# jlogan03/interpn

Hardware: AMD Instinct MI355X
Metric: Mpoints/sec (f64) per GPU + achieved HBM GB/s vs roofline, 3D linear-regular (higher is better)
Workload: dtype f64

## Files before the change

### interpn_amd/csrc/abi_binned.hip

```cpp
#include "abi_internal.h"

using namespace interpn;
using namespace interpn_abi;

namespace interpn_abi {


size_t bin_slice_points(const GridDesc& g) {
  const int lg = g.cfg.bin_slice_log2 >= 16 && g.cfg.bin_slice_log2 <= 27 ? g.cfg.bin_slice_log2 : 25;
  const size_t s = (size_t)1 << lg;
  return s < kBinSlicePoints ? s : kBinSlicePoints;
}

int binned_applies(const GridDesc& g, size_t npoints) {
  if (g.method != kCubic || !g.bricks || g.ndims < 2 || g.ndims > 4) return 0;
  if (g.cfg.binned == 0 || g.cfg.force_generic) return 1;
  const bool main11 = g.brick_step[0] == 1 && g.brick_step[1] == 1;
  const bool second = !main11 && g.bricks11 != nullptr;
  if (g.cfg.binned < 0) {
    if (g.ndims != 4 && g.ndims != 3) return 0;
    if (!main11 && !second) return 0;
    if (g.ndims == 3) return 0;
    if (main11) {
      unsigned nb[2];
// ... 117 lines not shown
    } else if (column) {
      if (g.dtype == kF64)
        err = launch_cubic_column<double>(*use, plan, extras, index, reinterpret_cast<double*>(dst), count, max_parts, h->first_bad, begin, stream);
      else
        err = launch_cubic_column<float>(*use, plan, extras, index, reinterpret_cast<float*>(dst), count, max_parts, h->first_bad, begin, stream);
    } else if (g.dtype == kF64) {
      err = launch_cubic_brick<double>(*use, reinterpret_cast<const double* const*>(sorted), reinterpret_cast<double*>(dst), count,
                                       h->first_bad, stream, index, begin);
    } else {
      err = launch_cubic_brick<float>(*use, reinterpret_cast<const float* const*>(sorted), reinterpret_cast<float*>(dst), count,
                                      h->first_bad, stream, index, begin);
    }
  }
  release_bin_slot(h, slot, stream, stage && err == hipSuccess && hipEventRecord(stage[4], stream) == hipSuccess);
  if (err == hipSuccess) {
    std::lock_guard<std::mutex> lk(h->bin_mu);
    h->desc.tag = use->tag;
    h->desc.last_binned = 1;
  }
  if (err != hipSuccess) {
    (void)hipGetLastError();
    return hip_fail(err);
  }
  return INTERPN_HIP_OK;
}

}

extern "C" {

int interpn_hip_eval_device_ex(interpn_hip_interp* h, const void* const* obs, size_t nobs, void* out, size_t npoints,
                               void* stream, unsigned flags, int* path_taken, int* why_out) {
  if (path_taken) *path_taken = INTERPN_HIP_PATH_IN_PLACE;
  if (why_out) *why_out = INTERPN_HIP_WHY_NONE;
  if (!h || (!obs && nobs)) return INTERPN_HIP_ERR_INVALID_ARGUMENT;
  if (flags & ~(unsigned)INTERPN_HIP_EVAL_NO_ALLOC) return INTERPN_HIP_ERR_INVALID_ARGUMENT;
  int st = validate_obs(h->desc, nullptr, nobs, npoints);
  if (st) return st;
  if (npoints == 0) return INTERPN_HIP_OK;
  if (!out) return INTERPN_HIP_ERR_INVALID_ARGUMENT;
  for (size_t i = 0; i < nobs; ++i)
    if (!obs[i]) return INTERPN_HIP_ERR_INVALID_ARGUMENT;
  DeviceGuard guard(h->device);
  if (!guard.ok()) return INTERPN_HIP_ERR_NO_DEVICE;
  int why = INTERPN_HIP_WHY_NONE;
  st = eval_device_binned(h, obs, out, npoints, static_cast<hipStream_t>(stream), flags, &why);
  if (why_out) *why_out = why;
  if (st > 0) {
    std::lock_guard<std::mutex> lk(h->marks_mu);
    h->sync_device_at_destroy = true;
    return st;
  }
  bool swept = false;
  if (st < 0 && sweep_applies(h->desc, npoints)) {
    int why_sweep = INTERPN_HIP_WHY_NONE;
    const int ss = eval_device_sweep(h, obs, out, npoints, static_cast<hipStream_t>(stream), flags, &why_sweep);
    if (why_out && (why == INTERPN_HIP_WHY_NONE || why_sweep > INTERPN_HIP_WHY_SMALL_OR_OFF)) *why_out = why_sweep;
    if (ss > 0) {
      std::lock_guard<std::mutex> lk(h->marks_mu);
      h->sync_device_at_destroy = true;
      return ss;
    }
    swept = ss == 0;
  }
  if (swept) {
    if (path_taken) *path_taken = INTERPN_HIP_PATH_SWEEP;
    h->desc.last_binned = 0;
    h->evals_sweep.fetch_add(1);
  } else if (st < 0) {
    HIP_TRY(launch_any(h->desc, obs, out, npoints, h->first_bad, static_cast<hipStream_t>(stream)));
    if (binned_applies(h->desc, npoints)) {
      std::lock_guard<std::mutex> lk(h->bin_mu);
      h->desc.last_binned = 0;
    } else {
      h->desc.last_binned = 0;
    }
    h->evals_in_place.fetch_add(1);
  } else {
    if (path_taken) *path_taken = INTERPN_HIP_PATH_BINNED;
    h->evals_binned.fetch_add(1);
  }
  mark_stream(h, static_cast<hipStream_t>(stream));
  return INTERPN_HIP_OK;
}

int interpn_hip_eval_device(interpn_hip_interp* h, const void* const* obs, size_t nobs, void* out, size_t npoints,
                            void* stream) {
  return interpn_hip_eval_device_ex(h, obs, nobs, out, npoints, stream, 0u, nullptr, nullptr);
}

int interpn_hip_stage_ms(interpn_hip_interp* h, double* ms, size_t n) {
  if (!h || !ms || n < 4) return INTERPN_HIP_ERR_INVALID_ARGUMENT;
  DeviceGuard guard(h->device);
  if (!guard.ok()) return INTERPN_HIP_ERR_NO_DEVICE;
  std::lock_guard<std::mutex> lk(h->bin_mu);
  const interpn_hip_interp::BinSlot* best = nullptr;
  for (const auto& sl : h->bin_slots)
    if (sl.staged && !sl.busy && (!best || sl.stamp > best->stamp)) best = &sl;
  if (!best) return INTERPN_HIP_ERR_INVALID_ARGUMENT;
  HIP_TRY(hipEventSynchronize(best->stage[4]));
  for (int k = 0; k < 4; ++k) {
    float f = 0.f;
    HIP_TRY(hipEventElapsedTime(&f, best->stage[k], best->stage[k + 1]));
    ms[k] = (double)f;
  }
  return INTERPN_HIP_OK;
}

int interpn_hip_reserve(interpn_hip_interp* h, size_t npoints, int nstreams) {
  if (!h || nstreams < 0) return INTERPN_HIP_ERR_INVALID_ARGUMENT;
  if ((size_t)nstreams > interpn_hip_interp::kMaxBinSlots) nstreams = (int)interpn_hip_interp::kMaxBinSlots;
  const GridDesc& g = h->desc;
  const bool sorts = binned_applies(g, npoints) >= 2, sweeps = sweep_applies(g, npoints) >= 2;
  if (npoints == 0 || nstreams == 0 || (!sorts && !sweeps)) return INTERPN_HIP_OK;
  DeviceGuard guard(h->device);
  if (!guard.ok()) return INTERPN_HIP_ERR_NO_DEVICE;
  const size_t slice_max = bin_slice_points(g);
  const size_t need = sorts ? bin_scratch_bytes(g, npoints < slice_max ? npoints : slice_max) : sweep_work_bytes();
  return reserve_slots(h, need, nstreams);
}

}
```

### interpn_amd/csrc/abi_create.hip

```cpp
#include "abi_internal.h"
#include "cubic_cell_record.h"

using namespace interpn;
using namespace interpn_abi;

namespace interpn_abi {

thread_local bool t_defer_tables = false;

int finish_create(interpn_hip_interp* h, const void* vals, size_t nvals, size_t elem, int vals_mem) {
  GridDesc& g = h->desc;
  {
    const DeviceProps dp = device_props(h->device);
    g.cfg.num_cus = dp.num_cus;
    g.cfg.num_xcds = dp.num_xcds;
    g.cfg.l2_bytes = dp.l2_bytes;
    g.cfg.lds_per_cu = dp.lds_per_cu;
    g.cfg.lds_per_wg = dp.lds_per_wg;
  }
  latch_env(g.cfg);
  g.nvals = nvals;
  if (vals_mem == INTERPN_HIP_MEM_DEVICE) {
    g.vals = vals;
  } else {
// ... 474 lines not shown
  g.axis_image = nullptr;
  g.tag = KernelTag();
  for (int d = 0; d < 8; ++d) g.grid[d] = nullptr;
  const size_t elem = g.dtype == kF64 ? 8 : 4;
  hipError_t e = pool_alloc(dev, &h->vals_owned, g.nvals * elem);
  if (e == hipSuccess) e = hipMemcpyPeer(h->vals_owned, dev, src->desc.vals, src->device, g.nvals * elem);
  if (e == hipSuccess && src->desc.axis_image && g.axis_alloc_bytes) {
    e = pool_alloc(dev, &h->grids_owned, g.axis_alloc_bytes);
    if (e == hipSuccess) e = hipMemcpyPeer(h->grids_owned, dev, src->desc.axis_image, src->device, g.axis_alloc_bytes);
    if (e == hipSuccess) {
      g.axis_image = h->grids_owned;
      for (int d = 0; d < g.ndims; ++d) g.grid[d] = (const char*)h->grids_owned + g.axis_g_off[d];
    }
  }
  if (e != hipSuccess) {
    interpn_hip_destroy(h);
    return hip_fail(e);
  }
  st = finish_create(h, h->vals_owned, g.nvals, elem, INTERPN_HIP_MEM_DEVICE);
  if (st) {
    interpn_hip_destroy(h);
    return st;
  }
  *out = h;
  return INTERPN_HIP_OK;
}

int interpn_hip_elem_size(const interpn_hip_interp* h) { return h ? (h->desc.dtype == kF64 ? 8 : 4) : 0; }
int interpn_hip_ndims(const interpn_hip_interp* h) { return h ? h->desc.ndims : 0; }
int interpn_hip_device(const interpn_hip_interp* h) { return h ? h->device : -1; }

void interpn_hip_destroy(interpn_hip_interp* h) {
  if (!h) return;
  DeviceGuard guard(h->device);
  scratch_slots::destroy_wait(*h, [h] {
    bool ok = true;
    for (auto& l : h->lane)
      if (l.stream && hipStreamSynchronize(l.stream) != hipSuccess) { (void)hipGetLastError(); ok = false; }
    return ok;
  });
  for (auto& l : h->lane) {
    if (l.stream) pool_return_kit(h->device, l.stream, l.flag_host);
    pool_free(h->device, l.flag_dev);
    pool_free(h->device, l.obs);
    pool_free(h->device, l.out);
  }
  pool_return_small(h->device, h->small_host);
  scratch_slots::free_blocks(*h, [](interpn_hip_interp::BinSlot& sl) {
    for (hipEvent_t e : sl.stage)
      if (e) (void)hipEventDestroy(e);
  });
  pool_free(h->device, h->first_bad);
  pool_return_pinned_word(h->device, h->finish_word);
  pool_return_pinned_word(h->device, h->sampling.host);
  pool_free(h->device, h->grids_owned);
  pool_free(h->device, h->bricks_owned);
  pool_free(h->device, h->bricks11_owned);
  pool_free(h->device, h->sweep_owned);
  pool_free(h->device, h->vals_owned);
  delete h;
}

}
```

### interpn_amd/csrc/abi_fields.hip

```cpp
#include <climits>

#include "abi_internal.h"

using namespace interpn;
using namespace interpn_abi;

namespace {

struct DeferTables {
  explicit DeferTables(bool on) { t_defer_tables = on; }
  ~DeferTables() { t_defer_tables = false; }
};

long long env_number(const char* name, long long fallback) {
  const char* env = getenv(name);
  if (!env || !*env) return fallback;
  char* end = nullptr;
  const long long v = strtoll(env, &end, 0);
  return (end == env || *end != 0) ? fallback : v;
}

}

namespace interpn_abi {
// ... 299 lines not shown
  for (size_t i = 0; i < nobs; ++i)
    if (!obs[i]) return INTERPN_HIP_ERR_INVALID_ARGUMENT;
  DeviceGuard guard(s->device);
  if (!guard.ok()) return INTERPN_HIP_ERR_NO_DEVICE;
  hipStream_t hs = static_cast<hipStream_t>(stream);
  const bool fused = columns_take_fused(s, npoints, hs, flags);
  st = eval_columns(s, fused, obs, out, out_stride, npoints, hs, flags);
  if (st == INTERPN_HIP_OK && fused && path_taken) *path_taken = INTERPN_HIP_FIELDS_PATH_FUSED;
  return st;
}

int interpn_hip_fields_finish(interpn_hip_fields* s, void* stream, uint64_t* first_bad_index) {
  if (!s || s->sub.empty()) return INTERPN_HIP_ERR_INVALID_ARGUMENT;
  const size_t count = s->per_field_pending ? s->nfields : 1;
  s->per_field_pending = false;
  if (count > 1 && count <= (size_t)kMaxStatusWords) {
    unsigned long long* words[kMaxStatusWords];
    for (size_t f = 0; f < count; ++f) words[f] = s->sub[f]->first_bad;
    const int st = finish_words(s->sub[0], static_cast<hipStream_t>(stream), words, (int)count, first_bad_index);
    if (st >= 0) return st;
  }
  int error = INTERPN_HIP_OK;
  uint64_t best = ~(uint64_t)0;
  for (size_t f = 0; f < count; ++f) {
    uint64_t bad = 0;
    const int st = interpn_hip_finish(s->sub[f], stream, &bad);
    if (st == s->sub[f]->desc.unrep_status) best = bad < best ? bad : best;
    else if (st != INTERPN_HIP_OK && error == INTERPN_HIP_OK) error = st;
  }
  if (error) return error;
  if (best != ~(uint64_t)0) {
    if (first_bad_index) *first_bad_index = best;
    return s->sub[0]->desc.unrep_status;
  }
  return INTERPN_HIP_OK;
}

int interpn_hip_fields_eval_host(interpn_hip_fields* s, const void* const* obs, const size_t* obs_lens, size_t nobs, void* out,
                                 size_t out_stride, size_t nout) {
  if (!s || s->sub.empty() || (!obs && nobs) || (!obs_lens && nobs)) return INTERPN_HIP_ERR_INVALID_ARGUMENT;
  int st = validate_obs(s->sub[0]->desc, obs_lens, nobs, nout);
  if (st) return st;
  if (nout == 0) return INTERPN_HIP_OK;
  if (!out || out_stride < nout) return INTERPN_HIP_ERR_INVALID_ARGUMENT;
  for (size_t i = 0; i < nobs; ++i)
    if (!obs[i]) return INTERPN_HIP_ERR_INVALID_ARGUMENT;
  DeviceGuard guard(s->device);
  if (!guard.ok()) return INTERPN_HIP_ERR_NO_DEVICE;
  const size_t elem = s->dtype == kF64 ? 8 : 4;
  const long long opt_chunk = s->sub[0]->desc.cfg.host_chunk;
  size_t chunk = opt_chunk >= 1 ? (size_t)opt_chunk : ((size_t)2 << 20);
  if (chunk > nout) chunk = nout;
  std::lock_guard<std::mutex> host_lock(s->host_mu);
  if (!s->stream) HIP_TRY(pool_take_kit(s->device, &s->stream, &s->kit_word));
  if (s->host_points < chunk) {
    HIP_TRY(hipStreamSynchronize(s->stream));
    pool_free(s->device, s->host_obs);
    pool_free(s->device, s->host_out);
    s->host_obs = s->host_out = nullptr;
    s->host_points = 0;
    HIP_TRY(pool_alloc(s->device, &s->host_obs, (size_t)s->ndims * chunk * elem));
    HIP_TRY(pool_alloc(s->device, &s->host_out, s->nfields * chunk * elem));
    s->host_points = chunk;
  }
  const size_t cap = s->host_points;
  char* dev_obs_base = static_cast<char*>(s->host_obs);
  char* dev_out = static_cast<char*>(s->host_out);
  const void* dev_obs[8];
  for (size_t begin = 0; begin < nout; begin += chunk) {
    const size_t count = nout - begin < chunk ? nout - begin : chunk;
    for (int d = 0; d < s->ndims; ++d) {
      char* dst = dev_obs_base + (size_t)d * cap * elem;
      HIP_TRY(hipMemcpyAsync(dst, static_cast<const char*>(obs[d]) + begin * elem, count * elem, hipMemcpyHostToDevice, s->stream));
      dev_obs[d] = dst;
    }
    st = interpn_hip_fields_eval_device(s, dev_obs, nobs, dev_out, cap, count, s->stream, 0u, nullptr);
    if (st) return st;
    uint64_t bad = 0;
    st = interpn_hip_fields_finish(s, s->stream, &bad);
    const bool failed = st == s->sub[0]->desc.unrep_status;
    if (st && !failed) return st;
    const size_t good = failed ? (size_t)bad : count;
    if (good)
      for (size_t f = 0; f < s->nfields; ++f)
        HIP_TRY(hipMemcpyAsync(static_cast<char*>(out) + (f * out_stride + begin) * elem, dev_out + f * cap * elem, good * elem,
                               hipMemcpyDeviceToHost, s->stream));
    HIP_TRY(hipStreamSynchronize(s->stream));
    if (failed) return st;
  }
  return INTERPN_HIP_OK;
}

int interpn_hip_fields_eval_points_device(interpn_hip_fields* s, const void* pts, size_t point_stride, size_t npoints, void* out,
                                          size_t out_stride, void* stream, unsigned flags, int* path_taken) {
  if (path_taken) *path_taken = INTERPN_HIP_FIELDS_POINTS_PATH_SPLIT;
  if (flags & ~(unsigned)INTERPN_HIP_EVAL_NO_ALLOC) return INTERPN_HIP_ERR_INVALID_ARGUMENT;
  bool nothing = false;
  int path = INTERPN_HIP_FIELDS_POINTS_PATH_SPLIT;
  const int st0 = points_checks(s, pts, point_stride, npoints, out, out_stride, &nothing, &path);
  if (st0 || nothing) return st0;
  DeviceGuard guard(s->device);
  if (!guard.ok()) return INTERPN_HIP_ERR_NO_DEVICE;
  const int st = points_device(s, path, pts, point_stride, npoints, out, out_stride, static_cast<hipStream_t>(stream), flags);
  if (st == INTERPN_HIP_OK && path_taken) *path_taken = path;
  return st;
}

int interpn_hip_fields_reserve_points(interpn_hip_fields* s, size_t npoints, int nstreams) {
  if (!s || s->sub.empty() || nstreams < 0) return INTERPN_HIP_ERR_INVALID_ARGUMENT;
  if ((size_t)nstreams > interpn_hip_interp::kMaxBinSlots) nstreams = (int)interpn_hip_interp::kMaxBinSlots;
  if (npoints == 0 || nstreams == 0) return INTERPN_HIP_OK;
  DeviceGuard guard(s->device);
  if (!guard.ok()) return INTERPN_HIP_ERR_NO_DEVICE;
  return reserve_slots(s->sub[0], points_need(s, npoints), nstreams);
}

int interpn_hip_fields_eval_points_host(interpn_hip_fields* s, const void* pts, size_t point_stride, size_t npoints, void* out,
                                        size_t out_stride) {
  bool nothing = false;
  int path = INTERPN_HIP_FIELDS_POINTS_PATH_SPLIT;
  const int st0 = points_checks(s, pts, point_stride, npoints, out, out_stride, &nothing, &path);
  if (st0 || nothing) return st0;
  DeviceGuard guard(s->device);
  if (!guard.ok()) return INTERPN_HIP_ERR_NO_DEVICE;
  const size_t elem = s->dtype == kF64 ? 8 : 4;
  const size_t nd = (size_t)s->ndims, k = s->nfields;
  const long long opt_chunk = s->sub[0]->desc.cfg.host_chunk;
  size_t chunk = opt_chunk >= 1 ? (size_t)opt_chunk : ((size_t)2 << 20);
  if (chunk > npoints) chunk = npoints;
  const size_t widest = point_stride > k ? point_stride : k;
  const size_t cap = ((size_t)256 << 20) / (widest * elem);
  if (chunk > cap) chunk = cap ? cap : 1;
  std::lock_guard<std::mutex> host_lock(s->host_mu);
  if (!s->stream) HIP_TRY(pool_take_kit(s->device, &s->stream, &s->kit_word));
  const size_t rows_bytes = align_up(chunk * point_stride * elem, 256);
  void* block = nullptr;
  if (pool_alloc(s->device, &block, rows_bytes + chunk * k * elem) != hipSuccess) { (void)hipGetLastError(); return INTERPN_HIP_ERR_OUT_OF_MEMORY; }
  char* results = static_cast<char*>(block) + rows_bytes;
  hipError_t err = hipSuccess;
  int st = INTERPN_HIP_OK;
  for (size_t begin = 0; begin < npoints && err == hipSuccess && st == INTERPN_HIP_OK; begin += chunk) {
    const size_t count = npoints - begin < chunk ? npoints - begin : chunk;
    err = hipMemcpyAsync(block, static_cast<const char*>(pts) + begin * point_stride * elem, ((count - 1) * point_stride + nd) * elem,
                         hipMemcpyHostToDevice, s->stream);
    if (err != hipSuccess) break;
    st = points_device(s, path, block, point_stride, count, results, k, s->stream, 0u);
    if (st) break;
    uint64_t bad = 0;
    st = interpn_hip_fields_finish(s, s->stream, &bad);
    const bool failed = st == s->sub[0]->desc.unrep_status;
    if (st && !failed) break;
    const size_t good = failed ? (size_t)bad : count;
    char* dst = static_cast<char*>(out) + begin * out_stride * elem;
    if (good && out_stride == k) err = hipMemcpyAsync(dst, results, good * k * elem, hipMemcpyDeviceToHost, s->stream);
    else if (good) err = hipMemcpy2DAsync(dst, out_stride * elem, results, k * elem, k * elem, good, hipMemcpyDeviceToHost, s->stream);
    if (err == hipSuccess) err = hipStreamSynchronize(s->stream);
  }
  (void)hipStreamSynchronize(s->stream);
  pool_free(s->device, block);
  if (err != hipSuccess) return hip_fail(err);
  return st;
}

void interpn_hip_fields_destroy(interpn_hip_fields* s) {
  if (!s) return;
  DeviceGuard guard(s->device);
  if (s->stream && hipStreamSynchronize(s->stream) != hipSuccess) (void)hipGetLastError();
  for (interpn_hip_interp* h : s->sub) interpn_hip_destroy(h);
  if (s->stream) pool_return_kit(s->device, s->stream, s->kit_word);
  pool_free(s->device, s->host_obs);
  pool_free(s->device, s->host_out);
  pool_free(s->device, s->host_grad);
  pool_free(s->device, s->table);
  pool_free(s->device, s->vals_owned);
  delete s;
}

size_t interpn_hip_fields_count(const interpn_hip_fields* s) { return s ? s->nfields : 0; }
int interpn_hip_fields_ndims(const interpn_hip_fields* s) { return s ? s->ndims : 0; }
int interpn_hip_fields_elem_size(const interpn_hip_fields* s) { return s ? (s->dtype == kF64 ? 8 : 4) : 0; }
int interpn_hip_fields_device(const interpn_hip_fields* s) { return s ? s->device : -1; }

int interpn_hip_fields_kernel_name(const interpn_hip_fields* s, char* buf, size_t buflen) {
  if (!s || s->sub.empty()) return INTERPN_HIP_ERR_INVALID_ARGUMENT;
  return interpn_hip_kernel_name(s->sub[0], buf, buflen);
}
// ... 56 lines not shown
```

### interpn_amd/csrc/abi_fields_grad.hip

```cpp
#include "abi_internal.h"

using namespace interpn;
using namespace interpn_abi;

namespace {

bool grad_auto_takes_fused(const interpn_hip_fields* s) { return s->table != nullptr; }

bool grad_takes_fused(const interpn_hip_fields* s) {
  return s->table && (s->fused == 1 || (s->fused < 0 && grad_auto_takes_fused(s)));
}

int fields_grad_checks(const interpn_hip_fields* s, const void* const* obs, const size_t* obs_lens, bool need_lens, size_t nobs,
                       const void* out, size_t out_stride, const void* grad, size_t grad_stride, size_t npoints, bool* nothing) {
  *nothing = false;
  if (!s || s->sub.empty() || (!obs && nobs) || (need_lens && !obs_lens && nobs)) return INTERPN_HIP_ERR_INVALID_ARGUMENT;
  const int method = s->sub[0]->desc.method;
  if (method != kLinear && method != kCubic) return INTERPN_HIP_ERR_UNSUPPORTED;
  const int st = validate_obs(s->sub[0]->desc, obs_lens, nobs, npoints);
  if (st) return st;
  if (npoints == 0) { *nothing = true; return INTERPN_HIP_OK; }
  if (!out || out_stride < npoints || !grad || grad_stride < npoints) return INTERPN_HIP_ERR_INVALID_ARGUMENT;
  for (size_t i = 0; i < nobs; ++i)
    if (!obs[i]) return INTERPN_HIP_ERR_INVALID_ARGUMENT;
// ... 12 lines not shown
    return INTERPN_HIP_OK;
  }
  if (!s->sub_tables && !(flags & INTERPN_HIP_EVAL_NO_ALLOC) && !stream_capturing(hs)) {
    const int st = ensure_sub_tables(s);
    if (st) return st;
  }
  const size_t elem = s->dtype == kF64 ? 8 : 4;
  const size_t nd = (size_t)s->ndims;
  const bool cubic = s->sub[0]->desc.method == kCubic;
  s->per_field_pending = true;
  s->last_path = INTERPN_HIP_FIELDS_PATH_PER_FIELD;
  for (size_t f = 0; f < s->nfields; ++f) {
    void* rows[8];
    for (size_t d = 0; d < nd; ++d) rows[d] = static_cast<char*>(grad) + (f * nd + d) * grad_stride * elem;
    void* out_f = static_cast<char*>(out) + f * out_stride * elem;
    const int st = cubic ? interpn_hip_eval_cubic_grad_device(s->sub[f], obs, nobs, out_f, rows, npoints, hs)
                         : interpn_hip_eval_grad_device(s->sub[f], obs, nobs, out_f, rows, npoints, hs);
    if (st) return st;
  }
  return INTERPN_HIP_OK;
}

}

extern "C" {

int interpn_hip_fields_eval_grad_device(interpn_hip_fields* s, const void* const* obs, size_t nobs, void* out, size_t out_stride,
                                        void* grad, size_t grad_stride, size_t npoints, void* stream, unsigned flags,
                                        int* path_taken) {
  if (path_taken) *path_taken = INTERPN_HIP_FIELDS_PATH_PER_FIELD;
  if (flags & ~(unsigned)INTERPN_HIP_EVAL_NO_ALLOC) return INTERPN_HIP_ERR_INVALID_ARGUMENT;
  bool nothing = false;
  const int st = fields_grad_checks(s, obs, nullptr, false, nobs, out, out_stride, grad, grad_stride, npoints, &nothing);
  if (st || nothing) return st;
  DeviceGuard guard(s->device);
  if (!guard.ok()) return INTERPN_HIP_ERR_NO_DEVICE;
  return fields_grad_device(s, obs, nobs, out, out_stride, grad, grad_stride, npoints, static_cast<hipStream_t>(stream), flags,
                            path_taken);
}

int interpn_hip_fields_eval_grad_host(interpn_hip_fields* s, const void* const* obs, const size_t* obs_lens, size_t nobs, void* out,
                                      size_t out_stride, void* grad, size_t grad_stride, size_t nout) {
  bool nothing = false;
  int st = fields_grad_checks(s, obs, obs_lens, true, nobs, out, out_stride, grad, grad_stride, nout, &nothing);
  if (st || nothing) return st;
  DeviceGuard guard(s->device);
  if (!guard.ok()) return INTERPN_HIP_ERR_NO_DEVICE;
  const size_t elem = s->dtype == kF64 ? 8 : 4;
  const size_t nd = (size_t)s->ndims;
  const long long opt_chunk = s->sub[0]->desc.cfg.host_chunk;
  size_t chunk = opt_chunk >= 1 ? (size_t)opt_chunk : ((size_t)2 << 20);
  if (chunk > nout) chunk = nout;
  std::lock_guard<std::mutex> host_lock(s->host_mu);
  if (!s->stream) HIP_TRY(pool_take_kit(s->device, &s->stream, &s->kit_word));
  if (s->host_points < chunk) {
    HIP_TRY(hipStreamSynchronize(s->stream));
    pool_free(s->device, s->host_obs);
    pool_free(s->device, s->host_out);
    s->host_obs = s->host_out = nullptr;
    s->host_points = 0;
    HIP_TRY(pool_alloc(s->device, &s->host_obs, nd * chunk * elem));
    HIP_TRY(pool_alloc(s->device, &s->host_out, s->nfields * chunk * elem));
    s->host_points = chunk;
  }
  if (s->host_grad_points < chunk) {
    HIP_TRY(hipStreamSynchronize(s->stream));
    pool_free(s->device, s->host_grad);
    s->host_grad = nullptr;
    s->host_grad_points = 0;
    HIP_TRY(pool_alloc(s->device, &s->host_grad, s->nfields * nd * chunk * elem));
    s->host_grad_points = chunk;
  }
  const size_t cap = s->host_points, gcap = s->host_grad_points;
  char* dev_obs_base = static_cast<char*>(s->host_obs);
  char* dev_out = static_cast<char*>(s->host_out);
  char* dev_grad = static_cast<char*>(s->host_grad);
  const void* dev_obs[8];
  for (size_t begin = 0; begin < nout; begin += chunk) {
    const size_t count = nout - begin < chunk ? nout - begin : chunk;
    for (size_t d = 0; d < nd; ++d) {
      char* dst = dev_obs_base + d * cap * elem;
      HIP_TRY(hipMemcpyAsync(dst, static_cast<const char*>(obs[d]) + begin * elem, count * elem, hipMemcpyHostToDevice, s->stream));
      dev_obs[d] = dst;
    }
    st = fields_grad_device(s, dev_obs, nobs, dev_out, cap, dev_grad, gcap, count, s->stream, 0u, nullptr);
    if (st) return st;
    uint64_t bad = 0;
    st = interpn_hip_fields_finish(s, s->stream, &bad);
    const bool failed = st == s->sub[0]->desc.unrep_status;
    if (st && !failed) return st;
    const size_t good = failed ? (size_t)bad : count;
    if (good)
      for (size_t f = 0; f < s->nfields; ++f) {
        HIP_TRY(hipMemcpyAsync(static_cast<char*>(out) + (f * out_stride + begin) * elem, dev_out + f * cap * elem, good * elem,
                               hipMemcpyDeviceToHost, s->stream));
        for (size_t d = 0; d < nd; ++d)
          HIP_TRY(hipMemcpyAsync(static_cast<char*>(grad) + ((f * nd + d) * grad_stride + begin) * elem,
                                 dev_grad + (f * nd + d) * gcap * elem, good * elem, hipMemcpyDeviceToHost, s->stream));
      }
    HIP_TRY(hipStreamSynchronize(s->stream));
    if (failed) return st;
  }
  return INTERPN_HIP_OK;
}

}
// ... 1 lines not shown
```

### interpn_amd/csrc/abi_fields_lattice.hip

```cpp
#include "abi_internal.h"
#include "lattice.h"

using namespace interpn;
using namespace interpn_abi;

namespace {

using Slot = interpn_hip_interp::BinSlot;

constexpr size_t kHostChunkPointsFields = (size_t)1 << 25;

bool layout_ok(int layout) { return layout == INTERPN_HIP_FIELDS_LATTICE_FIELD_MAJOR || layout == INTERPN_HIP_FIELDS_LATTICE_FIELDS_LAST; }

FieldsLatticePlan plan_for(const interpn_hip_fields* s, const LatticeShape& sh, int layout) {
  const GridDesc& g = s->sub[0]->desc;
  if (!fast_path(g) || g.cfg.force_generic) return FieldsLatticePlan();
  return fields_lattice_plan(g.method, g.ndims, g.dtype == kF64 ? 8 : 4, g.n, sh.m, s->nfields, layout, lattice_lds_budget(g.cfg),
                             g.cfg.num_cus, g.cfg.lattice);
}

size_t slice_leading(const interpn_hip_fields* s, const LatticeShape& sh) {
  const size_t elem = s->dtype == kF64 ? 8 : 4;
  size_t points = kExpandSliceBytes / (s->nfields * elem);
  const long long opt = s->sub[0]->desc.cfg.points_slice;
// ... 126 lines not shown
}

}

extern "C" {

int interpn_hip_fields_eval_lattice_device(interpn_hip_fields* s, const void* const* axes, const size_t* axis_lens, size_t naxes,
                                           void* out, size_t out_stride, int layout, void* stream, unsigned flags, int* path_taken) {
  if (path_taken) *path_taken = INTERPN_HIP_FIELDS_LATTICE_PATH_PER_FIELD;
  if (flags & ~(unsigned)INTERPN_HIP_EVAL_NO_ALLOC) return INTERPN_HIP_ERR_INVALID_ARGUMENT;
  LatticeShape sh;
  bool empty = false;
  const int st = checks(s, axes, axis_lens, naxes, out, out_stride, layout, &sh, &empty);
  if (st || empty) return st;
  DeviceGuard guard(s->device);
  if (!guard.ok()) return INTERPN_HIP_ERR_NO_DEVICE;
  return fields_lattice_device(s, sh, out, out_stride, layout, static_cast<hipStream_t>(stream), flags, path_taken);
}

int interpn_hip_fields_reserve_lattice(interpn_hip_fields* s, const size_t* axis_lens, size_t naxes, int nstreams) {
  if (!s || s->sub.empty() || nstreams < 0 || (!axis_lens && naxes)) return INTERPN_HIP_ERR_INVALID_ARGUMENT;
  interpn_hip_interp* h0 = s->sub[0];
  if (is_one_dim(h0->desc.method)) return INTERPN_HIP_ERR_UNSUPPORTED;
  int st = validate_obs(h0->desc, nullptr, naxes, 0);
  if (st) return st;
  LatticeShape sh;
  st = lattice_make_shape(nullptr, axis_lens, naxes, &sh);
  if (st) return st;
  if ((size_t)nstreams > interpn_hip_interp::kMaxBinSlots) nstreams = (int)interpn_hip_interp::kMaxBinSlots;
  if (sh.npoints == 0 || nstreams == 0) return INTERPN_HIP_OK;
  DeviceGuard guard(s->device);
  if (!guard.ok()) return INTERPN_HIP_ERR_NO_DEVICE;
  for (size_t f = 1; f < s->nfields; ++f) {
    st = reserve_slots(s->sub[f], lattice_reserve_need(s->sub[f]->desc, sh), nstreams);
    if (st) return st;
  }
  size_t need = lattice_reserve_need(h0->desc, sh);
  const size_t rows = join_need(s, sh);
  if (rows > need) need = rows;
  int blocks = 2 * nstreams;
  if ((size_t)blocks > interpn_hip_interp::kMaxBinSlots) blocks = (int)interpn_hip_interp::kMaxBinSlots;
  return reserve_slots(h0, need, blocks);
}

int interpn_hip_fields_eval_lattice_host(interpn_hip_fields* s, const void* const* axes, const size_t* axis_lens, size_t naxes,
                                         void* out, size_t out_stride, int layout, uint64_t* first_bad_index) {
  LatticeShape sh;
  bool empty = false;
  int st = checks(s, axes, axis_lens, naxes, out, out_stride, layout, &sh, &empty);
  if (st || empty) return st;
  DeviceGuard guard(s->device);
  if (!guard.ok()) return INTERPN_HIP_ERR_NO_DEVICE;
  std::lock_guard<std::mutex> host_lock(s->host_mu);
  if (!s->stream) HIP_TRY(pool_take_kit(s->device, &s->stream, &s->kit_word));
  const size_t elem = s->dtype == kF64 ? 8 : 4;
  const size_t k = s->nfields;
  const bool last = layout == INTERPN_HIP_FIELDS_LATTICE_FIELDS_LAST;
  const size_t per0 = (size_t)sh.weight[0];
  const long long opt_chunk = s->sub[0]->desc.cfg.host_chunk;
  const size_t chunk_points = opt_chunk >= 1 ? (size_t)opt_chunk : kHostChunkPointsFields / k;
  size_t rows0 = chunk_points / per0;
  if (rows0 < 1) rows0 = 1;
  if (rows0 > sh.m[0]) rows0 = sh.m[0];
  size_t axes_bytes = 0, off[8] = {0};
  for (int d = 0; d < sh.ndims; ++d) { off[d] = axes_bytes; axes_bytes += align_up(sh.m[d] * elem, 256); }
  void* block = nullptr;
  if (pool_alloc(s->device, &block, axes_bytes + rows0 * per0 * k * elem) != hipSuccess) { (void)hipGetLastError(); return INTERPN_HIP_ERR_OUT_OF_MEMORY; }
  char* dev_out = static_cast<char*>(block) + axes_bytes;
  hipError_t err = hipSuccess;
  for (int d = 0; d < sh.ndims && err == hipSuccess; ++d)
    err = hipMemcpyAsync(static_cast<char*>(block) + off[d], axes[d], sh.m[d] * elem, hipMemcpyHostToDevice, s->stream);
  st = INTERPN_HIP_OK;
  for (size_t i0 = 0; i0 < sh.m[0] && err == hipSuccess && st == INTERPN_HIP_OK; i0 += rows0) {
    const size_t cnt0 = sh.m[0] - i0 < rows0 ? sh.m[0] - i0 : rows0;
    const void* sub_axes[8];
    size_t sub_lens[8];
    for (int d = 0; d < sh.ndims; ++d) {
      sub_axes[d] = static_cast<char*>(block) + off[d] + (d == 0 ? i0 * elem : 0);
      sub_lens[d] = d == 0 ? cnt0 : sh.m[d];
    }
    LatticeShape sub;
    st = lattice_make_shape(sub_axes, sub_lens, (size_t)sh.ndims, &sub);
    if (st) break;
    const size_t count = sub.npoints;
    st = fields_lattice_device(s, sub, dev_out, last ? k : count, layout, s->stream, 0u, nullptr);
    if (st) break;
    uint64_t bad = 0;
    st = interpn_hip_fields_finish(s, s->stream, &bad);
    const bool failed = st == s->sub[0]->desc.unrep_status;
    if (st && !failed) break;
    const size_t good = failed ? (size_t)bad : count;
    if (failed && first_bad_index) *first_bad_index = (uint64_t)(i0 * per0 + good);
    if (good && !last) {
      for (size_t f = 0; f < k && err == hipSuccess; ++f)
        err = hipMemcpyAsync(static_cast<char*>(out) + (f * out_stride + i0 * per0) * elem, dev_out + f * count * elem, good * elem,
                             hipMemcpyDeviceToHost, s->stream);
    } else if (good) {
      char* dst = static_cast<char*>(out) + i0 * per0 * out_stride * elem;
      if (out_stride == k) err = hipMemcpyAsync(dst, dev_out, good * k * elem, hipMemcpyDeviceToHost, s->stream);
      else err = hipMemcpy2DAsync(dst, out_stride * elem, dev_out, k * elem, k * elem, good, hipMemcpyDeviceToHost, s->stream);
    }
    if (err == hipSuccess) err = hipStreamSynchronize(s->stream);
  }
  (void)hipStreamSynchronize(s->stream);
  pool_free(s->device, block);
  if (err != hipSuccess) return hip_fail(err);
// ... 26 lines not shown
```

### interpn_amd/csrc/abi_grad.hip

```cpp
#include "abi_internal.h"

using namespace interpn;
using namespace interpn_abi;

namespace {

constexpr size_t kGradChunkPoints = (size_t)2 << 20;

struct PoolBlock {
  int device;
  void* p = nullptr;
  explicit PoolBlock(int dev) : device(dev) {}
  ~PoolBlock() { if (p) pool_free(device, p); }
};

int grad_checks(interpn_hip_interp* h, int method, const void* const* obs, const size_t* obs_lens, bool need_lens, size_t nobs,
                void* out, void* const* grad, size_t npoints, bool* nothing) {
  *nothing = false;
  if (!h || (!obs && nobs) || (need_lens && !obs_lens && nobs)) return INTERPN_HIP_ERR_INVALID_ARGUMENT;
  if (h->desc.method != method) return INTERPN_HIP_ERR_UNSUPPORTED;
  const int st = validate_obs(h->desc, obs_lens, nobs, npoints);
  if (st) return st;
  if (npoints == 0) { *nothing = true; return INTERPN_HIP_OK; }
  if (!out || !grad) return INTERPN_HIP_ERR_INVALID_ARGUMENT;
  for (size_t i = 0; i < nobs; ++i)
    if (!obs[i] || !grad[i]) return INTERPN_HIP_ERR_INVALID_ARGUMENT;
  return INTERPN_HIP_OK;
}

}

namespace interpn_abi {

hipError_t launch_grad(const GridDesc& g, const void* const* obs, void* out, void* const* grad, size_t npts,
                       unsigned long long* first_bad, hipStream_t stream) {
  return g.method == kCubic ? launch_cubic_grad(g, obs, out, grad, npts, first_bad, stream)
                            : launch_linear_grad(g, obs, out, grad, npts, first_bad, stream);
}

}

namespace {

int grad_device(interpn_hip_interp* h, int method, const void* const* obs, size_t nobs, void* out, void* const* grad,
                size_t npoints, void* stream) {
  bool nothing = false;
  const int st = grad_checks(h, method, obs, nullptr, false, nobs, out, grad, npoints, &nothing);
  if (st || nothing) return st;
  DeviceGuard guard(h->device);
  if (!guard.ok()) return INTERPN_HIP_ERR_NO_DEVICE;
  HIP_TRY(launch_grad(h->desc, obs, out, grad, npoints, h->first_bad, static_cast<hipStream_t>(stream)));
  h->desc.last_binned = 0;
  h->evals_in_place.fetch_add(1);
  mark_stream(h, static_cast<hipStream_t>(stream));
  return INTERPN_HIP_OK;
}

int grad_host(interpn_hip_interp* h, int method, const void* const* obs, const size_t* obs_lens, size_t nobs, void* out, size_t nout,
              void* const* grad) {
  bool nothing = false;
  const int st0 = grad_checks(h, method, obs, obs_lens, true, nobs, out, grad, nout, &nothing);
  if (st0 || nothing) return st0;
  std::lock_guard<std::mutex> host_lock(h->host_mu);
  DeviceGuard guard(h->device);
  if (!guard.ok()) return INTERPN_HIP_ERR_NO_DEVICE;
  const size_t elem = h->desc.dtype == kF64 ? 8 : 4;
  const int nd = h->desc.ndims;
  size_t chunk = nout < kGradChunkPoints ? nout : kGradChunkPoints;
  if (h->desc.cfg.host_chunk >= 1)
    chunk = (size_t)h->desc.cfg.host_chunk < nout ? (size_t)h->desc.cfg.host_chunk : nout;
  const int st = ensure_lane(h, 0, chunk);
  if (st) return st;
  const interpn_hip_interp::HostLane& l = h->lane[0];
  PoolBlock gbuf(h->device);
  if (pool_alloc(h->device, &gbuf.p, (size_t)nd * chunk * elem) != hipSuccess) {
    (void)hipGetLastError();
    gbuf.p = nullptr;
    return INTERPN_HIP_ERR_OUT_OF_MEMORY;
  }
  const void* dev_obs[8];
  void* dev_grad[8];
  for (int d = 0; d < nd; ++d) {
    dev_obs[d] = (char*)l.obs + (size_t)d * l.points * elem;
    dev_grad[d] = (char*)gbuf.p + (size_t)d * chunk * elem;
  }
  for (size_t begin = 0; begin < nout; begin += chunk) {
    const size_t count = (nout - begin) < chunk ? (nout - begin) : chunk;
    for (int d = 0; d < nd; ++d)
      HIP_TRY(hipMemcpyAsync(const_cast<void*>(dev_obs[d]), (const char*)obs[d] + begin * elem, count * elem, hipMemcpyHostToDevice, l.stream));
    HIP_TRY(launch_grad(h->desc, dev_obs, l.out, dev_grad, count, l.flag_dev, l.stream));
    HIP_TRY(hipMemcpyAsync(l.flag_host, l.flag_dev, sizeof(unsigned long long), hipMemcpyDeviceToHost, l.stream));
    HIP_TRY(hipStreamSynchronize(l.stream));
    const unsigned long long bad = *l.flag_host;
    size_t good = count;
    if (bad != kNoBadIndexHost) {
      HIP_TRY(hipMemsetAsync(l.flag_dev, 0xFF, sizeof(unsigned long long), l.stream));
      good = (size_t)bad;
    }
    if (good) {
      HIP_TRY(hipMemcpyAsync((char*)out + begin * elem, l.out, good * elem, hipMemcpyDeviceToHost, l.stream));
      for (int d = 0; d < nd; ++d)
        HIP_TRY(hipMemcpyAsync((char*)grad[d] + begin * elem, dev_grad[d], good * elem, hipMemcpyDeviceToHost, l.stream));
    }
    HIP_TRY(hipStreamSynchronize(l.stream));
    if (bad != kNoBadIndexHost) return h->desc.unrep_status;
  }
  return INTERPN_HIP_OK;
}

}

extern "C" {

int interpn_hip_eval_grad_device(interpn_hip_interp* h, const void* const* obs, size_t nobs, void* out, void* const* grad,
                                 size_t npoints, void* stream) {
  return grad_device(h, kLinear, obs, nobs, out, grad, npoints, stream);
// ... 19 lines not shown
```

### interpn_amd/csrc/abi_host.hip

```cpp
#include "abi_internal.h"

using namespace interpn;
using namespace interpn_abi;

namespace interpn_abi {

int ensure_lane(interpn_hip_interp* h, int which, size_t points) {
  interpn_hip_interp::HostLane& l = h->lane[which];
  if (l.points >= points && l.obs) return INTERPN_HIP_OK;
  const size_t elem = h->desc.dtype == kF64 ? 8 : 4;
  if (l.obs) { HIP_TRY(hipStreamSynchronize(l.stream)); pool_free(h->device, l.obs); l.obs = nullptr; }
  if (l.out) { pool_free(h->device, l.out); l.out = nullptr; }
  l.points = 0;
  if (!l.stream) HIP_TRY(pool_take_kit(h->device, &l.stream, &l.flag_host));
  HIP_TRY(pool_alloc(h->device, &l.obs, (size_t)h->desc.ndims * points * elem));
  HIP_TRY(pool_alloc(h->device, &l.out, points * elem));
  if (!l.flag_dev) {
    HIP_TRY(pool_alloc(h->device, (void**)&l.flag_dev, sizeof(unsigned long long)));
    HIP_TRY(hipMemsetAsync(l.flag_dev, 0xFF, sizeof(unsigned long long), l.stream));
  }
  l.points = points;
  return INTERPN_HIP_OK;
}

// ... 80 lines not shown
    void* buf = nullptr;
    if (pool_take_small(h->device, &buf) != hipSuccess) { (void)hipGetLastError(); return kSmallPathUnavailable; }
    void* dbuf = nullptr;
    if (hipHostGetDevicePointer(&dbuf, buf, 0) != hipSuccess || !dbuf) {
      (void)hipGetLastError();
      pool_return_small(h->device, buf);
      return kSmallPathUnavailable;
    }
    h->small_host = buf;
    h->small_dev = dbuf;
  }
  if (!l.stream) HIP_TRY(pool_take_kit(h->device, &l.stream, &l.flag_host));
  if (!l.flag_dev) {
    HIP_TRY(pool_alloc(h->device, (void**)&l.flag_dev, sizeof(unsigned long long)));
    HIP_TRY(hipMemsetAsync(l.flag_dev, 0xFF, sizeof(unsigned long long), l.stream));
  }
  const size_t elem = h->desc.dtype == kF64 ? 8 : 4;
  const int nd = h->desc.ndims;
  const size_t stride = kSmallPoints * 8;
  const void* dev_obs[8];
  for (int d = 0; d < nd; ++d) {
    memcpy((char*)h->small_host + (size_t)d * stride, obs[d], nout * elem);
    dev_obs[d] = (const char*)h->small_dev + (size_t)d * stride;
  }
  char* host_out = (char*)h->small_host + (size_t)8 * stride;
  void* dev_out = (char*)h->small_dev + (size_t)8 * stride;
  HIP_TRY(launch_any(h->desc, dev_obs, dev_out, nout, l.flag_dev, l.stream));
  HIP_TRY(hipMemcpyAsync(l.flag_host, l.flag_dev, sizeof(unsigned long long), hipMemcpyDeviceToHost, l.stream));
  HIP_TRY(hipStreamSynchronize(l.stream));
  const unsigned long long bad = *l.flag_host;
  size_t good = nout;
  if (bad != kNoBadIndexHost) {
    HIP_TRY(hipMemsetAsync(l.flag_dev, 0xFF, sizeof(unsigned long long), l.stream));
    good = (size_t)bad;
  }
  if (good) memcpy(out, host_out, good * elem);
  if (bad != kNoBadIndexHost) {
    if (bad_index) *bad_index = (size_t)bad;
    return h->desc.unrep_status;
  }
  return INTERPN_HIP_OK;
}

constexpr size_t kPipelineChunkPoints = (size_t)2 << 20;

}

namespace interpn_abi {

int eval_host_impl(interpn_hip_interp* h, const void* const* obs, size_t nobs, void* out, size_t nout,
                          size_t* bad_index) {
  (void)nobs;
  std::lock_guard<std::mutex> host_lock(h->host_mu);
  DeviceGuard guard(h->device);
  if (!guard.ok()) return INTERPN_HIP_ERR_NO_DEVICE;
  if (nout <= kSmallPoints && h->desc.cfg.host_chunk < 1) {
    const int sst = eval_host_small(h, obs, out, nout, bad_index);
    if (sst != kSmallPathUnavailable) return sst;
  }
  HostPipeline p;
  p.h = h;
  p.obs = obs;
  p.out = out;
  p.nout = nout;
  p.chunk = nout <= kPipelineChunkPoints ? nout : kPipelineChunkPoints;
  if (h->desc.cfg.host_chunk >= 1)
    p.chunk = (size_t)h->desc.cfg.host_chunk < nout ? (size_t)h->desc.cfg.host_chunk : nout;
  p.nchunks = (nout + p.chunk - 1) / p.chunk;
  int st = ensure_lane(h, 0, p.chunk);
  if (st) return st;
  if (p.nchunks > 1) {
    st = ensure_lane(h, 1, p.chunk);
    if (st) return st;
    std::thread helper([&p] { p.lane_main(1); });
    p.lane_main(0);
    helper.join();
  } else {
    p.checked[1] = ~(size_t)0;
    p.lane_main(0);
  }
  if (p.error) return p.error;
  if (p.fail_chunk != ~(size_t)0) {
    if (bad_index) *bad_index = p.fail_index;
    return h->desc.unrep_status;
  }
  return INTERPN_HIP_OK;
}

}

namespace {
struct StatusWords {
  const unsigned long long* word[interpn_abi::kMaxStatusWords];
  int count;
};
__global__ void k_status_to_host(StatusWords w, unsigned long long* host_word) {
  unsigned long long v = ~0ull;
  for (int k = 0; k < w.count; ++k) {
    const unsigned long long x = __hip_atomic_load(w.word[k], __ATOMIC_RELAXED, __HIP_MEMORY_SCOPE_AGENT);
    v = x < v ? x : v;
  }
  __hip_atomic_store(host_word, v, __ATOMIC_RELEASE, __HIP_MEMORY_SCOPE_SYSTEM);
}
}

namespace interpn_abi {

int finish_words(interpn_hip_interp* h, hipStream_t s, unsigned long long* const* words, int count, uint64_t* first_bad_index) {
  DeviceGuard guard(h->device);
  if (!guard.ok()) return INTERPN_HIP_ERR_NO_DEVICE;
  std::lock_guard<std::mutex> lk(h->finish_mu);
  if (!h->finish_word) {
    HIP_TRY(pool_take_pinned_word(h->device, &h->finish_word));
    void* dp = nullptr;
    if (hipHostGetDevicePointer(&dp, h->finish_word, 0) == hipSuccess) h->finish_word_dev = static_cast<unsigned long long*>(dp);
    else (void)hipGetLastError();
  }
  hipStreamCaptureStatus cs = hipStreamCaptureStatusNone;
  const hipError_t asked = hipStreamIsCapturing(s, &cs);
  if (asked != hipSuccess) (void)hipGetLastError();
  const bool by_kernel = h->finish_word_dev && h->desc.cfg.finish_kernel != 0 && count <= kMaxStatusWords && asked == hipSuccess &&
                         cs == hipStreamCaptureStatusNone;
  if (!by_kernel && count > 1) return -1;
  if (by_kernel) {
    StatusWords w;
    for (int k = 0; k < kMaxStatusWords; ++k) w.word[k] = words[k < count ? k : 0];
    w.count = count;
    hipLaunchKernelGGL(k_status_to_host, dim3(1), dim3(1), 0, s, w, h->finish_word_dev);
    HIP_TRY(hipGetLastError());
  } else {
    HIP_TRY(hipMemcpyAsync(h->finish_word, words[0], sizeof(unsigned long long), hipMemcpyDeviceToHost, s));
  }
  HIP_TRY(hipStreamSynchronize(s));
  const unsigned long long word = *(volatile unsigned long long*)h->finish_word;
  if (word == kNoBadIndexHost) return INTERPN_HIP_OK;
  for (int k = 0; k < count; ++k) HIP_TRY(hipMemsetAsync(words[k], 0xFF, sizeof(word), s));
  HIP_TRY(hipStreamSynchronize(s));
  if (first_bad_index) *first_bad_index = (uint64_t)word;
  return h->desc.unrep_status;
}

}

extern "C" {

int interpn_hip_finish(interpn_hip_interp* h, void* stream, uint64_t* first_bad_index) {
  if (!h) return INTERPN_HIP_ERR_INVALID_ARGUMENT;
  return finish_words(h, static_cast<hipStream_t>(stream), &h->first_bad, 1, first_bad_index);
}

int interpn_hip_eval_host(interpn_hip_interp* h, const void* const* obs, const size_t* obs_lens, size_t nobs,
                          void* out, size_t nout) {
  if (!h || (!obs && nobs) || (!obs_lens && nobs)) return INTERPN_HIP_ERR_INVALID_ARGUMENT;
  int st = validate_obs(h->desc, obs_lens, nobs, nout);
  if (st) return st;
  if (nout == 0) return INTERPN_HIP_OK;
  if (!out) return INTERPN_HIP_ERR_INVALID_ARGUMENT;
  for (size_t i = 0; i < nobs; ++i)
    if (!obs[i]) return INTERPN_HIP_ERR_INVALID_ARGUMENT;
  return eval_host_impl(h, obs, nobs, out, nout, nullptr);
}

#define ONESHOT_TAIL(T)                                                                         \
  st = interpn_hip_eval_host(h, reinterpret_cast<const void* const*>(obs), obs_lens, nobs, out, nout); \
  interpn_hip_destroy(h);                                                                       \
  return st;

#define ONESHOT_PRECHECK(METHOD, NDIMS, VALIDATE)                  \
  {                                                                \
    int pst = (VALIDATE);                                          \
    if (pst) return pst;                                           \
    GridDesc tmp;                                                  \
    tmp.method = (METHOD);                                         \
    tmp.ndims = (int)(NDIMS);                                      \
    if (!obs_lens && nobs) return INTERPN_HIP_ERR_INVALID_ARGUMENT; \
    pst = validate_obs(tmp, obs_lens, nobs, nout);                 \
    if (pst) return pst;                                           \
  }

#define DEFINE_ONESHOT(T, SUFFIX)                                                                             \
  int interpn_hip_linear_regular_##SUFFIX(const size_t* dims, size_t ndims, const T* starts, size_t nstarts, \
                                          const T* steps, size_t nsteps, const T* vals, size_t nvals,        \
                                          const T* const* obs, const size_t* obs_lens, size_t nobs, T* out,  \
                                          size_t nout) {                                                     \
                                                                               \
    if (nstarts != ndims || nsteps != ndims || nobs != ndims) return INTERPN_HIP_ERR_DIM_MISMATCH;           \
    ONESHOT_PRECHECK(kLinear, ndims, validate_regular<T>(kLinear, dims, ndims, starts, nstarts, steps, nsteps, nvals)) \
    interpn_hip_interp* h = nullptr;                                                                         \
// ... 73 lines not shown
```

### interpn_amd/csrc/abi_internal.h

```cpp
#pragma once
#include <hip/hip_runtime.h>

#include <atomic>
#include <condition_variable>
#include <cctype>
#include <cmath>
#include <cstdint>
#include <cstdio>
#include <cstdlib>
#include <cstring>
#include <chrono>
#include <mutex>
#include <new>
#include <string>
#include <thread>
#include <unordered_map>
#include <vector>

#include "../../include/interpn_hip.h"
#include "interpn_host.h"
#include "scratch_slots.h"

namespace interpn {
hipError_t launch_linear_grad(const GridDesc& g, const void* const* obs, void* out, void* const* grad, size_t npts,
// ... 71 lines not shown
  using Stream = hipStream_t;
  using Event = hipEvent_t;
  static constexpr int kNotReady = (int)hipErrorNotReady;
  const int* device = nullptr;
  int is_capturing(Stream s, bool* capturing) const {
    hipStreamCaptureStatus cs = hipStreamCaptureStatusNone;
    const hipError_t e = hipStreamIsCapturing(s, &cs);
    *capturing = cs != hipStreamCaptureStatusNone;
    return (int)e;
  }
  int event_create(Event* ev) const { return (int)hipEventCreateWithFlags(ev, hipEventDisableTiming); }
  int event_destroy(Event ev) const { return (int)hipEventDestroy(ev); }
  int event_record(Event ev, Stream s) const { return (int)hipEventRecord(ev, s); }
  int event_query(Event ev) const { return (int)hipEventQuery(ev); }
  int event_synchronize(Event ev) const { return (int)hipEventSynchronize(ev); }
  int stream_wait_event(Stream s, Event ev) const { return (int)hipStreamWaitEvent(s, ev, 0); }
  int stream_synchronize(Stream s) const { return (int)hipStreamSynchronize(s); }
  int device_synchronize() const { return (int)hipDeviceSynchronize(); }
  void clear_last_error() const { (void)hipGetLastError(); }
  int alloc_block(void** out, size_t bytes) const { return (int)pool_alloc(*device, out, bytes); }
  void free_block(void* p) const { pool_free(*device, p); }
};

}

struct interpn_hip_interp : scratch_slots::Table<interpn_abi::HipRuntime> {
  interpn::GridDesc desc;
  int device = 0;
  void* vals_owned = nullptr;
  void* grids_owned = nullptr;
  void* bricks_owned = nullptr;
  void* bricks11_owned = nullptr;
  void* sweep_owned = nullptr;
  unsigned long long* first_bad = nullptr;
  unsigned long long* finish_word = nullptr;
  unsigned long long* finish_word_dev = nullptr;
  std::mutex finish_mu;
  std::mutex host_mu;
  struct HostLane {
    size_t points = 0;
    void* obs = nullptr;
    void* out = nullptr;
    unsigned long long* flag_dev = nullptr;
    unsigned long long* flag_host = nullptr;
    hipStream_t stream = nullptr;
  } lane[2];
  void* small_host = nullptr;
  void* small_dev = nullptr;
  interpn_hip_interp() {
    rt.device = &device;
    word_in_block = &sampling.last_word;
  }
  std::atomic<long long> evals_binned{0}, evals_in_place{0}, evals_sweep{0};
  struct SweepSampling {
    unsigned long long* host = nullptr;
    unsigned* host_dev = nullptr;
    unsigned seq = 0, seen = 0;
    int streak = 0;
    int streak_coherent = 0;
    int skipped = 0;
    const void* last_word = nullptr;
  } sampling;
};

struct interpn_hip_fields {
  int device = 0;
  int dtype = interpn::kF64;
  int ndims = 0;
  size_t nfields = 0;
  size_t field_stride = 0;
  size_t field_elems = 0;
  int per_line = 0;
  size_t lines = 0;
  void* vals_owned = nullptr;
  const void* vals = nullptr;
  std::vector<interpn_hip_interp*> sub;
  void* table = nullptr;
  size_t table_bytes = 0;
  int fused = -1;
  int last_path = INTERPN_HIP_FIELDS_PATH_PER_FIELD;
  int points_path = -1;
  int last_points_path = -1;
  int last_lattice_path = -1;
  int last_lattice_group = 0;
  bool sub_tables = true;
  bool per_field_pending = false;
  std::mutex mu;
  std::mutex host_mu;
  hipStream_t stream = nullptr;
  unsigned long long* kit_word = nullptr;
  void* host_obs = nullptr;
  void* host_out = nullptr;
  size_t host_points = 0;
  void* host_grad = nullptr;
  size_t host_grad_points = 0;
};

namespace interpn {
struct LatticeShape;
struct LatticePlan;
}

namespace interpn_abi {

template <typename T>
int validate_regular(int method, const size_t* dims, size_t ndims, const T* starts, size_t nstarts,
// ... 82 lines not shown
int create_one_dim(int method, int kind, T start, T step, const T* grid, size_t ngrid, const T* vals, size_t nvals,
                   int vals_mem, int device, interpn_hip_interp** handle);

inline size_t align_up(size_t v, size_t a) { return (v + a - 1) / a * a; }

inline bool stream_capturing(hipStream_t stream) {
  hipStreamCaptureStatus cs = hipStreamCaptureStatusNone;
  if (hipStreamIsCapturing(stream, &cs) != hipSuccess) { (void)hipGetLastError(); return true; }
  return cs != hipStreamCaptureStatusNone;
}

inline int fail_sequence(interpn_hip_interp* h, hipError_t err, int st) {
  (void)hipGetLastError();
  std::lock_guard<std::mutex> lk(h->marks_mu);
  h->sync_device_at_destroy = true;
  return err != hipSuccess ? hip_fail(err) : st;
}

hipError_t launch_any(const GridDesc& g, const void* const* obs, void* out, size_t npts,
                      unsigned long long* first_bad, hipStream_t stream);
void mark_stream(interpn_hip_interp* h, hipStream_t stream);
constexpr size_t kHostChunkPoints = (size_t)4 << 20;

constexpr int kMaxStatusWords = 32;
int finish_words(interpn_hip_interp* h, hipStream_t s, unsigned long long* const* words, int count, uint64_t* first_bad_index);

int binned_applies(const GridDesc& g, size_t npoints);
interpn_hip_interp::BinSlot* take_bin_slot(interpn_hip_interp* h, size_t need, hipStream_t stream, bool may_alloc, int* why);
void release_bin_slot(interpn_hip_interp* h, interpn_hip_interp::BinSlot* slot, hipStream_t stream, bool staged);
bool settle_slot(interpn_hip_interp* h, interpn_hip_interp::BinSlot& slot);

interpn_hip_interp::BinSlot* take_slot_captured(interpn_hip_interp* h, size_t need, hipStream_t stream);
void release_slot_captured(interpn_hip_interp* h, interpn_hip_interp::BinSlot* slot);
void claim_slot(interpn_hip_interp* h, interpn_hip_interp::BinSlot* slot);
int reserve_slots(interpn_hip_interp* h, size_t need, int nstreams);
int lattice_plan_args(size_t elem_size, int method, size_t ndims, const size_t* dims, const size_t* axis_lens, int* n,
                      interpn::LatticeShape* s, bool* indexable);
int lattice_make_shape(const void* const* axes, const size_t* axis_lens, size_t naxes, interpn::LatticeShape* s);
int validate_lattice(const interpn_hip_interp* h, const void* const* axes, const size_t* axis_lens, size_t naxes, const void* out,
                     interpn::LatticeShape* s, bool* empty);
interpn::LatticePlan lattice_plan_for(const GridDesc& g, const interpn::LatticeShape& s);
size_t lattice_scratch_need(const GridDesc& g, const interpn::LatticeShape& s, const interpn::LatticePlan& p);
size_t lattice_reserve_need(const GridDesc& g, const interpn::LatticeShape& s);
size_t lattice_expand_slice(const GridDesc& g, size_t npoints);
int lattice_device(interpn_hip_interp* h, const interpn::LatticeShape& s, void* out, hipStream_t stream, unsigned flags, int* path_taken);
constexpr size_t kExpandSliceBytes = (size_t)64 << 20;
constexpr size_t kExpandSliceMin = (size_t)1 << 16;

int ensure_sub_tables(interpn_hip_fields* s);

hipError_t launch_grad(const GridDesc& g, const void* const* obs, void* out, void* const* grad, size_t npts,
                       unsigned long long* first_bad, hipStream_t stream);

int eval_device_sweep(interpn_hip_interp* h, const void* const* obs, void* out, size_t npoints, hipStream_t stream,
                      unsigned flags, int* why);

int ensure_lane(interpn_hip_interp* h, int which, size_t points);
int eval_host_impl(interpn_hip_interp* h, const void* const* obs, size_t nobs, void* out, size_t nout, size_t* bad_index);

}
```

### interpn_amd/csrc/abi_lattice.hip

```cpp
#include "abi_internal.h"
#include "lattice.h"

using namespace interpn;
using namespace interpn_abi;

namespace interpn_abi {

using Slot = interpn_hip_interp::BinSlot;

Slot* take_slot_captured(interpn_hip_interp* h, size_t need, hipStream_t stream) { return scratch_slots::take_slot_captured(*h, need, stream); }

void release_slot_captured(interpn_hip_interp* h, Slot* slot) { scratch_slots::release_slot_captured(*h, slot); }

void claim_slot(interpn_hip_interp* h, Slot* slot) {
  std::lock_guard<std::mutex> lk(h->bin_mu);
  slot->totals_clean = false;
  slot->sweep_clean = false;
  slot->staged = false;
  const unsigned char* word = static_cast<const unsigned char*>(h->sampling.last_word);
  const unsigned char* base = static_cast<const unsigned char*>(slot->scratch);
  if (word && word >= base && word < base + slot->bytes) h->sampling.last_word = nullptr;
}

int reserve_slots(interpn_hip_interp* h, size_t need, int nstreams) {
// ... 159 lines not shown
  LatticeShape s;
  bool indexable = false;
  const int st = lattice_plan_args(elem_size, method, ndims, dims, axis_lens, n, &s, &indexable);
  if (st) return st;
  method &= 0xFF;
  LaunchConfig c;
  latch_env(c);
  LatticePlan p;
  if (indexable && s.npoints && !c.force_generic)
    p = lattice_plan(method, (int)ndims, elem_size, n, s.m, lattice_lds_budget(c), c.num_cus, c.lattice);
  if (path) *path = p.fused ? INTERPN_HIP_LATTICE_PATH_FUSED : INTERPN_HIP_LATTICE_PATH_EXPANDED;
  if (lds_bytes) *lds_bytes = p.lds_bytes;
  if (npoints) *npoints = s.npoints;
  return INTERPN_HIP_OK;
}

int interpn_hip_eval_lattice_device(interpn_hip_interp* h, const void* const* axes, const size_t* axis_lens, size_t naxes,
                                    void* out, void* stream, unsigned flags, int* path_taken) {
  if (path_taken) *path_taken = INTERPN_HIP_LATTICE_PATH_EXPANDED;
  if (flags & ~(unsigned)INTERPN_HIP_EVAL_NO_ALLOC) return INTERPN_HIP_ERR_INVALID_ARGUMENT;
  LatticeShape s;
  bool empty = false;
  const int st = validate_lattice(h, axes, axis_lens, naxes, out, &s, &empty);
  if (st || empty) return st;
  DeviceGuard guard(h->device);
  if (!guard.ok()) return INTERPN_HIP_ERR_NO_DEVICE;
  return lattice_device(h, s, out, static_cast<hipStream_t>(stream), flags, path_taken);
}

int interpn_hip_reserve_lattice(interpn_hip_interp* h, const size_t* axis_lens, size_t naxes, int nstreams) {
  if (!h || nstreams < 0 || (!axis_lens && naxes)) return INTERPN_HIP_ERR_INVALID_ARGUMENT;
  if (is_one_dim(h->desc.method)) return INTERPN_HIP_ERR_UNSUPPORTED;
  int st = validate_obs(h->desc, nullptr, naxes, 0);
  if (st) return st;
  LatticeShape s;
  st = lattice_make_shape(nullptr, axis_lens, naxes, &s);
  if (st) return st;
  if ((size_t)nstreams > interpn_hip_interp::kMaxBinSlots) nstreams = (int)interpn_hip_interp::kMaxBinSlots;
  if (s.npoints == 0 || nstreams == 0) return INTERPN_HIP_OK;
  const GridDesc& g = h->desc;
  const size_t need = lattice_reserve_need(g, s);
  DeviceGuard guard(h->device);
  if (!guard.ok()) return INTERPN_HIP_ERR_NO_DEVICE;
  return reserve_slots(h, need, nstreams);
}

int interpn_hip_eval_lattice_host(interpn_hip_interp* h, const void* const* axes, const size_t* axis_lens, size_t naxes,
                                  void* out, uint64_t* first_bad_index) {
  LatticeShape s;
  bool empty = false;
  int st = validate_lattice(h, axes, axis_lens, naxes, out, &s, &empty);
  if (st || empty) return st;
  std::lock_guard<std::mutex> host_lock(h->host_mu);
  DeviceGuard guard(h->device);
  if (!guard.ok()) return INTERPN_HIP_ERR_NO_DEVICE;
  interpn_hip_interp::HostLane& l = h->lane[0];
  if (!l.stream) HIP_TRY(pool_take_kit(h->device, &l.stream, &l.flag_host));
  const size_t elem = h->desc.dtype == kF64 ? 8 : 4;
  const size_t per0 = (size_t)s.weight[0];
  size_t rows0 = kHostChunkPointsLattice / per0;
  if (rows0 < 1) rows0 = 1;
  if (rows0 > s.m[0]) rows0 = s.m[0];
  size_t axes_bytes = 0, off[8] = {0};
  for (int d = 0; d < s.ndims; ++d) { off[d] = axes_bytes; axes_bytes += align_up(s.m[d] * elem, 256); }
  void* block = nullptr;
  HIP_TRY(pool_alloc(h->device, &block, axes_bytes + rows0 * per0 * elem));
  char* dev_out = static_cast<char*>(block) + axes_bytes;
  hipError_t err = hipSuccess;
  for (int d = 0; d < s.ndims && err == hipSuccess; ++d)
    err = hipMemcpyAsync(static_cast<char*>(block) + off[d], axes[d], s.m[d] * elem, hipMemcpyHostToDevice, l.stream);
  st = INTERPN_HIP_OK;
  for (size_t i0 = 0; i0 < s.m[0] && err == hipSuccess && st == INTERPN_HIP_OK; i0 += rows0) {
    const size_t cnt0 = s.m[0] - i0 < rows0 ? s.m[0] - i0 : rows0;
    const void* sub_axes[8];
    size_t sub_lens[8];
    for (int d = 0; d < s.ndims; ++d) {
      sub_axes[d] = static_cast<char*>(block) + off[d] + (d == 0 ? i0 * elem : 0);
      sub_lens[d] = d == 0 ? cnt0 : s.m[d];
    }
    LatticeShape sub;
    st = lattice_make_shape(sub_axes, sub_lens, (size_t)s.ndims, &sub);
    if (st) break;
    st = lattice_device(h, sub, dev_out, l.stream, 0u, nullptr);
    if (st) break;
    err = hipMemcpyAsync(l.flag_host, h->first_bad, sizeof(unsigned long long), hipMemcpyDeviceToHost, l.stream);
    if (err == hipSuccess) err = hipStreamSynchronize(l.stream);
    if (err != hipSuccess) break;
    const unsigned long long bad = *l.flag_host;
    size_t good = sub.npoints;
    if (bad != kNoBadIndexHost) {
      err = hipMemsetAsync(h->first_bad, 0xFF, sizeof(unsigned long long), l.stream);
      good = (size_t)bad;
      if (first_bad_index) *first_bad_index = (uint64_t)(i0 * per0 + good);
      st = h->desc.unrep_status;
    }
    if (good && err == hipSuccess)
      err = hipMemcpyAsync(static_cast<char*>(out) + i0 * per0 * elem, dev_out, good * elem, hipMemcpyDeviceToHost, l.stream);
    if (err == hipSuccess) err = hipStreamSynchronize(l.stream);
  }
  (void)hipStreamSynchronize(l.stream);
  pool_free(h->device, block);
  if (err != hipSuccess) return hip_fail(err);
  return st;
}

}
// ... 1 lines not shown
```

### interpn_amd/csrc/abi_lattice_grad.hip

```cpp
#include "abi_internal.h"
#include "lattice.h"

using namespace interpn;
using namespace interpn_abi;

namespace {

using Slot = interpn_hip_interp::BinSlot;

constexpr size_t kHostChunkResultsLatticeGrad = (size_t)1 << 25;

LatticePlan grad_plan_for(const GridDesc& g, const LatticeShape& s) {
  if (!fast_path(g) || g.cfg.force_generic) return LatticePlan();
  return lattice_grad_plan(g.method, g.ndims, g.dtype == kF64 ? 8 : 4, g.n, s.m, lattice_lds_budget(g.cfg), g.cfg.num_cus, g.cfg.lattice);
}

int lattice_grad_device(interpn_hip_interp* h, const LatticeShape& s, void* out, void* const* grad, hipStream_t stream, unsigned flags,
                        int* path_taken) {
  const GridDesc& g = h->desc;
  const LatticePlan plan = grad_plan_for(g, s);
  const size_t elem = g.dtype == kF64 ? 8 : 4;
  const bool capturing = stream_capturing(stream);
  const size_t need = lattice_scratch_need(g, s, plan);
  Slot* slot = nullptr;
// ... 48 lines not shown
  if (st) return st;
  if (h->desc.method != kLinear && h->desc.method != kCubic) return INTERPN_HIP_ERR_UNSUPPORTED;
  if (*empty) return INTERPN_HIP_OK;
  if (!grad) return INTERPN_HIP_ERR_INVALID_ARGUMENT;
  for (size_t d = 0; d < naxes; ++d)
    if (!grad[d]) return INTERPN_HIP_ERR_INVALID_ARGUMENT;
  return INTERPN_HIP_OK;
}

}

extern "C" {

int interpn_hip_lattice_grad_plan(size_t elem_size, int method, size_t ndims, const size_t* dims, const size_t* axis_lens,
                                  int* path, size_t* lds_bytes, size_t* npoints) {
  int n[8] = {0};
  LatticeShape s;
  bool indexable = false;
  const int st = lattice_plan_args(elem_size, method, ndims, dims, axis_lens, n, &s, &indexable);
  if (st) return st;
  method &= 0xFF;
  if (method == kNearest) return INTERPN_HIP_ERR_UNSUPPORTED;
  LaunchConfig c;
  latch_env(c);
  LatticePlan p;
  if (indexable && s.npoints && !c.force_generic)
    p = lattice_grad_plan(method, (int)ndims, elem_size, n, s.m, lattice_lds_budget(c), c.num_cus, c.lattice);
  if (path) *path = p.fused ? INTERPN_HIP_LATTICE_PATH_FUSED : INTERPN_HIP_LATTICE_PATH_EXPANDED;
  if (lds_bytes) *lds_bytes = p.lds_bytes;
  if (npoints) *npoints = s.npoints;
  return INTERPN_HIP_OK;
}

int interpn_hip_eval_lattice_grad_device(interpn_hip_interp* h, const void* const* axes, const size_t* axis_lens, size_t naxes,
                                         void* out, void* const* grad, void* stream, unsigned flags, int* path_taken) {
  if (path_taken) *path_taken = INTERPN_HIP_LATTICE_PATH_EXPANDED;
  if (flags & ~(unsigned)INTERPN_HIP_EVAL_NO_ALLOC) return INTERPN_HIP_ERR_INVALID_ARGUMENT;
  LatticeShape s;
  bool empty = false;
  const int st = checks(h, axes, axis_lens, naxes, out, grad, &s, &empty);
  if (st || empty) return st;
  DeviceGuard guard(h->device);
  if (!guard.ok()) return INTERPN_HIP_ERR_NO_DEVICE;
  return lattice_grad_device(h, s, out, grad, static_cast<hipStream_t>(stream), flags, path_taken);
}

int interpn_hip_eval_lattice_grad_host(interpn_hip_interp* h, const void* const* axes, const size_t* axis_lens, size_t naxes,
                                       void* out, void* const* grad, uint64_t* first_bad_index) {
  LatticeShape s;
  bool empty = false;
  int st = checks(h, axes, axis_lens, naxes, out, grad, &s, &empty);
  if (st || empty) return st;
  std::lock_guard<std::mutex> host_lock(h->host_mu);
  DeviceGuard guard(h->device);
  if (!guard.ok()) return INTERPN_HIP_ERR_NO_DEVICE;
  interpn_hip_interp::HostLane& l = h->lane[0];
  if (!l.stream) HIP_TRY(pool_take_kit(h->device, &l.stream, &l.flag_host));
  const size_t elem = h->desc.dtype == kF64 ? 8 : 4;
  const int nd = s.ndims;
  const size_t per0 = (size_t)s.weight[0];
  const long long opt_chunk = h->desc.cfg.host_chunk;
  const size_t chunk_points = opt_chunk >= 1 ? (size_t)opt_chunk : kHostChunkResultsLatticeGrad / (size_t)(nd + 1);
  size_t rows0 = chunk_points / per0;
  if (rows0 < 1) rows0 = 1;
  if (rows0 > s.m[0]) rows0 = s.m[0];
  size_t axes_bytes = 0, off[8] = {0};
  for (int d = 0; d < nd; ++d) { off[d] = axes_bytes; axes_bytes += align_up(s.m[d] * elem, 256); }
  const size_t pitch = align_up(rows0 * per0 * elem, 256);
  void* block = nullptr;
  if (pool_alloc(h->device, &block, axes_bytes + (size_t)(nd + 1) * pitch) != hipSuccess) { (void)hipGetLastError(); return INTERPN_HIP_ERR_OUT_OF_MEMORY; }
  char* dev_out = static_cast<char*>(block) + axes_bytes;
  void* dev_grad[8] = {nullptr};
  for (int d = 0; d < nd; ++d) dev_grad[d] = dev_out + (size_t)(d + 1) * pitch;
  hipError_t err = hipSuccess;
  for (int d = 0; d < nd && err == hipSuccess; ++d)
    err = hipMemcpyAsync(static_cast<char*>(block) + off[d], axes[d], s.m[d] * elem, hipMemcpyHostToDevice, l.stream);
  st = INTERPN_HIP_OK;
  for (size_t i0 = 0; i0 < s.m[0] && err == hipSuccess && st == INTERPN_HIP_OK; i0 += rows0) {
    const size_t cnt0 = s.m[0] - i0 < rows0 ? s.m[0] - i0 : rows0;
    const void* sub_axes[8];
    size_t sub_lens[8];
    for (int d = 0; d < nd; ++d) {
      sub_axes[d] = static_cast<char*>(block) + off[d] + (d == 0 ? i0 * elem : 0);
      sub_lens[d] = d == 0 ? cnt0 : s.m[d];
    }
    LatticeShape sub;
    st = lattice_make_shape(sub_axes, sub_lens, (size_t)nd, &sub);
    if (st) break;
    st = lattice_grad_device(h, sub, dev_out, dev_grad, l.stream, 0u, nullptr);
    if (st) break;
    err = hipMemcpyAsync(l.flag_host, h->first_bad, sizeof(unsigned long long), hipMemcpyDeviceToHost, l.stream);
    if (err == hipSuccess) err = hipStreamSynchronize(l.stream);
    if (err != hipSuccess) break;
    const unsigned long long bad = *l.flag_host;
    size_t good = sub.npoints;
    if (bad != kNoBadIndexHost) {
      err = hipMemsetAsync(h->first_bad, 0xFF, sizeof(unsigned long long), l.stream);
      good = (size_t)bad;
      if (first_bad_index) *first_bad_index = (uint64_t)(i0 * per0 + good);
      st = h->desc.unrep_status;
    }
    if (good && err == hipSuccess)
      err = hipMemcpyAsync(static_cast<char*>(out) + i0 * per0 * elem, dev_out, good * elem, hipMemcpyDeviceToHost, l.stream);
    for (int d = 0; d < nd && good && err == hipSuccess; ++d)
      err = hipMemcpyAsync(static_cast<char*>(grad[d]) + i0 * per0 * elem, dev_grad[d], good * elem, hipMemcpyDeviceToHost, l.stream);
    if (err == hipSuccess) err = hipStreamSynchronize(l.stream);
// ... 9 lines not shown
```

### interpn_amd/csrc/abi_launch.hip

```cpp
#include "abi_internal.h"

using namespace interpn;
using namespace interpn_abi;

namespace interpn_abi {

template <typename T>
hipError_t launch(const GridDesc& g, const T* const* obs, T* out, size_t npts, unsigned long long* first_bad,
                  hipStream_t stream) {
  if (npts == 0) return hipSuccess;
  if (g.method == kNearest) return launch_nearest<T>(g, obs, out, npts, first_bad, stream);
  if (g.cfg.force_generic || !fast_path(g)) return launch_generic<T>(g, obs, out, npts, first_bad, stream);
  if (g.method == kLinear)
    return g.kind == kRegular ? launch_linear_regular<T>(g, obs, out, npts, first_bad, stream)
                              : launch_linear_rectilinear<T>(g, obs, out, npts, first_bad, stream);
  return g.kind == kRegular ? launch_cubic_regular<T>(g, obs, out, npts, first_bad, stream)
                            : launch_cubic_rectilinear<T>(g, obs, out, npts, first_bad, stream);
}

hipError_t launch_any(const GridDesc& g, const void* const* obs, void* out, size_t npts,
                      unsigned long long* first_bad, hipStream_t stream) {
  if (is_one_dim(g.method)) return launch_one_dim(g, obs[0], out, npts, first_bad, stream);
  if (g.bricks && npts && g.method == kCubic && !g.cfg.force_generic) {
    if (g.dtype == kF64)
      return launch_cubic_brick<double>(g, reinterpret_cast<const double* const*>(obs), static_cast<double*>(out),
                                        npts, first_bad, stream);
    return launch_cubic_brick<float>(g, reinterpret_cast<const float* const*>(obs), static_cast<float*>(out), npts,
                                     first_bad, stream);
  }
  if (g.bricks && npts && g.ndims == 1 && g.method == kLinear && g.rec1_buckets && !g.cfg.force_generic) {
    if (g.dtype == kF64)
      return launch_linear1_records<double>(g, reinterpret_cast<const double* const*>(obs), static_cast<double*>(out), npts, stream);
    return launch_linear1_records<float>(g, reinterpret_cast<const float* const*>(obs), static_cast<float*>(out), npts, stream);
  }
  if (g.bricks && npts && g.ndims == 2 && !g.cfg.force_generic) {
    if (g.dtype == kF64)
      return launch_linear2_brick<double>(g, reinterpret_cast<const double* const*>(obs), static_cast<double*>(out),
                                          npts, first_bad, stream);
    return launch_linear2_brick<float>(g, reinterpret_cast<const float* const*>(obs), static_cast<float*>(out), npts,
                                       first_bad, stream);
  }
  if (g.bricks && npts && !g.cfg.force_generic) {
    if (g.dtype == kF64)
      return launch_linear_brick<double>(g, reinterpret_cast<const double* const*>(obs), static_cast<double*>(out),
                                         npts, first_bad, stream);
    return launch_linear_brick<float>(g, reinterpret_cast<const float* const*>(obs), static_cast<float*>(out), npts,
                                      first_bad, stream);
  }
  if (g.dtype == kF64)
    return launch<double>(g, reinterpret_cast<const double* const*>(obs), static_cast<double*>(out), npts, first_bad, stream);
  return launch<float>(g, reinterpret_cast<const float* const*>(obs), static_cast<float*>(out), npts, first_bad, stream);
}

void mark_stream(interpn_hip_interp* h, hipStream_t stream) { scratch_slots::mark_stream(*h, stream); }

}
```

### interpn_amd/csrc/abi_options.hip

```cpp
#include "abi_internal.h"

using namespace interpn;
using namespace interpn_abi;

namespace interpn_abi {

bool option_access(LaunchConfig& c, const char* name, long long* value, bool set) {
  struct Opt { const char* name; int* field; long long lo, hi; };
  const Opt opts[] = {
      {"blocks_per_cu", &c.blocks_per_cu, 1, 65536},
      {"iters_per_block", &c.iters_per_block, 0, 65536},
      {"ppl", &c.ppl, 0, 2},
      {"axis_regs", &c.axis_regs, -1, 2},
      {"force_generic", &c.force_generic, 0, 1},
      {"generic_runtime", &c.generic_runtime, 0, 1},
      {"generic_vec", &c.generic_vec, -1, 1},
      {"persistent", &c.persistent, 0, 1},
      {"axis_lds_kb", &c.axis_lds_kb, -1, 60},
      {"binned", &c.binned, -1, 1},
      {"deal", &c.deal, 0, 1},
      {"bin_slice_log2", &c.bin_slice_log2, 16, 27},
      {"column", &c.column, -1, 1},
      {"column_part", &c.column_part, 0, 1 << 20},
      {"column_threads", &c.column_threads, 256, 1024},
// ... 111 lines not shown
  if (!strcmp(name, "fma")) { *value = h->desc.fma; return INTERPN_HIP_OK; }
  if (!strcmp(name, "last_lattice_path")) { *value = h->desc.last_lattice_path; return INTERPN_HIP_OK; }
  if (!strcmp(name, "last_points_path")) { *value = h->desc.last_points_path; return INTERPN_HIP_OK; }
  if (!strcmp(name, "axis_rec_mode")) { *value = h->desc.axis_rec_bytes ? (h->desc.axis_rec_compact ? 2 : 1) : 0; return INTERPN_HIP_OK; }
  if (!strcmp(name, "axis_rec_bytes")) { *value = h->desc.axis_rec_bytes; return INTERPN_HIP_OK; }
  if (!strcmp(name, "axis_image_bytes")) { *value = h->desc.axis_image_bytes; return INTERPN_HIP_OK; }
  {
    const LaunchConfig& c = h->desc.cfg;
    const Thresholds t = thresholds(c);
    const struct { const char* nm; long long v; } ro[] = {
        {"dev_num_cus", c.num_cus}, {"dev_num_xcds", c.num_xcds}, {"dev_l2_bytes", c.l2_bytes}, {"dev_lds_per_cu", c.lds_per_cu},
        {"dev_lds_per_wg", c.lds_per_wg}, {"thr_table_l2_sized", (long long)t.table_l2_sized}, {"thr_table_l2_share", (long long)t.table_l2_share},
        {"thr_binned_table_min", (long long)t.binned_table_min}, {"thr_binned_points_min", (long long)t.binned_points_min},
        {"thr_bin_table_share", (long long)t.bin_table_share}, {"thr_axis_lds", (long long)t.axis_lds},
        {"thr_axis_lds_wide", (long long)t.axis_lds_wide}, {"thr_column_lds", (long long)t.column_lds}};
    for (const auto& r : ro)
      if (!strcmp(name, r.nm)) { *value = r.v; return INTERPN_HIP_OK; }
  }
  if (!strncmp(name, "col_", 4)) {
    ColumnPlan cp;
    const bool ok = h->desc.method == kCubic && h->desc.ndims == 4 && cubic_column_plan(h->desc, &cp);
    const struct { const char* nm; long long v; } ro[] = {
        {"col_applies", ok ? 1 : 0}, {"col_nphase", ok ? cp.nphase : 0}, {"col_cpp", ok ? cp.cpp : 0}, {"col_pitch", ok ? (long long)cp.pitch : 0},
        {"col_lds_bytes", ok ? (long long)cp.lds_bytes : 0}, {"col_part_points", ok ? (long long)cp.part_points : 0},
        {"col_perm_pad", ok ? (long long)cp.perm_pad : 0}, {"col_q3", ok ? cp.q3 : 0}, {"col_sh3", ok ? cp.sh3 : 0},
        {"col_threads", ok ? cp.threads : 0}, {"col_groups", ok ? cp.groups : 0}};
    for (const auto& r : ro)
      if (!strcmp(name, r.nm)) { *value = r.v; return INTERPN_HIP_OK; }
    return INTERPN_HIP_ERR_INVALID_ARGUMENT;
  }
  if (!strcmp(name, "evals_binned")) { *value = h->evals_binned.load(); return INTERPN_HIP_OK; }
  if (!strcmp(name, "evals_in_place")) { *value = h->evals_in_place.load(); return INTERPN_HIP_OK; }
  if (!strcmp(name, "evals_sweep")) { *value = h->evals_sweep.load(); return INTERPN_HIP_OK; }
  if (!strcmp(name, "sweep_table_bytes")) { *value = h->desc.sweep_bricks ? (long long)h->desc.sweep_table_bytes : 0; return INTERPN_HIP_OK; }
  if (!strcmp(name, "sweep_probe_took_brick")) {
    interpn_hip_interp* hm = const_cast<interpn_hip_interp*>(h);
    std::lock_guard<std::mutex> lk(hm->bin_mu);
    const unsigned char* word = static_cast<const unsigned char*>(hm->sampling.last_word);
    bool idle = false;
    for (const auto& sl : hm->bin_slots) {
      const unsigned char* base = static_cast<const unsigned char*>(sl.scratch);
      if (!sl.busy && word && base && word >= base && word + sizeof(unsigned) <= base + sl.bytes) idle = true;
    }
    *value = -1;
    if (idle) {
      DeviceGuard guard(h->device);
      if (!guard.ok()) return INTERPN_HIP_ERR_NO_DEVICE;
      unsigned w = 0;
      if (hipDeviceSynchronize() != hipSuccess || hipMemcpy(&w, word, sizeof(w), hipMemcpyDeviceToHost) != hipSuccess) { (void)hipGetLastError(); return INTERPN_HIP_ERR_INVALID_ARGUMENT; }
      *value = w ? 1 : 0;
    }
    return INTERPN_HIP_OK;
  }
  if (!strcmp(name, "sweep_probe_streak")) {
    interpn_hip_interp* hm = const_cast<interpn_hip_interp*>(h);
    std::lock_guard<std::mutex> lk(hm->bin_mu);
    *value = hm->sampling.streak;
    return INTERPN_HIP_OK;
  }
  if (!strcmp(name, "sweep_cell")) { *value = h->desc.sweep_bricks ? h->desc.sweep_cell : 0; return INTERPN_HIP_OK; }
  if (!strcmp(name, "dev_pci")) {
    int dom = 0, bus = 0, dv = 0;
    if (hipDeviceGetAttribute(&dom, hipDeviceAttributePciDomainID, h->device) != hipSuccess ||
        hipDeviceGetAttribute(&bus, hipDeviceAttributePciBusId, h->device) != hipSuccess ||
        hipDeviceGetAttribute(&dv, hipDeviceAttributePciDeviceId, h->device) != hipSuccess) {
      (void)hipGetLastError();
      *value = -1;
    } else {
      *value = ((long long)dom << 16) | ((long long)(bus & 0xFF) << 8) | (long long)(dv & 0xFF);
    }
    return INTERPN_HIP_OK;
  }
  if (!strcmp(name, "sweep_layout")) { *value = h->desc.sweep_bricks ? h->desc.sweep_step[0] * 10 + h->desc.sweep_step[1] : 0; return INTERPN_HIP_OK; }
  if (!strcmp(name, "scratch_allocs")) { *value = h->scratch_allocs.load(); return INTERPN_HIP_OK; }
  if (!strcmp(name, "scratch_bytes")) {
    interpn_hip_interp* hm = const_cast<interpn_hip_interp*>(h);
    std::lock_guard<std::mutex> lk(hm->bin_mu);
    long long tot = 0;
    for (const auto& sl : hm->bin_slots) tot += (long long)sl.bytes;
    *value = tot;
    return INTERPN_HIP_OK;
  }
  LaunchConfig c = h->desc.cfg;
  return option_access(c, name, value, false) ? INTERPN_HIP_OK : INTERPN_HIP_ERR_INVALID_ARGUMENT;
}

int interpn_hip_kernel_name(const interpn_hip_interp* h, char* buf, size_t buflen) {
  if (!h || !buf || buflen == 0) return INTERPN_HIP_ERR_INVALID_ARGUMENT;
  const KernelTag t = h->desc.tag;
  if (!t.name) {
    buf[0] = 0;
    return INTERPN_HIP_OK;
  }
  std::string out = std::string("interpn::") + t.name + "<" + (h->desc.dtype == kF64 ? "double" : "float");
  for (int k = 0; k < t.nargs; ++k) {
    out += ", ";
    if (t.bool_mask & (1u << k)) out += t.args[k] ? "true" : "false";
    else out += std::to_string(t.args[k]);
  }
  out += ">";
  snprintf(buf, buflen, "%s", out.c_str());
  return INTERPN_HIP_OK;
}

size_t interpn_hip_table_bytes(const interpn_hip_interp* h, int* step_i, int* step_j) {
  if (!h || !h->desc.bricks) return 0;
// ... 22 lines not shown
```

### interpn_amd/csrc/abi_points.hip

```cpp
#include "abi_internal.h"

using namespace interpn;
using namespace interpn_abi;

namespace {

constexpr size_t kPointsChunk = (size_t)2 << 20;

using Slot = interpn_hip_interp::BinSlot;

size_t split_slice(const GridDesc& g, size_t npoints) {
  const size_t elem = g.dtype == kF64 ? 8 : 4;
  size_t slice = kExpandSliceBytes / ((size_t)g.ndims * elem);
  if (slice < kExpandSliceMin) slice = kExpandSliceMin;
  if (g.cfg.points_slice > 0) slice = (size_t)g.cfg.points_slice < 256 ? 256 : (size_t)g.cfg.points_slice;
  slice &= ~(size_t)255;
  return npoints < slice ? npoints : slice;
}

size_t split_need(const GridDesc& g, size_t npoints) {
  const size_t elem = g.dtype == kF64 ? 8 : 4;
  return 256 + (size_t)g.ndims * align_up(split_slice(g, npoints) * elem, 256);
}

// ... 110 lines not shown

int points_grad_checks(const interpn_hip_interp* h, const void* pts, size_t stride, size_t npoints, const void* out, const void* grad,
                       size_t gstride, bool* nothing, int* path) {
  *nothing = false;
  if (!h) return INTERPN_HIP_ERR_INVALID_ARGUMENT;
  if (h->desc.method != kLinear && h->desc.method != kCubic) return INTERPN_HIP_ERR_UNSUPPORTED;
  if (stride < (size_t)h->desc.ndims || gstride < (size_t)h->desc.ndims) return INTERPN_HIP_ERR_INVALID_ARGUMENT;
  if (npoints == 0) { *nothing = true; return INTERPN_HIP_OK; }
  if (!pts || !out || !grad) return INTERPN_HIP_ERR_INVALID_ARGUMENT;
  if (npoints > (~(size_t)0) / 8 / stride || npoints > (~(size_t)0) / 8 / gstride) return INTERPN_HIP_ERR_INVALID_ARGUMENT;
  *path = choose_grad_path(h->desc, stride, gstride);
  return *path < 0 ? INTERPN_HIP_ERR_UNSUPPORTED : INTERPN_HIP_OK;
}

int split_grad_device(interpn_hip_interp* h, const void* pts, size_t stride, size_t npoints, void* out, void* grad, size_t gstride,
                      hipStream_t stream, unsigned flags) {
  const GridDesc& g = h->desc;
  const size_t elem = g.dtype == kF64 ? 8 : 4;
  void* comp[8] = {nullptr};
  return split_slices(
      h, split_grad_need(g, npoints), pts, stride, npoints, stream, flags,
      [&](void* const* col, unsigned char* rest, size_t pitch, size_t begin, size_t count, hipError_t* err) {
        for (int d = 0; d < g.ndims; ++d) comp[d] = rest + (size_t)d * pitch;
        *err = launch_grad(g, col, static_cast<char*>(out) + begin * elem, comp, count, h->first_bad, stream);
        return (int)INTERPN_HIP_OK;
      },
      [&](unsigned char*, size_t, size_t begin, size_t count) {
        return launch_join_grad(g, comp, static_cast<char*>(grad) + begin * gstride * elem, gstride, count, stream);
      });
}

int points_grad_device(interpn_hip_interp* h, int path, const void* pts, size_t stride, size_t npoints, void* out, void* grad,
                       size_t gstride, hipStream_t stream, unsigned flags) {
  if (path == INTERPN_HIP_POINTS_PATH_SPLIT) {
    const int st = split_grad_device(h, pts, stride, npoints, out, grad, gstride, stream, flags);
    if (st) return st;
  } else {
    if (path == INTERPN_HIP_POINTS_PATH_FUSED)
      HIP_TRY(launch_points_grad(h->desc, pts, stride, out, grad, gstride, npoints, h->first_bad, stream));
    else
      HIP_TRY(launch_grad(h->desc, &pts, out, &grad, npoints, h->first_bad, stream));
    mark_stream(h, stream);
  }
  h->desc.last_binned = 0;
  h->evals_in_place.fetch_add(1);
  h->desc.last_points_path = path;
  return INTERPN_HIP_OK;
}

template <typename Bytes, typename Eval, typename Download>
int host_chunks(interpn_hip_interp* h, const void* pts, size_t point_stride, size_t npoints, Bytes result_bytes, Eval eval,
                Download download) {
  std::lock_guard<std::mutex> host_lock(h->host_mu);
  DeviceGuard guard(h->device);
  if (!guard.ok()) return INTERPN_HIP_ERR_NO_DEVICE;
  interpn_hip_interp::HostLane& l = h->lane[0];
  if (!l.stream) HIP_TRY(pool_take_kit(h->device, &l.stream, &l.flag_host));
  const size_t elem = h->desc.dtype == kF64 ? 8 : 4;
  const size_t nd = (size_t)h->desc.ndims;
  size_t chunk = npoints < kPointsChunk ? npoints : kPointsChunk;
  if (h->desc.cfg.host_chunk >= 1)
    chunk = (size_t)h->desc.cfg.host_chunk < npoints ? (size_t)h->desc.cfg.host_chunk : npoints;
  const size_t cap = ((size_t)256 << 20) / (point_stride * elem);
  if (chunk > cap) chunk = cap ? cap : 1;
  const size_t rows_bytes = align_up(chunk * point_stride * elem, 256);
  void* block = nullptr;
  if (pool_alloc(h->device, &block, rows_bytes + result_bytes(chunk)) != hipSuccess) { (void)hipGetLastError(); return INTERPN_HIP_ERR_OUT_OF_MEMORY; }
  char* results = static_cast<char*>(block) + rows_bytes;
  hipError_t err = hipSuccess;
  int st = INTERPN_HIP_OK;
  for (size_t begin = 0; begin < npoints && err == hipSuccess && st == INTERPN_HIP_OK; begin += chunk) {
    const size_t count = npoints - begin < chunk ? npoints - begin : chunk;
    err = hipMemcpyAsync(block, static_cast<const char*>(pts) + begin * point_stride * elem, ((count - 1) * point_stride + nd) * elem,
                         hipMemcpyHostToDevice, l.stream);
    if (err != hipSuccess) break;
    st = eval(block, results, chunk, count, l.stream);
    if (st) break;
    err = hipMemcpyAsync(l.flag_host, h->first_bad, sizeof(unsigned long long), hipMemcpyDeviceToHost, l.stream);
    if (err == hipSuccess) err = hipStreamSynchronize(l.stream);
    if (err != hipSuccess) break;
    const unsigned long long bad = *l.flag_host;
    size_t good = count;
    if (bad != kNoBadIndexHost) {
      err = hipMemsetAsync(h->first_bad, 0xFF, sizeof(unsigned long long), l.stream);
      good = (size_t)bad;
      st = h->desc.unrep_status;
    }
    if (good && err == hipSuccess) err = download(results, chunk, begin, good, l.stream);
    if (err == hipSuccess) err = hipStreamSynchronize(l.stream);
  }
  (void)hipStreamSynchronize(l.stream);
  pool_free(h->device, block);
  if (err != hipSuccess) return hip_fail(err);
  return st;
}

}

extern "C" {

int interpn_hip_eval_points_device(interpn_hip_interp* h, const void* pts, size_t point_stride, size_t npoints, void* out,
                                   void* stream, unsigned flags, int* path_taken) {
  if (path_taken) *path_taken = INTERPN_HIP_POINTS_PATH_SPLIT;
  if (flags & ~(unsigned)INTERPN_HIP_EVAL_NO_ALLOC) return INTERPN_HIP_ERR_INVALID_ARGUMENT;
  bool nothing = false;
  int path = INTERPN_HIP_POINTS_PATH_SPLIT;
// ... 86 lines not shown
```

### interpn_amd/csrc/abi_sweep.hip

```cpp
#include "abi_internal.h"

using namespace interpn;
using namespace interpn_abi;

namespace interpn {

int sweep_applies(const GridDesc& g, size_t npts) {
  if (g.method == kNearest) return nearest_sweep_applies(g, npts);
  if (g.method == kCubic) return cubic_sweep_applies(g, npts);
  if (g.ndims == 2) return linear2_sweep_applies(g, npts);
  return linear3_sweep_applies(g, npts);
}

hipError_t launch_sweep(const GridDesc& g, const void* const* obs, void* out, size_t npts, unsigned long long* first_bad,
                        void* work, hipStream_t stream) {
  if (!work || npts == 0) return hipErrorInvalidValue;
  if (g.method == kNearest) return launch_nearest_sweep(g, obs, out, npts, first_bad, work, stream);
  if (g.method == kCubic) return launch_cubic_sweep(g, obs, out, npts, first_bad, work, stream);
  if (g.ndims == 2) return launch_linear2_sweep(g, obs, out, npts, first_bad, work, stream);
  return launch_linear3_sweep(g, obs, out, npts, first_bad, work, stream);
}

}

// ... 1 lines not shown

namespace {

struct SampleChoice {
  bool sample = false;
  bool one_pass_only = false;
  unsigned* host_word = nullptr;
  unsigned seq = 0;
};

SampleChoice choose_sample(interpn_hip_interp* h, size_t npoints) {
  const GridDesc& g = h->desc;
  SampleChoice c;
  c.sample = sweep_probe_applies(g) && npoints >= 256u * 64u;
  std::lock_guard<std::mutex> lk(h->bin_mu);
  interpn_hip_interp::SweepSampling& s = h->sampling;
  if (c.sample && g.cfg.sweep_probe == 2) {
    if (!s.host) {
      void* dp = nullptr;
      if (pool_take_pinned_word(h->device, &s.host) == hipSuccess && s.host &&
          hipHostGetDevicePointer(&dp, s.host, 0) == hipSuccess && dp) {
        *(volatile unsigned long long*)s.host = 0;
        s.host_dev = static_cast<unsigned*>(dp);
      } else {
        (void)hipGetLastError();
        s.host_dev = nullptr;
      }
    }
    if (s.host_dev) {
      const unsigned w = (unsigned)*(volatile unsigned long long*)s.host;
      if ((w >> 1) != s.seen && (w >> 1) != 0) {
        s.seen = w >> 1;
        s.streak = (w & 1u) ? 0 : s.streak + 1;
        s.streak_coherent = (w & 1u) ? s.streak_coherent + 1 : 0;
      }
      if ((s.streak >= 3 || s.streak_coherent >= 3) && s.skipped < 15) {
        ++s.skipped;
        c.sample = false;
        c.one_pass_only = s.streak < 3;
      } else {
        s.skipped = 0;
        s.seq = s.seq >= 0x7FFFFFFEu ? 1u : s.seq + 1u;
        c.host_word = s.host_dev;
        c.seq = s.seq;
      }
    }
  }
  s.last_word = nullptr;
  return c;
}

}

int eval_device_sweep(interpn_hip_interp* h, const void* const* obs, void* out, size_t npoints, hipStream_t stream,
                      unsigned flags, int* why) {
  const GridDesc& g = h->desc;
  *why = INTERPN_HIP_WHY_NONE;
  const int applies = sweep_applies(g, npoints);
  if (applies < 2) { *why = applies ? INTERPN_HIP_WHY_SMALL_OR_OFF : INTERPN_HIP_WHY_NONE; return -1; }
  if (reinterpret_cast<uintptr_t>(out) % 16) { *why = INTERPN_HIP_WHY_MISALIGNED; return -1; }
  for (int d = 0; d < g.ndims; ++d)
    if (reinterpret_cast<uintptr_t>(obs[d]) % 16) { *why = INTERPN_HIP_WHY_MISALIGNED; return -1; }
  hipStreamCaptureStatus cs = hipStreamCaptureStatusNone;
  if (hipStreamIsCapturing(stream, &cs) != hipSuccess) { (void)hipGetLastError(); *why = INTERPN_HIP_WHY_CAPTURE; return -1; }
  if (cs != hipStreamCaptureStatusNone) { *why = INTERPN_HIP_WHY_CAPTURE; return -1; }
  const SampleChoice c = choose_sample(h, npoints);
  if (c.one_pass_only) {
    GridDesc gb = g;
    gb.launch_fat = true;
    const hipError_t e1 = launch_any(gb, obs, out, npoints, h->first_bad, stream);
    g.tag = gb.tag;
    if (e1 != hipSuccess) {
      (void)hipGetLastError();
      return hip_fail(e1);
    }
    return INTERPN_HIP_OK;
  }
  interpn_hip_interp::BinSlot* slot = take_bin_slot(h, sweep_work_bytes(), stream, !(flags & INTERPN_HIP_EVAL_NO_ALLOC), why);
  if (!slot) return -1;
  if (c.sample) {
    std::lock_guard<std::mutex> lk(h->bin_mu);
    h->sampling.last_word = static_cast<const unsigned char*>(slot->scratch) + sweep_probe_word_offset();
  }
  hipError_t err = hipSuccess;
  if (!slot->sweep_clean) err = hipMemsetAsync(slot->scratch, 0, sweep_work_bytes(), stream);
  if (c.sample && err == hipSuccess) err = launch_sweep_probe(g, obs, npoints, slot->scratch, stream, c.host_word, c.seq);
  if (err == hipSuccess) {
    if (c.sample) {
      GridDesc gs = g;
      gs.sweep_gated = true;
      err = launch_sweep(gs, obs, out, npoints, h->first_bad, slot->scratch, stream);
      g.tag = gs.tag;
    } else {
      err = launch_sweep(g, obs, out, npoints, h->first_bad, slot->scratch, stream);
    }
  }
  if (c.sample && err == hipSuccess) {
    GridDesc gb = g;
    gb.launch_gate = reinterpret_cast<const unsigned*>(static_cast<const unsigned char*>(slot->scratch) + sweep_probe_word_offset());
    err = launch_any(gb, obs, out, npoints, h->first_bad, stream);
  }
  slot->sweep_clean = err == hipSuccess;
  slot->totals_clean = false;
  release_bin_slot(h, slot, stream, false);
  if (err != hipSuccess) {
    (void)hipGetLastError();
    return hip_fail(err);
  }
  return INTERPN_HIP_OK;
}

}
```

### interpn_amd/csrc/interpn_host.h

```cpp
#pragma once

#include <hip/hip_runtime.h>
#include <stddef.h>

#include <initializer_list>

namespace interpn {

enum Method : int { kLinear = 0, kCubic = 1, kNearest = 2 };
enum OneDimMethod : int { kLinear1D = 16, kLinearHoldLast1D = 17, kLeft1D = 18, kRight1D = 19, kNearest1D = 20 };
inline bool is_one_dim(int method) { return method >= kLinear1D && method <= kNearest1D; }
enum Kind : int { kRegular = 0, kRectilinear = 1 };
enum DType : int { kF64 = 0, kF32 = 1 };

struct LaunchConfig {
  int num_cus = 256;
  int num_xcds = 8;
  long long l2_bytes = 4ll << 20;
  long long lds_per_cu = 160ll << 10;
  long long lds_per_wg = 64ll << 10;
  int blocks_per_cu = 8;
  int iters_per_block = 0;
  int ppl = 0;
  int axis_regs = -1;
// ... 2 lines not shown
  int generic_vec = -1;
  int persistent = 0;
  int axis_lds_kb = -1;
  long long host_chunk = 0;
  int deal = 1;
  int binned = -1;
  int column = -1;
  int column_part = 0;
  int axis_records = 1;
  int stage_timing = 0;
  int bin_scramble = 0;
  int column_threads = 768;
  int column_groups = 1;
  int scatter_staged = 1;
  int column_coef = 1;
  int column_tail = 0x84;
  int column_keys = 1;
  int hist_wgs_per_cu = 4;
  int column_pad = -1;
  int column_cpp = 0;
  long long debug_stamps = 0;
  long long debug_stamps_bytes = 0;
  int bin_slice_log2 = 25;
  int sweep = -1;
  int finish_kernel = 1;
  int gated_iters = 4;
  int sweep_probe = 2;
  int lattice = -1;
  int points_path = 0;
  int points_load = 0;
  int points_store = 0;
  long long points_slice = 0;
  int sweep_period = 0;
};

struct KernelTag {
  const char* name = nullptr;
  int nargs = 0;
  int args[12] = {0};
  unsigned bool_mask = 0;
  void set(const char* nm, std::initializer_list<int> a, unsigned bools) {
    name = nm;
    nargs = 0;
    for (int v : a)
      if (nargs < 12) args[nargs++] = v;
    bool_mask = bools;
  }
};

struct GridDesc {
  const unsigned* launch_gate = nullptr;
  bool sweep_gated = false;
  bool launch_fat = false;
  int method = kLinear;
  int kind = kRegular;
  int dtype = kF64;
  int ndims = 0;
  int linearize = 0;
  int fma = 1;
  int n[8] = {0};
  double start[8] = {0};
  double step[8] = {0};
  const void* vals = nullptr;
  size_t nvals = 0;
  const void* grid[8] = {nullptr};
  size_t grid_total = 0;
  const void* axis_image = nullptr;
  unsigned axis_image_bytes = 0;
  unsigned axis_alloc_bytes = 0;
  unsigned axis_g_off[8] = {0};
  unsigned axis_tab_off[8] = {0};
  int axis_buckets[8] = {0};
  double axis_g0[8] = {0};
  double axis_scale[8] = {0};
  unsigned axis_ltab_off[8] = {0};
  double axis_lscale[8] = {0};
  int axis_lscan[8] = {0};
  unsigned axis_rec_off[8] = {0};
  unsigned axis_rec_base = 0;
  unsigned axis_rec_bytes = 0;
  int axis_rec_compact = 0;
  unsigned axis_recg_off[8] = {0};
  unsigned axis_crec_off[8] = {0};
  unsigned axis_crec_bytes = 0;
  const void* bricks = nullptr;
  int rec1_buckets = 0;
  double rec1_scale = 0.0;
  int brick_step[2] = {2, 2};
  unsigned brick_nb[4] = {0, 0, 0, 0};
  const void* bricks11 = nullptr;
  unsigned bricks11_nb[2] = {0, 0};
  int brick_cell = 0;
  const void* sweep_bricks = nullptr;
  int sweep_step[2] = {0, 0};
  int sweep_cell = 0;
  unsigned sweep_nb[3] = {0, 0, 0};
  size_t sweep_table_bytes = 0;
  double bound_lo[8] = {0};
  double bound_hi[8] = {0};
  int unrep_status = 7;
  double od_start = 0, od_step = 0, od_stop = 0, od_rstep = 0;
  int od_fast = 0;
  int od_M = 0;
  double od_g0 = 0, od_scale = 0;
  size_t od_g_off = 0, od_tab_off = 0, od_table_bytes = 0;
  LaunchConfig cfg;
// ... 12 lines not shown

constexpr unsigned long long kNoBadIndexHost = ~0ull;

constexpr size_t kMaxGridLdsBytes = 20 * 1024;
constexpr size_t kMaxGridLdsBytesWide = 60 * 1024;

struct Thresholds {
  size_t table_l2_sized;
  size_t table_l2_share;
  double table_l2_model;
  size_t binned_table_min;
  size_t binned_points_min;
  size_t bin_table_share;
  size_t axis_lds;
  size_t axis_lds_wide;
  size_t column_lds;
};
inline Thresholds thresholds(const LaunchConfig& c) {
  Thresholds t;
  const size_t l2 = (size_t)c.l2_bytes;
  t.table_l2_sized = l2 + l2 / 2;
  t.table_l2_share = l2 - l2 / 4;
  t.table_l2_model = 0.875 * (double)l2;
  t.binned_table_min = 2 * l2;
  t.binned_points_min = (size_t)2048 * (size_t)c.num_cus;
  t.bin_table_share = l2 / 8;
  t.axis_lds = (size_t)c.lds_per_cu / 8;
  t.axis_lds_wide = (size_t)c.lds_per_wg - 4096;
  t.column_lds = (size_t)c.lds_per_cu;
  return t;
}

int sweep_applies(const GridDesc& g, size_t npts);
hipError_t launch_sweep(const GridDesc& g, const void* const* obs, void* out, size_t npts, unsigned long long* first_bad,
                        void* work, hipStream_t stream);
size_t sweep_work_bytes();
bool sweep_layout(const GridDesc& g, int* si, int* sj, int* cell);
int linear3_sweep_applies(const GridDesc& g, size_t npts);
hipError_t launch_linear3_sweep(const GridDesc& g, const void* const* obs, void* out, size_t npts, unsigned long long* first_bad,
                                void* work, hipStream_t stream);
int linear2_sweep_applies(const GridDesc& g, size_t npts);
hipError_t launch_linear2_sweep(const GridDesc& g, const void* const* obs, void* out, size_t npts, unsigned long long* first_bad,
                                void* work, hipStream_t stream);
int nearest_sweep_applies(const GridDesc& g, size_t npts);
hipError_t launch_nearest_sweep(const GridDesc& g, const void* const* obs, void* out, size_t npts, unsigned long long* first_bad,
                                void* work, hipStream_t stream);
int cubic_sweep_applies(const GridDesc& g, size_t npts);
hipError_t launch_cubic_sweep(const GridDesc& g, const void* const* obs, void* out, size_t npts, unsigned long long* first_bad,
                              void* work, hipStream_t stream);
bool sweep_probe_applies(const GridDesc& g);
hipError_t launch_sweep_probe(const GridDesc& g, const void* const* obs, size_t npts, void* work, hipStream_t stream,
                              unsigned* host_word = nullptr, unsigned seq = 0);
size_t sweep_probe_word_offset();

hipError_t allow_dynamic_lds(const void* kernel, size_t bytes);

template <typename T>
hipError_t launch_linear_regular(const GridDesc& g, const T* const* obs, T* out, size_t npts,
                                 unsigned long long* first_bad, hipStream_t stream);
template <typename T>
hipError_t launch_linear_rectilinear(const GridDesc& g, const T* const* obs, T* out, size_t npts,
                                     unsigned long long* first_bad, hipStream_t stream);
template <typename T>
hipError_t launch_cubic_regular(const GridDesc& g, const T* const* obs, T* out, size_t npts,
                                unsigned long long* first_bad, hipStream_t stream);
template <typename T>
hipError_t launch_cubic_rectilinear(const GridDesc& g, const T* const* obs, T* out, size_t npts,
                                    unsigned long long* first_bad, hipStream_t stream);
template <typename T>
hipError_t launch_nearest(const GridDesc& g, const T* const* obs, T* out, size_t npts,
                          unsigned long long* first_bad, hipStream_t stream);
template <typename T>
hipError_t launch_generic(const GridDesc& g, const T* const* obs, T* out, size_t npts,
                          unsigned long long* first_bad, hipStream_t stream);

void brick_geometry(const GridDesc& g, int si, int sj, unsigned nb[3], size_t* bytes);
void brick_cell_geometry(const GridDesc& g, unsigned nb[4], size_t* bytes);
void brick_j4_geometry(const GridDesc& g, unsigned nb[3], size_t* bytes);
hipError_t build_bricks(const GridDesc& g, void* bricks, hipStream_t stream);
template <typename T>
hipError_t launch_linear_brick(const GridDesc& g, const T* const* obs, T* out, size_t npts,
                               unsigned long long* first_bad, hipStream_t stream);

struct FieldsGeometry {
  int fields_per_line = 0;
  size_t lines_per_point = 0;
  size_t cells = 0;
  size_t table_bytes = 0;
};
bool fields_geometry(size_t elem_size, int ndims, const size_t* dims, size_t nfields, FieldsGeometry* out);
hipError_t build_fields_table(const GridDesc& g, const void* vals, size_t field_stride, int nfields, void* table, hipStream_t stream);
hipError_t launch_linear_fields(const GridDesc& g, const void* table, int nfields, const void* const* obs, void* out,
                                size_t out_stride, size_t npts, unsigned long long* first_bad, hipStream_t stream);
hipError_t launch_linear_fields_grad(const GridDesc& g, const void* table, int nfields, const void* const* obs, void* out,
                                     size_t out_stride, void* grad, size_t grad_stride, size_t npts, unsigned long long* first_bad,
                                     hipStream_t stream);
hipError_t launch_linear_fields_points(const GridDesc& g, const void* table, int nfields, const void* pts, size_t stride, void* out,
                                       size_t out_stride, size_t npts, unsigned long long* first_bad, hipStream_t stream);
hipError_t launch_join_fields(const GridDesc& g, const void* src, size_t pitch, size_t nfields, void* out, size_t out_stride,
                              size_t count, hipStream_t stream);

size_t records1_bytes(const GridDesc& g, int M);
hipError_t build_records1(const GridDesc& g, int M, double scale, void* recs, unsigned* maxpop_dev, hipStream_t stream);
template <typename T>
hipError_t launch_linear1_records(const GridDesc& g, const T* const* obs, T* out, size_t npts, hipStream_t stream);

// ... 97 lines not shown
```

### interpn_amd/csrc/k_cubic_sweep.hip

```cpp
#include "cubic_sweep.h"

namespace interpn {

namespace {

constexpr int kCubicSweepThreads = 768;
template <typename T, bool RECT, int N = 3> constexpr int cubic_sweep_rows() { return N == 2 ? (sizeof(T) == 8 ? 10 : 24) : (sizeof(T) == 8 ? 6 : 16); }
template <typename T, bool RECT, int N = 3> constexpr int cubic_sweep_parked() { return N == 2 ? 4 : (sizeof(T) == 8 ? 2 : 4); }
template <typename T, bool RECT, int N = 3> constexpr int cubic_sweep_threads() { return RECT && sizeof(T) == 8 ? 512 : kCubicSweepThreads; }
constexpr size_t kCubicSweepAxisLds = 16 * 1024;

const void* tiles11(const GridDesc& g, unsigned nb[2]) {
  if (g.bricks && g.brick_step[0] == 1 && g.brick_step[1] == 1) { nb[0] = g.brick_nb[0]; nb[1] = g.brick_nb[1]; return g.bricks; }
  if (g.bricks11) { nb[0] = g.bricks11_nb[0]; nb[1] = g.bricks11_nb[1]; return g.bricks11; }
  return nullptr;
}

size_t cubic_sweep_wave_lds(const GridDesc& g) {
  const unsigned waves = kCubicSweepThreads / 64;
  if (g.ndims == 2)
    return g.dtype == kF64 ? (size_t)CubicSweepLds<double, cubic_sweep_rows<double, false, 2>(), cubic_sweep_parked<double, false, 2>(), 2>::kWave * waves + 16
                           : (size_t)CubicSweepLds<float, cubic_sweep_rows<float, false, 2>(), cubic_sweep_parked<float, false, 2>(), 2>::kWave * waves + 16;
  return g.dtype == kF64 ? (size_t)CubicSweepLds<double, cubic_sweep_rows<double, false, 3>(), cubic_sweep_parked<double, false, 3>(), 3>::kWave * waves + 16
                         : (size_t)CubicSweepLds<float, cubic_sweep_rows<float, false, 3>(), cubic_sweep_parked<float, false, 3>(), 3>::kWave * waves + 16;
}

}

int cubic_sweep_applies(const GridDesc& g, size_t npts) {
  if (g.method != kCubic || (g.ndims != 3 && g.ndims != 2) || g.cfg.sweep == 0 || g.cfg.force_generic) return 0;
  unsigned nb[2];
  if (!tiles11(g, nb)) return 0;
  if ((long long)cubic_sweep_wave_lds(g) > g.cfg.lds_per_cu) return 0;
  if (g.cfg.sweep > 0) return 2;
  if (g.kind == kRectilinear) return 1;
  if (g.ndims == 2) {
    if (g.dtype != kF64) return 1;
    const size_t cus2 = (size_t)(g.cfg.num_cus > 0 ? g.cfg.num_cus : 256);
    return npts >= (size_t)8 * 14 * kCubicSweepThreads * cus2 ? 2 : 1;
  }
  unsigned nbb[2];
  size_t bytes = 0;
  cubic_tile_geometry(g, 1, 1, nbb, &bytes);
  if (bytes <= thresholds(g.cfg).table_l2_sized) return 0;
  if (bytes > (g.dtype == kF64 ? (size_t)128 << 20 : (size_t)32 << 20)) return 0;
  const size_t cus = (size_t)(g.cfg.num_cus > 0 ? g.cfg.num_cus : 256);
  const size_t per_round = (size_t)(g.ndims == 2 ? (g.dtype == kF64 ? 14 : 28) : (g.dtype == kF64 ? 8 : 20)) * kCubicSweepThreads * cus;
  if (npts < (g.dtype == kF64 ? 2 * per_round : per_round + per_round / 2)) return 1;
  return 2;
}

template <typename T, int N, bool RECT, bool FMA, int K = cubic_sweep_rows<T, RECT, N>(), int KL = cubic_sweep_parked<T, RECT, N>(), int TH = cubic_sweep_threads<T, RECT, N>()>
static hipError_t go(const GridDesc& g, CubicSweepArgs<T, N> s, void* work, hipStream_t stream) {
  if (!sweep_schedule(s.r, g, s.r.npts, (size_t)64 * (K + KL), 4000, work)) return hipErrorInvalidValue;
  const unsigned blocks = sweep_blocks(g, s.r.rounds, TH);
  auto kern = k_cubic_sweep<T, RECT, FMA, K, KL, TH, N>;
  const size_t lds = (size_t)CubicSweepLds<T, K, KL, N>::kWave * (TH / 64) + CubicSweepLds<T, K, KL, N>::kWorkgroup + ((RECT && s.c.ax.use_lds) ? (size_t)s.c.ax.image_bytes : 0);
  size_t most = (size_t)CubicSweepLds<T, K, KL, N>::kWave * (TH / 64) + CubicSweepLds<T, K, KL, N>::kWorkgroup + (RECT ? kCubicSweepAxisLds : 0);
  if (g.cfg.lds_per_cu > 0 && most > (size_t)g.cfg.lds_per_cu) most = (size_t)g.cfg.lds_per_cu;
  hipError_t e = allow_dynamic_lds(reinterpret_cast<const void*>(kern), most);
  if (e != hipSuccess) return e;
  if (N == 3) g.tag.set("k_cubic_sweep", {RECT, FMA, K, KL, TH}, 0b00011u);
  else g.tag.set("k_cubic_sweep", {RECT, FMA, K, KL, TH, N}, 0b000011u);
  hipLaunchKernelGGL(kern, dim3(blocks), dim3(TH), lds, stream, s);
  return hipGetLastError();
}

template <typename T, int N>
static hipError_t launch_t(const GridDesc& g, const void* const* obs, void* out, size_t npts, unsigned long long* first_bad,
                           void* work, hipStream_t stream) {
  constexpr int KD = N == 3 ? 2 : 0;
  CubicSweepArgs<T, N> s;
  CubicBrickArgs<T, N>& a = s.c;
  unsigned nb[2];
  a.bricks = static_cast<const T*>(tiles11(g, nb));
  if (!a.bricks) return hipErrorInvalidValue;
  {
    unsigned nbb[2];
    size_t bytes = 0;
    cubic_tile_geometry(g, 1, 1, nbb, &bytes);
    if (bytes >= 0xFFFFF000ull) return hipErrorInvalidValue;
    a.table_bytes = (unsigned)bytes;
  }
  SweepRounds<T, N>& r = s.r;
  a.out = static_cast<T*>(out);
  a.first_bad = first_bad;
  a.npts = npts;
  r.out = a.out;
  r.npts = npts;
  a.scatter = nullptr;
  a.gate = nullptr;
  a.index_base = 0;
  a.eighth = 0;
  a.linearize = g.linearize;
  for (int d = 0; d < N; ++d) {
    a.obs[d] = static_cast<const T*>(obs[d]);
    r.obs[d] = a.obs[d];
    r.absent[d] = g.kind == kRectilinear ? (T)0 : (T)g.start[d];
    a.start[d] = (T)g.start[d];
    a.step[d] = (T)g.step[d];
    a.n[d] = g.n[d];
    a.plane_stride[d] = 0;
  }
  a.nbj = nb[1];
  if constexpr (N == 3) a.plane_stride[2] = nb[0] * nb[1] * 16u;
  step_reciprocals(g, s.rstep, &s.fastdiv);
  a.ax.use_lds = 0;
// ... 25 lines not shown
```

### interpn_amd/csrc/k_linear2_brick.hip

```cpp
#include <type_traits>

#include "lane_axes.h"
#include "linear_cell.h"
#include "sweep_rounds.h"
#include "rect_args.h"

namespace interpn {

template <typename T> struct Brick2Geom {
  static constexpr int KW = 64 / (int)sizeof(T);
  static constexpr int SJ = KW - 1;
  static constexpr int ELEMS = 2 * KW;
};

template <typename T>
struct Brick2Args {
  const T* bricks;
  const T* obs[2];
  T* out;
  unsigned long long* first_bad;
  size_t npts;
  T start[2];
  T step[2];
  int n[2];
// ... 247 lines not shown
  else if (axr == 1) { if (g.fma) GO(true, true, 1); else GO(true, false, 1); }
  else { if (g.fma) GO(true, true, 0); else GO(true, false, 0); }
#undef GO
#undef GO2
  return hipGetLastError();
}

template hipError_t launch_linear2_brick<double>(const GridDesc&, const double* const*, double*, size_t, unsigned long long*, hipStream_t);
template hipError_t launch_linear2_brick<float>(const GridDesc&, const float* const*, float*, size_t, unsigned long long*, hipStream_t);

namespace {
constexpr int kSweep2Threads = 768;
template <typename T> constexpr int sweep2_rows() { return sizeof(T) == 8 ? 16 : 28; }
template <typename T> constexpr int sweep2_parked() { return 4; }
}

int linear2_sweep_applies(const GridDesc& g, size_t npts) {
  if (g.method != kLinear || g.ndims != 2 || g.kind != kRegular || !g.bricks || g.cfg.sweep == 0 || g.cfg.force_generic) return 0;
  unsigned nb[2];
  size_t bytes = 0;
  brick2_geometry(g, nb, &bytes);
  if (bytes >= (1ull << 32) / 2) return 0;
  const size_t lds = (size_t)SweepRoundsLds<double, 2, 16, 4>::kWave * (kSweep2Threads / 64) + SweepRoundsLds<double, 2, 16, 4>::kWorkgroup;
  if ((long long)lds > g.cfg.lds_per_cu) return 0;
  if (g.cfg.sweep > 0) return 2;
  const bool beyond_l2 = bytes > thresholds(g.cfg).table_l2_sized;
  const size_t cus = (size_t)(g.cfg.num_cus > 0 ? g.cfg.num_cus : 256);
  const size_t per_round = (size_t)(g.dtype == kF64 ? 20 : 32) * kSweep2Threads * cus;
  if (npts < (beyond_l2 ? per_round * 5 / 2 : per_round * 6)) return 1;
  return 2;
}

template <typename T>
static hipError_t launch2_t(const GridDesc& g, const void* const* obs, void* out, size_t npts, unsigned long long* first_bad, void* work, hipStream_t stream) {
  constexpr int K = sweep2_rows<T>(), KL = sweep2_parked<T>(), TH = kSweep2Threads;
  Linear2SweepArgs<T> s;
  SweepRounds<T, 2>& r = s.r;
  s.bricks = static_cast<const T*>(g.bricks);
  r.out = static_cast<T*>(out);
  s.first_bad = first_bad;
  r.npts = npts;
  for (int d = 0; d < 2; ++d) {
    r.obs[d] = static_cast<const T*>(obs[d]);
    s.start[d] = (T)g.start[d];
    r.absent[d] = s.start[d];
    s.step[d] = (T)g.step[d];
    s.n[d] = g.n[d];
  }
  step_reciprocals(g, s.rstep, &s.fastdiv);
  s.nbj = g.brick_nb[1];
  sweep_key(g, 0, &r.key_start, &r.key_scale);
  r.key_cells = g.n[0] - 2;
  r.key_shift = sweep_key_shift(r.key_cells);
  if (!sweep_schedule(r, g, npts, (size_t)64 * (K + KL), 2500, work)) return hipErrorInvalidValue;
  const unsigned blocks = sweep_blocks(g, r.rounds, TH);
  const size_t lds = (size_t)SweepRoundsLds<T, 2, K, KL>::kWave * (TH / 64) + SweepRoundsLds<T, 2, K, KL>::kWorkgroup;
  auto launch = [&](auto kern, bool fma) -> hipError_t {
    hipError_t e = allow_dynamic_lds(reinterpret_cast<const void*>(kern), lds);
    if (e != hipSuccess) return e;
    g.tag.set("k_linear2_sweep", {fma, K, KL, TH}, 0b0001u);
    hipLaunchKernelGGL(kern, dim3(blocks), dim3(TH), lds, stream, s);
    return hipGetLastError();
  };
  return g.fma ? launch(k_linear2_sweep<T, true, K, KL, TH>, true) : launch(k_linear2_sweep<T, false, K, KL, TH>, false);
}

hipError_t launch_linear2_sweep(const GridDesc& g, const void* const* obs, void* out, size_t npts, unsigned long long* first_bad, void* work, hipStream_t stream) {
  if (g.ndims != 2 || !g.bricks) return hipErrorInvalidValue;
  if (g.dtype == kF64) return launch2_t<double>(g, obs, out, npts, first_bad, work, stream);
  return launch2_t<float>(g, obs, out, npts, first_bad, work, stream);
}

}
```

### interpn_amd/csrc/k_linear_sweep.hip

```cpp
#include <cstdlib>
#include <cstring>

#include "linear_sweep.h"

namespace interpn {

namespace {

constexpr int kSweepRows = 12;
constexpr int kSweepParked = 4;
#ifndef INTERPN_SWEEP_RECT_PARKED
#define INTERPN_SWEEP_RECT_PARKED 2
#endif
#ifndef INTERPN_SWEEP_RECT_ROWS
#define INTERPN_SWEEP_RECT_ROWS 12
#endif
constexpr int kSweepParkedRect = INTERPN_SWEEP_RECT_PARKED;
#ifndef INTERPN_SWEEP_F32_ROWS
#define INTERPN_SWEEP_F32_ROWS 24
#endif
#ifndef INTERPN_SWEEP_F32_PARKED
#define INTERPN_SWEEP_F32_PARKED 0
#endif
constexpr int kSweepRowsF32 = INTERPN_SWEEP_F32_ROWS;
// ... 115 lines not shown
    id = id * 0x9E3779B1u + (unsigned)(d == N - 1 ? c / p.sk : c);
  }
  const unsigned prev = (unsigned)__shfl_up((int)id, 1);
  const unsigned changes = (unsigned)__builtin_popcountll(__builtin_amdgcn_ballot_w64(lane > 0 && id != prev));
  if (lane == 0) {
    const unsigned r1 = atomicAdd(&p.work->probe_changes, changes);
    asm volatile("" ::"v"(r1));
    if (atomicAdd(&p.work->probe_done, 1u) == rows - 1u) {
      const unsigned total = atomicAdd(&p.work->probe_changes, 0u);
      const unsigned coherent = total * 4u < rows * 63u ? 1u : 0u;
      atomicExch(&p.work->take_brick, coherent);
      if (p.host_word) __hip_atomic_store(p.host_word, (p.seq << 1) | coherent, __ATOMIC_RELAXED, __HIP_MEMORY_SCOPE_SYSTEM);
      atomicExch(&p.work->probe_changes, 0u);
      atomicExch(&p.work->probe_done, 0u);
    }
  }
}

template <typename T, int N>
static hipError_t probe_t(const GridDesc& g, const void* const* obs, size_t npts, void* work, hipStream_t stream, unsigned* host_word, unsigned seq) {
  ProbeArgs<T, N> p;
  p.host_word = host_word;
  p.seq = seq;
  for (int d = 0; d < N; ++d) {
    p.obs[d] = static_cast<const T*>(obs[d]);
    sweep_key(g, d, &p.start[d], &p.scale[d]);
    p.top[d] = g.n[d] - 2;
  }
  const int per_line = (int)(128 / sizeof(T));
  if (g.method == kLinear && N == 3) p.sk = g.dtype == kF64 ? BrickGeom<double, 0>::SK : (g.brick_cell == 2 ? BrickGeom<float, 2>::SK : BrickGeom<float, 0>::SK);
  else if (g.method == kLinear) p.sk = per_line / 2 - 1;
  else if (g.method == kNearest) p.sk = per_line;
  else p.sk = 1;
  p.npts = npts;
  p.work = static_cast<SweepWork*>(work);
  hipLaunchKernelGGL((k_sweep_probe<T, N>), dim3(kProbeRows / 4), dim3(256), 0, stream, p);
  return hipGetLastError();
}

bool sweep_probe_applies(const GridDesc& g) {
  if (g.cfg.sweep == 0 || g.cfg.sweep == 1 || g.cfg.sweep_probe == 0) return false;
  if (g.ndims != 2 && g.ndims != 3) return false;
  if (g.method == kCubic) return g.ndims == 2;
  return g.method == kLinear ? g.bricks != nullptr : g.method == kNearest;
}

hipError_t launch_sweep_probe(const GridDesc& g, const void* const* obs, size_t npts, void* work, hipStream_t stream, unsigned* host_word, unsigned seq) {
  if ((g.ndims != 2 && g.ndims != 3) || !work || npts < (size_t)kProbeRows * 64) return hipErrorInvalidValue;
  if (g.ndims == 3) return g.dtype == kF64 ? probe_t<double, 3>(g, obs, npts, work, stream, host_word, seq) : probe_t<float, 3>(g, obs, npts, work, stream, host_word, seq);
  return g.dtype == kF64 ? probe_t<double, 2>(g, obs, npts, work, stream, host_word, seq) : probe_t<float, 2>(g, obs, npts, work, stream, host_word, seq);
}

size_t sweep_probe_word_offset() { return offsetof(SweepWork, take_brick); }

template <typename T>
static hipError_t launch_t(const GridDesc& g, const void* const* obs, void* out, size_t npts, unsigned long long* first_bad,
                           void* work, hipStream_t stream) {
  SweepArgs<T> s;
  BrickArgs<T, 3>& a = s.b;
  a.gate = nullptr;
  a.bricks = static_cast<const T*>(g.sweep_bricks);
  a.out = static_cast<T*>(out);
  a.first_bad = first_bad;
  a.npts = npts;
  for (int d = 0; d < 3; ++d) {
    a.obs[d] = static_cast<const T*>(obs[d]);
    a.start[d] = (T)g.start[d];
    a.step[d] = (T)g.step[d];
    a.n[d] = g.n[d];
  }
  a.nbj = g.sweep_nb[1];
  a.nbk = g.sweep_nb[2];
  a.lead_stride[0] = 0;
  a.iters = 1;
  a.ax.use_lds = 0;
  a.ax.image = nullptr;
  a.ax.image_bytes = 0;
  int axr = 0;
  if (g.kind == kRectilinear) {
    axr = lane_axes_mode(g);
    if (axr == 0) axr = 4;
    (void)fill_axis_args<T, 3>(g, a.ax, false, axr == 4);
    if (a.ax.use_lds && a.ax.image_bytes > kSweepAxisLds) a.ax.use_lds = 0;
  }
  sweep_key(g, 0, &s.key_start, &s.key_scale);
  s.key_shift = sweep_key_shift(g.n[0] - 2);
  step_reciprocals(g, s.rstep, &s.fastdiv);
  const size_t chunk = (size_t)64 * (g.kind == kRectilinear ? sweep_rows<T, true>() + sweep_parked<T, true>() : sweep_rows<T, false>() + sweep_parked<T, false>());
  if (!sweep_schedule(s, g, npts, chunk, 2600, work)) return hipErrorInvalidValue;
  const unsigned blocks = sweep_blocks(g, s.rounds, kSweepThreads);
#define SWEEP_KIND(RECT_, AXR_) (g.fma ? go_layout<T, RECT_, true, AXR_>(g, s, blocks, stream) : go_layout<T, RECT_, false, AXR_>(g, s, blocks, stream))
  switch (axr) {
    case 0: return SWEEP_KIND(false, 0);
    case 1: return SWEEP_KIND(true, 1);
    case 2: return SWEEP_KIND(true, 2);
    case 3: return SWEEP_KIND(true, 3);
    case 4: return SWEEP_KIND(true, 4);
  }
#undef SWEEP_KIND
  return hipErrorInvalidValue;
}

hipError_t launch_linear3_sweep(const GridDesc& g, const void* const* obs, void* out, size_t npts, unsigned long long* first_bad,
                                void* work, hipStream_t stream) {
  if (g.ndims != 3 || !g.sweep_bricks) return hipErrorInvalidValue;
  if (g.dtype == kF64) return launch_t<double>(g, obs, out, npts, first_bad, work, stream);
  return launch_t<float>(g, obs, out, npts, first_bad, work, stream);
}

}
```

### interpn_amd/csrc/k_nearest.hip

```cpp
#include <type_traits>

#include "lane_axes.h"
#include "sweep_rounds.h"
#include "rect_args.h"

namespace interpn {

template <typename T, int N>
struct NearestArgs {
  const T* vals;
  const T* obs[N];
  T* out;
  unsigned long long* first_bad;
  size_t npts;
  T start[N];
  T step[N];
  int n[N];
  unsigned long long stride[N];
  AxisArgs<T, N> ax;
  const unsigned* gate;
};

template <typename T, int N, bool RECT, bool FMA, bool LDS, int AXR, int PPL>
__device__ __forceinline__ void nearest_body(const NearestArgs<T, N>& a, const unsigned char* lds) {
// ... 192 lines not shown
    case 3: return launch_n<T, 3>(g, obs, out, npts, first_bad, stream);
    case 4: return launch_n<T, 4>(g, obs, out, npts, first_bad, stream);
    case 5: return launch_n<T, 5>(g, obs, out, npts, first_bad, stream);
    case 6: return launch_n<T, 6>(g, obs, out, npts, first_bad, stream);
    default: return hipErrorInvalidValue;
  }
}

template hipError_t launch_nearest<double>(const GridDesc&, const double* const*, double*, size_t, unsigned long long*, hipStream_t);
template hipError_t launch_nearest<float>(const GridDesc&, const float* const*, float*, size_t, unsigned long long*, hipStream_t);

namespace {
constexpr int kNearestSweepThreads = 768;
template <typename T, int N> constexpr int nearest_sweep_rows() { return sizeof(T) == 8 ? (N == 2 ? 16 : 12) : (N == 2 ? 32 : 24); }
template <typename T, int N> constexpr int nearest_sweep_parked() { return sizeof(T) == 8 ? 4 : 0; }
}

int nearest_sweep_applies(const GridDesc& g, size_t npts) {
  if (g.method != kNearest || (g.ndims != 2 && g.ndims != 3) || g.kind != kRegular || g.cfg.sweep == 0 || g.cfg.force_generic) return 0;
  const size_t lds = (size_t)SweepRoundsLds<double, 3, 12, 4>::kWave * (kNearestSweepThreads / 64) + SweepRoundsLds<double, 3, 12, 4>::kWorkgroup;
  if ((long long)lds > g.cfg.lds_per_cu) return 0;
  if (g.cfg.sweep > 0) return 2;
  const size_t cus = (size_t)(g.cfg.num_cus > 0 ? g.cfg.num_cus : 256);
  const size_t rows = g.dtype == kF64 ? (g.ndims == 2 ? 20 : 16) : (g.ndims == 2 ? 32 : 24);
  size_t grid_bytes = g.dtype == kF64 ? 8 : 4;
  for (int d = 0; d < g.ndims; ++d) grid_bytes *= (size_t)g.n[d];
  if (npts < (grid_bytes > thresholds(g.cfg).table_l2_sized ? 4 : 8) * rows * kNearestSweepThreads * cus) return 1;
  return 2;
}

template <typename T, int N>
static hipError_t launch_sweep_n(const GridDesc& g, const void* const* obs, void* out, size_t npts, unsigned long long* first_bad, void* work, hipStream_t stream) {
  constexpr int K = nearest_sweep_rows<T, N>(), KL = nearest_sweep_parked<T, N>(), TH = kNearestSweepThreads;
  NearestSweepArgs<T, N> s;
  SweepRounds<T, N>& r = s.r;
  s.vals = static_cast<const T*>(g.vals);
  r.out = static_cast<T*>(out);
  s.first_bad = first_bad;
  r.npts = npts;
  unsigned long long acc = 1;
  for (int d = N - 1; d >= 0; --d) {
    r.obs[d] = static_cast<const T*>(obs[d]);
    s.start[d] = (T)g.start[d];
    r.absent[d] = s.start[d];
    s.step[d] = (T)g.step[d];
    s.n[d] = g.n[d];
    s.stride[d] = acc;
    acc *= (unsigned long long)g.n[d];
  }
  step_reciprocals(g, s.rstep, &s.fastdiv);
  sweep_key(g, 0, &r.key_start, &r.key_scale);
  r.key_cells = g.n[0] - 2;
  r.key_shift = sweep_key_shift(r.key_cells);
  if (!sweep_schedule(r, g, npts, (size_t)64 * (K + KL), 2000, work)) return hipErrorInvalidValue;
  const unsigned blocks = sweep_blocks(g, r.rounds, TH);
  const size_t lds = (size_t)SweepRoundsLds<T, N, K, KL>::kWave * (TH / 64) + SweepRoundsLds<T, N, K, KL>::kWorkgroup;
  auto launch = [&](auto kern, bool fma) -> hipError_t {
    hipError_t e = allow_dynamic_lds(reinterpret_cast<const void*>(kern), lds);
    if (e != hipSuccess) return e;
    g.tag.set("k_nearest_sweep", {N, fma, K, KL, TH}, 0b00010u);
    hipLaunchKernelGGL(kern, dim3(blocks), dim3(TH), lds, stream, s);
    return hipGetLastError();
  };
  return g.fma ? launch(k_nearest_sweep<T, N, true, K, KL, TH>, true) : launch(k_nearest_sweep<T, N, false, K, KL, TH>, false);
}

hipError_t launch_nearest_sweep(const GridDesc& g, const void* const* obs, void* out, size_t npts, unsigned long long* first_bad, void* work, hipStream_t stream) {
  if (g.ndims == 2) return g.dtype == kF64 ? launch_sweep_n<double, 2>(g, obs, out, npts, first_bad, work, stream) : launch_sweep_n<float, 2>(g, obs, out, npts, first_bad, work, stream);
  if (g.ndims == 3) return g.dtype == kF64 ? launch_sweep_n<double, 3>(g, obs, out, npts, first_bad, work, stream) : launch_sweep_n<float, 3>(g, obs, out, npts, first_bad, work, stream);
  return hipErrorInvalidValue;
}

}
```

### interpn_amd/csrc/linear_sweep.h

```cpp
#pragma once

#include "linear_brick.h"
#include "sweep_rounds.h"

namespace interpn {


template <typename T>
struct SweepArgs {
  BrickArgs<T, 3> b;
  T key_start, key_scale;
  int key_shift;
  T rstep[3];
  unsigned fastdiv;
  unsigned rounds;
  unsigned per_shard;
  unsigned period;
  unsigned period_default;
  unsigned gated;
  SweepWork* work;
  unsigned long long* stamps;
};

template <typename T, int K, int KL = 0>
struct SweepLds {
  static constexpr unsigned kRowOnly = 64u * K * sizeof(T);
  static constexpr unsigned kPiece = 64u * kPieceRow * 2u * sizeof(T);
  static constexpr unsigned kRow = kRowOnly > kPiece ? kRowOnly : kPiece;
  static constexpr unsigned kPark = 64u * KL * 3u * sizeof(T);
  static constexpr unsigned kOff = 64u * 16u;
  static constexpr unsigned kWave = kRow + kPark + kOff;
  static constexpr unsigned kWorkgroup = 16;
  static_assert(kRow + kPark >= 64u * (K + KL) * sizeof(T), "the result exchange spans the row buffer and the parked rows' bytes");
  static_assert(64u * 4u * 2u <= kOff, "the sort's counters live in the piece offsets' bytes");
  static_assert(64u * (K + KL) * 2u <= kRow, "the 16-bit source-index exchange of a round stays inside the row buffer (the parked coordinates sit right behind it)");
};

template <typename T, bool RECT, bool FMA, int SI, int SJ, int K, int THREADS, int AXR = 0, bool STAMPS = false, int CELL = 0, int KL = 0, int ABL = 0>
__global__ void __launch_bounds__(THREADS) k_linear_sweep(const SweepArgs<T> s) {
  constexpr int PPV = 16 / (int)sizeof(T);
  constexpr int KT = K + KL;
  static_assert(KT % PPV == 0 && KT % 2 == 0 && K >= PPV && KT <= 32 && KL >= 0, "rows per wave and round");
  static_assert(CELL == 0 || (CELL == 2 && sizeof(T) == 4 && SI == 1 && SJ == 1), "2 x 4 x 4 bricks: f32");
  static_assert(RECT == (AXR != 0), "rectilinear grids: lane-resident axes only");
  typedef typename LeafVec<T, 2>::type P;
  typedef T TV __attribute__((ext_vector_type(PPV)));
  typedef BrickGeom<T, CELL> Geom;
  constexpr int SK = Geom::SK;
  typedef SweepLds<T, K, KL> L;
  const BrickArgs<T, 3>& a = s.b;
  if (s.gated && __hip_atomic_load(&s.work->take_brick, __ATOMIC_RELAXED, __HIP_MEMORY_SCOPE_AGENT) != 0u) return;
  extern __shared__ __attribute__((aligned(16))) unsigned char smem_raw[];
  const unsigned lane = threadIdx.x & 63u;
  const unsigned wave = threadIdx.x >> 6;
  unsigned char* const mine = smem_raw + wave * L::kWave;
  T* const row = reinterpret_cast<T*>(mine);
  typedef unsigned short __attribute__((may_alias)) lds_u16;
  lds_u16* const row16 = reinterpret_cast<lds_u16*>(mine);
  P* const lds_piece = reinterpret_cast<P*>(mine);
  T* const park = reinterpret_cast<T*>(mine + L::kRow);
  lds_u32* const lds_off = reinterpret_cast<lds_u32*>(mine + L::kRow + L::kPark);
  lds_u32* const cnt = lds_off;
  lds_u32* const wg_words = reinterpret_cast<lds_u32*>(smem_raw + (THREADS / 64) * L::kWave);
  if (threadIdx.x < 4) wg_words[threadIdx.x] = 0;
  if constexpr (RECT && AXR == 4) {
    if (s.b.ax.use_lds) {
      const unsigned words = s.b.ax.image_bytes >> 2;
      const unsigned* src = reinterpret_cast<const unsigned*>(s.b.ax.image);
      unsigned* dst = reinterpret_cast<unsigned*>(smem_raw + (THREADS / 64) * L::kWave + L::kWorkgroup);
      for (unsigned k = threadIdx.x; k < words; k += THREADS) dst[k] = src[k];
    }
  }
  __syncthreads();
  const unsigned q = lane & 3u;
  const unsigned quad = lane >> 2;
  constexpr size_t kChunk = (size_t)64 * KT;
  const unsigned nwaves = gridDim.x * (THREADS / 64);
  LaneAxes<T, 3> la;
  if constexpr (RECT && AXR <= 3) la = load_lane_axes<T, 3, AXR>(a.ax);
  const unsigned char* axis_base = a.ax.image;
  if constexpr (RECT && AXR == 4) {
    if (a.ax.use_lds) {
      axis_base = smem_raw + (THREADS / 64) * L::kWave + L::kWorkgroup;
    }
  }
  SweepWork* const work = s.work;
  unsigned period = s.period;
  if (period == 0) {
    period = __hip_atomic_load(&work->period, __ATOMIC_RELAXED, __HIP_MEMORY_SCOPE_AGENT);
    if (period == 0) period = s.period_default;
  }
  period = __builtin_amdgcn_readfirstlane(period);
  unsigned xcc;
  asm volatile("s_getreg_b32 %0, hwreg(HW_REG_XCC_ID)" : "=s"(xcc));
  unsigned shard = xcc & 7u;
  auto take = [&](unsigned sh) -> unsigned {
    unsigned v = 0;
    if (lane == 0) v = atomicAdd(&work->head[sh][0], 1u);
    return v;
  };
  const unsigned long long t_begin = __builtin_amdgcn_s_memrealtime();
  unsigned long long st_mark = t_begin, st_other = 0, st_rows = 0;
  unsigned st_rot = 0;
  unsigned my_rounds = 0;
  __builtin_amdgcn_s_setprio(2);
  unsigned ticket = take(shard);
  while (true) {
    unsigned rr = __builtin_amdgcn_readfirstlane(ticket);
    if (rr >= s.per_shard || shard * s.per_shard + rr >= s.rounds) {
      bool found = false;
      for (unsigned c = 1; c < 8 && !found; ++c) {
        const unsigned sh = (shard + c) & 7u;
        const unsigned seen = __hip_atomic_load(&work->head[sh][0], __ATOMIC_RELAXED, __HIP_MEMORY_SCOPE_AGENT);
        if (seen < s.per_shard && sh * s.per_shard + seen < s.rounds) { found = true; shard = sh; }
      }
      if (!found) break;
      ticket = take(shard);
      continue;
    }
    const unsigned r = shard * s.per_shard + rr;
    ticket = take(shard);
    ++my_rounds;
    const size_t base = (size_t)r * kChunk;
    T x[KT][3];
    const bool full = base + kChunk <= a.npts;
    if (full) {
#pragma unroll
      for (int d = 0; d < 3; ++d)
#pragma unroll
        for (int kv = 0; kv < KT / PPV; ++kv) {
          TV v;
          if constexpr (ABL == 2) {
#pragma unroll
            for (int h = 0; h < PPV; ++h) v[h] = ablate_coord<T>(base + (size_t)(kv * 64 + (int)lane) * PPV + h, d, a.start[d], a.step[d], a.n[d]);
          } else {
            v = stream_load(reinterpret_cast<const TV*>(a.obs[d] + base) + (kv * 64 + (int)lane));
          }
#pragma unroll
          for (int h = 0; h < PPV; ++h) x[PPV * kv + h][d] = v[h];
        }
    } else {
#pragma unroll
      for (int d = 0; d < 3; ++d)
#pragma unroll
        for (int kv = 0; kv < KT / PPV; ++kv) {
          const size_t i0 = base + (size_t)kv * (64 * PPV) + PPV * lane;
          TV v;
#pragma unroll
          for (int h = 0; h < PPV; ++h) v[h] = a.start[d];
          if (i0 + PPV - 1 < a.npts) {
            v = stream_load(reinterpret_cast<const TV*>(a.obs[d] + i0));
          } else {
#pragma unroll
            for (int h = 0; h < PPV; ++h)
              if (i0 + h < a.npts) v[h] = stream_load(a.obs[d] + i0 + h);
          }
#pragma unroll
          for (int h = 0; h < PPV; ++h) x[PPV * kv + h][d] = v[h];
        }
    }
    cnt[lane] = 0;
    wave_sync();
    unsigned pos[KT];
#pragma unroll
    for (int k = 0; k < KT; ++k) {
      const T u = (x[k][0] - s.key_start) * s.key_scale;
      int c = u >= (T)1 ? (u < (T)(a.n[0] - 2) ? (int)u : a.n[0] - 2) : 0;
      const unsigned bin = (unsigned)(c >> s.key_shift);
      pos[k] = atomicAdd(&cnt[bin], 1u) | (bin << 16);
    }
    wave_sync();
    {
      const unsigned mine_cnt = cnt[lane];
// ... 157 lines not shown
          for (int d = 0; d < 3; ++d) t[d] = av[d] / bv[d];
        }
        if constexpr (!RECT && ABL != 3) {
          if (!have_t) {
#pragma unroll
            for (int d = 0; d < 3; ++d) t[d] = step_cell_quotient(av[d], a.step[d], s.rstep[d]);
          }
        }
        const unsigned kpart = bk * (unsigned)Geom::ELEMS + ((unsigned)loc[2] - bk * (unsigned)SK);
#pragma unroll
        for (int p = 0; p < 4; ++p)
          lds_off[(quad * 4 + p) * 4 + q] = brick_piece<T, SI, SJ, CELL>(a.nbj, a.nbk, loc[0], loc[1], kpart, p >> 1, p & 1);
        wave_sync();
        const uint4 toff = *reinterpret_cast<const uint4*>(&lds_off[(quad * 4 + q) * 4]);
        if constexpr (ABL == 1) {
#pragma unroll
          for (int e = 0; e < 8; ++e) c.v[e >> 2][(e >> 1) & 1][e & 1] = t[e % 3] + (T)(toff.x & 7u) + (T)e;
        } else {
          c = gather_cell<T>(a.bricks, toff, 0u, lds_piece, quad, q);
        }
      }
      T rr2[2];
#pragma unroll
      for (int dk = 0; dk < 2; ++dk) {
        const T c0 = mul_add<FMA>(t[0], c.v[1][0][dk] - c.v[0][0][dk], c.v[0][0][dk]);
        const T c1 = mul_add<FMA>(t[0], c.v[1][1][dk] - c.v[0][1][dk], c.v[0][1][dk]);
        rr2[dk] = mul_add<FMA>(t[1], c1 - c0, c0);
      }
      res[k] = mul_add<FMA>(t[2], rr2[1] - rr2[0], rr2[0]);
      asm volatile("" : "+v"(res[k]));
    }
    if constexpr (STAMPS) { const unsigned long long now = __builtin_amdgcn_s_memrealtime(); st_rows += now - st_mark; st_mark = now; }
    __builtin_amdgcn_s_setprio(2);
#pragma unroll
    for (int k = 0; k < KT; ++k) row[(src[k / 2] >> (16 * (k & 1))) & 0xFFFFu] = res[k];
    wave_sync();
#pragma unroll
    for (int kv = 0; kv < KT / PPV; ++kv) {
      const size_t i0 = base + (size_t)kv * (64 * PPV) + PPV * lane;
      const TV v = *reinterpret_cast<const TV*>(&row[kv * (64 * PPV) + PPV * lane]);
      if constexpr (ABL == 2) {
        if (v[0] == (T)123.456) stream_store(reinterpret_cast<TV*>(a.out + i0), v);
      } else if (full || i0 + PPV - 1 < a.npts) {
        stream_store(reinterpret_cast<TV*>(a.out + i0), v);
      } else {
#pragma unroll
        for (int h = 0; h < PPV; ++h)
          if (i0 + h < a.npts) stream_store(a.out + i0 + h, v[h]);
      }
    }
    wave_sync();
  }
  const unsigned long long t_end = __builtin_amdgcn_s_memrealtime();
  if (lane == 0) {
    const unsigned my_ticks = (unsigned)(t_end - t_begin);
    atomicAdd(&wg_words[0], my_ticks);
    atomicAdd(&wg_words[1], my_rounds);
    __builtin_amdgcn_fence(__ATOMIC_RELEASE, "workgroup");
    if (atomicAdd(&wg_words[2], 1u) == THREADS / 64 - 1) {
      __builtin_amdgcn_fence(__ATOMIC_ACQUIRE, "workgroup");
      const unsigned wg_ticks = wg_words[0], wg_rounds = wg_words[1];
      if (wg_rounds) {
        const unsigned long long r1 = atomicAdd(&work->ticks, (unsigned long long)wg_ticks);
        const unsigned r2 = atomicAdd(&work->rounds, wg_rounds);
        asm volatile("" ::"v"(r1), "v"(r2));
      }
      const unsigned d = atomicAdd(&work->done[0], 1u);
      if (d == gridDim.x - 1) {
        const unsigned long long ticks = atomicAdd(&work->ticks, 0ull);
        const unsigned rounds = atomicAdd(&work->rounds, 0u);
        if (rounds >= 4 * nwaves) {
          unsigned long long p = ticks * 9 / ((unsigned long long)rounds * 10);
          p = p < 200 ? 200 : (p > 20000 ? 20000 : p);
          atomicExch(&work->period, (unsigned)p);
        }
        for (int x = 0; x < 8; ++x) atomicExch(&work->head[x][0], 0u);
        atomicExch(&work->ticks, 0ull);
        atomicExch(&work->rounds, 0u);
        atomicExch(&work->done[0], 0u);
      }
    }
    if constexpr (STAMPS) {
      if (s.stamps) {
        unsigned long long* o = s.stamps + (size_t)(blockIdx.x * (THREADS / 64) + wave) * 8;
        o[0] = t_begin; o[1] = t_end; o[2] = st_other; o[3] = st_rows;
        o[4] = xcc & 0xFu; o[5] = st_rot / 64u; o[6] = my_rounds; o[7] = period;
      }
    }
  }
}

}
```

### interpn_amd/csrc/scratch_slots.h

```cpp
#pragma once
#include <atomic>
#include <cstddef>
#include <mutex>
#include <vector>

#include "../../include/interpn_hip.h"

namespace scratch_slots {

template <class RT>
struct Slot {
  void* scratch = nullptr;
  size_t bytes = 0;
  typename RT::Event event{};
  bool recorded = false;
  bool unmarked = false;
  bool busy = false;
  typename RT::Stream last_stream{};
  unsigned long long stamp = 0;
  bool totals_clean = false;
  bool sweep_clean = false;
  typename RT::Event stage[5] = {};
  bool staged = false;
};

template <class RT>
struct Table {
  using Runtime = RT;
  using BinSlot = Slot<RT>;
  static constexpr size_t kMaxBinSlots = 4;
  static constexpr size_t kMaxMarks = 16;
  RT rt;
  std::mutex bin_mu;
  std::vector<BinSlot> bin_slots;
  unsigned long long bin_uses = 0;
  std::atomic<long long> scratch_allocs{0};
  const void** word_in_block = nullptr;
  std::mutex marks_mu;
  std::vector<typename RT::Stream> marks;
  bool sync_device_at_destroy = false;
  Table() { bin_slots.reserve(kMaxBinSlots); }
};

template <class T>
bool settle_slot(T& t, typename T::BinSlot& sl) {
  if (!sl.unmarked) return true;
  bool capturing = false;
  int e = t.rt.is_capturing(sl.last_stream, &capturing);
  if (e == 0 && capturing) return false;
  if (e == 0) e = t.rt.event_record(sl.event, sl.last_stream);
  sl.unmarked = false;
  sl.recorded = e == 0;
  if (e != 0) {
    t.rt.clear_last_error();
    if (t.rt.device_synchronize() != 0) t.rt.clear_last_error();
    std::lock_guard<std::mutex> lk(t.marks_mu);
    t.sync_device_at_destroy = true;
  }
  return true;
}

template <class T>
typename T::BinSlot* take_bin_slot(T& t, size_t need, typename T::Runtime::Stream stream, bool may_alloc, int* why) {
  using BinSlot = typename T::BinSlot;
  std::unique_lock<std::mutex> lk(t.bin_mu);
  BinSlot* pick = nullptr;
  bool wait = false;
  for (auto& sl : t.bin_slots) {
    if (sl.busy || sl.bytes < need || !(sl.recorded || sl.unmarked)) continue;
    if (sl.last_stream == stream) { pick = &sl; break; }
  }
  if (!pick)
    for (auto& sl : t.bin_slots) {
      if (sl.busy || sl.bytes < need || !settle_slot(t, sl)) continue;
// ... 193 lines not shown
```

### interpn_amd/csrc/sweep_rounds.h

```cpp
#pragma once

#include <type_traits>

#include "interpn_device.h"
#include "interpn_host.h"

namespace interpn {

struct SweepWork {
  unsigned head[8][32];
  unsigned done[32];
  unsigned long long ticks;
  unsigned rounds;
  unsigned period;
  unsigned probe_changes, probe_done, take_brick;
  unsigned pad[25];
};
static_assert(sizeof(SweepWork) == 10 * 128, "one line per counter");


template <int FROM, int TO, typename F>
__device__ __forceinline__ void sweep_static_for(F&& f) {
  if constexpr (FROM < TO) {
    f(std::integral_constant<int, FROM>{});
    sweep_static_for<FROM + 1, TO>(f);
  }
}

template <typename T, int N>
struct SweepRounds {
  const T* obs[N];
  T* out;
  size_t npts;
  T absent[N];
  T key_start, key_scale;
  int key_cells;
  int key_shift;
  unsigned rounds;
  unsigned per_shard;
  unsigned period;
  unsigned period_default;
  unsigned gated;
  SweepWork* work;
  T fake_start[N], fake_step[N];
  int fake_n[N];
  unsigned long long* stamps;
};

template <typename T, int N, int K, int KL, unsigned MIN_ROW_BYTES = 0, unsigned CNT_BYTES = 64u * 4u * 2u>
struct SweepRoundsLds {
  static constexpr unsigned kRowOnly = 64u * K * sizeof(T);
  static constexpr unsigned kRow = kRowOnly > MIN_ROW_BYTES ? kRowOnly : MIN_ROW_BYTES;
  static constexpr unsigned kPark = 64u * KL * (unsigned)N * sizeof(T);
  static constexpr unsigned kCnt = CNT_BYTES;
  static_assert(CNT_BYTES >= 64u * 4u * 2u, "64 counters + 64 first positions");
  static constexpr unsigned kWave = kRow + kPark + kCnt;
  static constexpr unsigned kWorkgroup = 16;
  static_assert(kRow + kPark >= 64u * (K + KL) * sizeof(T), "the result exchange spans the row buffer and the parked rows' bytes");
  static_assert(64u * (K + KL) * 2u <= kRow, "the 16-bit source-index exchange of a round stays inside the row buffer (the parked coordinates sit right behind it)");
};

template <typename T, int N, int K, int KL, int THREADS, int KEYDIM, typename L, int ABL = 0, bool STAMPS = false, int OPAQUE_LANE = 0, typename RowFn>
__device__ __forceinline__ void sweep_rounds(const SweepRounds<T, N>& sr, unsigned char* smem_raw, RowFn&& row_fn) {
  if (sr.gated && __hip_atomic_load(&sr.work->take_brick, __ATOMIC_RELAXED, __HIP_MEMORY_SCOPE_AGENT) != 0u) return;
  constexpr int PPV = 16 / (int)sizeof(T);
  constexpr int KT = K + KL;
  static_assert(KT % PPV == 0 && KT % 2 == 0 && K >= PPV && KT <= 32, "rows per wave and round");
  typedef T TV __attribute__((ext_vector_type(PPV)));
  const unsigned lane = threadIdx.x & 63u;
  const unsigned wave = threadIdx.x >> 6;
  unsigned char* const mine = smem_raw + wave * L::kWave;
  T* const row = reinterpret_cast<T*>(mine);
  typedef unsigned short __attribute__((may_alias)) lds_u16;
  lds_u16* const row16 = reinterpret_cast<lds_u16*>(mine);
  T* const park = reinterpret_cast<T*>(mine + L::kRow);
  lds_u32* const cnt = reinterpret_cast<lds_u32*>(mine + L::kRow + L::kPark);
  lds_u32* const wg_words = reinterpret_cast<lds_u32*>(smem_raw + (THREADS / 64) * L::kWave);
  if (threadIdx.x < 4) wg_words[threadIdx.x] = 0;
  __syncthreads();
  constexpr size_t kChunk = (size_t)64 * KT;
  const unsigned nwaves = gridDim.x * (THREADS / 64);
  SweepWork* const work = sr.work;
  unsigned period = sr.period;
  if (period == 0) {
    period = __hip_atomic_load(&work->period, __ATOMIC_RELAXED, __HIP_MEMORY_SCOPE_AGENT);
    if (period == 0) period = sr.period_default;
  }
  period = __builtin_amdgcn_readfirstlane(period);
  unsigned xcc;
  asm volatile("s_getreg_b32 %0, hwreg(HW_REG_XCC_ID)" : "=s"(xcc));
  unsigned shard = xcc & 7u;
  auto take = [&](unsigned sh) -> unsigned {
    unsigned v = 0;
    if (lane == 0) v = atomicAdd(&work->head[sh][0], 1u);
    return v;
  };
  const unsigned long long t_begin = __builtin_amdgcn_s_memrealtime();
  unsigned long long st_mark = t_begin, st_other = 0, st_rows = 0;
  unsigned st_rot = 0;
  unsigned my_rounds = 0;
  __builtin_amdgcn_s_setprio(2);
  unsigned ticket = take(shard);
  while (true) {
    unsigned rr = __builtin_amdgcn_readfirstlane(ticket);
    if (rr >= sr.per_shard || shard * sr.per_shard + rr >= sr.rounds) {
      bool found = false;
      for (unsigned c = 1; c < 8 && !found; ++c) {
        const unsigned sh = (shard + c) & 7u;
        const unsigned seen = __hip_atomic_load(&work->head[sh][0], __ATOMIC_RELAXED, __HIP_MEMORY_SCOPE_AGENT);
        if (seen < sr.per_shard && sh * sr.per_shard + seen < sr.rounds) { found = true; shard = sh; }
      }
      if (!found) break;
      ticket = take(shard);
      continue;
    }
    const unsigned r = shard * sr.per_shard + rr;
    ticket = take(shard);
    ++my_rounds;
    unsigned ln = lane;
    if constexpr (OPAQUE_LANE == 1) asm volatile("" : "+v"(ln));
    unsigned ln2 = ln;
    if constexpr (OPAQUE_LANE == 2) asm volatile("" : "+v"(ln2));
    const size_t base = (size_t)r * kChunk;
    T x[KT][N];
    const bool full = base + kChunk <= sr.npts;
    if (full) {
#pragma unroll
      for (int d = 0; d < N; ++d)
#pragma unroll
        for (int kv = 0; kv < KT / PPV; ++kv) {
          TV v;
          if constexpr (ABL == 2) {
#pragma unroll
            for (int h = 0; h < PPV; ++h) v[h] = ablate_coord<T>(base + (size_t)(kv * 64 + (int)ln) * PPV + h, d, sr.fake_start[d], sr.fake_step[d], sr.fake_n[d]);
          } else {
            v = stream_load(reinterpret_cast<const TV*>(sr.obs[d] + base) + (kv * 64 + (int)ln));
          }
#pragma unroll
          for (int h = 0; h < PPV; ++h) x[PPV * kv + h][d] = v[h];
        }
    } else {
#pragma unroll
      for (int d = 0; d < N; ++d)
#pragma unroll
        for (int kv = 0; kv < KT / PPV; ++kv) {
          const size_t i0 = base + (size_t)kv * (64 * PPV) + PPV * ln;
          TV v;
#pragma unroll
          for (int h = 0; h < PPV; ++h) v[h] = sr.absent[d];
          if (i0 + PPV - 1 < sr.npts) {
            v = stream_load(reinterpret_cast<const TV*>(sr.obs[d] + i0));
          } else {
#pragma unroll
            for (int h = 0; h < PPV; ++h)
              if (i0 + h < sr.npts) v[h] = stream_load(sr.obs[d] + i0 + h);
          }
#pragma unroll
          for (int h = 0; h < PPV; ++h) x[PPV * kv + h][d] = v[h];
        }
    }
    cnt[ln] = 0;
    wave_sync();
    unsigned pos[KT];
#pragma unroll
    for (int k = 0; k < KT; ++k) {
      const T u = (x[k][KEYDIM] - sr.key_start) * sr.key_scale;
      int c = u >= (T)1 ? (u < (T)sr.key_cells ? (int)u : sr.key_cells) : 0;
      const unsigned bin = (unsigned)(c >> sr.key_shift);
      pos[k] = atomicAdd(&cnt[bin], 1u) | (bin << 16);
// ... 28 lines not shown
#pragma unroll
      for (int k = 0; k < KT; ++k) {
        unsigned at = pos[k];
        if constexpr (KL > 0) at += pos[k] >= 64u * K ? kParkSkip + (unsigned)d * (64u * KL) : 0u;
        row[at] = x[k][d];
      }
      wave_sync();
#pragma unroll
      for (int k = 0; k < K; ++k) x[k][d] = row[k * 64 + ln];
      wave_sync();
    }
    unsigned src[KT / 2];
#pragma unroll
    for (int k = 0; k < KT; ++k) row16[pos[k]] = (unsigned short)((k / PPV) * (64 * PPV) + PPV * ln2 + (k % PPV));
    wave_sync();
#pragma unroll
    for (int k2 = 0; k2 < KT / 2; ++k2) src[k2] = (unsigned)row16[(2 * k2) * 64 + ln] | ((unsigned)row16[(2 * k2 + 1) * 64 + ln] << 16);
    wave_sync();
    if constexpr (STAMPS) { const unsigned long long now = __builtin_amdgcn_s_memrealtime(); st_other += now - st_mark; st_mark = now; st_rot = rot; }
    __builtin_amdgcn_s_setprio(0);
    T res[KT];
    sweep_static_for<0, KT>([&](auto kc) {
      constexpr int k = decltype(kc)::value;
      __builtin_amdgcn_sched_barrier(0);
      T xr[N];
#pragma unroll
      for (int d = 0; d < N; ++d) xr[d] = k < K ? x[k < K ? k : 0][d] : park[(d * KL + (k - K)) * 64 + ln];
      const size_t gi = base + ((src[k / 2] >> (16 * (k & 1))) & 0xFFFFu);
      res[k] = row_fn(kc, xr, gi);
      asm volatile("" : "+v"(res[k]));
    });
    if constexpr (STAMPS) { const unsigned long long now = __builtin_amdgcn_s_memrealtime(); st_rows += now - st_mark; st_mark = now; }
    __builtin_amdgcn_s_setprio(2);
#pragma unroll
    for (int k = 0; k < KT; ++k) row[(src[k / 2] >> (16 * (k & 1))) & 0xFFFFu] = res[k];
    wave_sync();
#pragma unroll
    for (int kv = 0; kv < KT / PPV; ++kv) {
      const size_t i0 = base + (size_t)kv * (64 * PPV) + PPV * ln;
      const TV v = *reinterpret_cast<const TV*>(&row[kv * (64 * PPV) + PPV * ln]);
      if constexpr (ABL == 2) {
        if (v[0] == (T)123.456) stream_store(reinterpret_cast<TV*>(sr.out + i0), v);
      } else if (full || i0 + PPV - 1 < sr.npts) {
        stream_store(reinterpret_cast<TV*>(sr.out + i0), v);
      } else {
#pragma unroll
        for (int h = 0; h < PPV; ++h)
          if (i0 + h < sr.npts) stream_store(sr.out + i0 + h, v[h]);
      }
    }
    wave_sync();
  }
  const unsigned long long t_end = __builtin_amdgcn_s_memrealtime();
  if (lane == 0) {
    const unsigned my_ticks = (unsigned)(t_end - t_begin);
    atomicAdd(&wg_words[0], my_ticks);
    atomicAdd(&wg_words[1], my_rounds);
    __builtin_amdgcn_fence(__ATOMIC_RELEASE, "workgroup");
    if (atomicAdd(&wg_words[2], 1u) == THREADS / 64 - 1) {
      __builtin_amdgcn_fence(__ATOMIC_ACQUIRE, "workgroup");
      const unsigned wg_ticks = wg_words[0], wg_rounds = wg_words[1];
      if (wg_rounds) {
        const unsigned long long r1 = atomicAdd(&work->ticks, (unsigned long long)wg_ticks);
        const unsigned r2 = atomicAdd(&work->rounds, wg_rounds);
        asm volatile("" ::"v"(r1), "v"(r2));
      }
      const unsigned d = atomicAdd(&work->done[0], 1u);
      if (d == gridDim.x - 1) {
        const unsigned long long ticks = atomicAdd(&work->ticks, 0ull);
        const unsigned rounds = atomicAdd(&work->rounds, 0u);
        if (rounds >= 4 * nwaves) {
          unsigned long long p = ticks * 9 / ((unsigned long long)rounds * 10);
          p = p < 200 ? 200 : (p > 40000 ? 40000 : p);
          atomicExch(&work->period, (unsigned)p);
        }
        for (int xx = 0; xx < 8; ++xx) atomicExch(&work->head[xx][0], 0u);
        atomicExch(&work->ticks, 0ull);
        atomicExch(&work->rounds, 0u);
        atomicExch(&work->done[0], 0u);
      }
    }
    if constexpr (STAMPS) {
      if (sr.stamps) {
        unsigned long long* o = sr.stamps + (size_t)(blockIdx.x * (THREADS / 64) + wave) * 8;
        o[0] = t_begin; o[1] = t_end; o[2] = st_other; o[3] = st_rows;
        o[4] = xcc & 0xFu; o[5] = st_rot / 64u; o[6] = my_rounds; o[7] = period;
      }
    }
  }
}


template <typename T>
inline void sweep_key(const GridDesc& g, int dim, T* start, T* scale) {
  if (g.kind == kRectilinear) {
    const double span = g.bound_hi[dim] - g.bound_lo[dim];
    *start = (T)g.bound_lo[dim];
    *scale = span > 0 ? (T)((double)(g.n[dim] - 1) / span) : (T)0;
  } else {
    *start = (T)g.start[dim];
    *scale = (T)(1.0 / g.step[dim]);
  }
  if (!(*scale > 0) || !(*scale < (T)1e30)) *scale = 0;
}

inline int sweep_key_shift(int cells) {
  int shift = 0;
  while ((cells >> shift) >= 64) ++shift;
  return shift;
}

template <typename T, int N>
inline void step_reciprocals(const GridDesc& g, T (&rstep)[N], unsigned* fastdiv) {
  *fastdiv = g.kind == kRectilinear ? 0u : 1u;
  for (int d = 0; d < N; ++d) {
    const T st = (T)g.step[d];
    const volatile T one = (T)1;
    rstep[d] = g.kind == kRectilinear ? (T)0 : one / st;
    const double mag = st < 0 ? -(double)st : (double)st;
    if (!(mag >= StepCellRange<T>::lo && mag <= StepCellRange<T>::hi)) *fastdiv = 0;
  }
}

template <typename A>
inline bool sweep_schedule(A& s, const GridDesc& g, size_t npts, size_t round_points, unsigned period_default, void* work) {
  const size_t rounds = (npts + round_points - 1) / round_points;
  if (rounds > 0xFFFFFFF0ull) return false;
  s.rounds = (unsigned)rounds;
  s.per_shard = (s.rounds + 7u) / 8u;
  s.period = g.cfg.sweep_period > 0 ? (unsigned)g.cfg.sweep_period : 0u;
  s.period_default = period_default;
  s.gated = g.sweep_gated ? 1u : 0u;
  s.work = static_cast<SweepWork*>(work);
  s.stamps = nullptr;
  return true;
}

inline unsigned sweep_blocks(const GridDesc& g, unsigned rounds, int threads) {
  const unsigned cus = (unsigned)(g.cfg.num_cus > 0 ? g.cfg.num_cus : 256);
  const unsigned need = (rounds + (unsigned)(threads / 64) - 1) / (unsigned)(threads / 64);
  return cus < need ? cus : need;
}

}
```

Before: 109,300.

## Double-buffer sweep work counters and publish status word directly to pinned host memory

```diff
diff --git a/interpn_amd/csrc/abi_binned.hip b/interpn_amd/csrc/abi_binned.hip
--- a/interpn_amd/csrc/abi_binned.hip
+++ b/interpn_amd/csrc/abi_binned.hip
@@ -193,9 +193,10 @@
     return st;
   }
   bool swept = false;
+  int published_slot = -1;
   if (st < 0 && sweep_applies(h->desc, npoints)) {
     int why_sweep = INTERPN_HIP_WHY_NONE;
-    const int ss = eval_device_sweep(h, obs, out, npoints, static_cast<hipStream_t>(stream), flags, &why_sweep);
+    const int ss = eval_device_sweep(h, obs, out, npoints, static_cast<hipStream_t>(stream), flags, &why_sweep, &published_slot);
     if (why_out && (why == INTERPN_HIP_WHY_NONE || why_sweep > INTERPN_HIP_WHY_SMALL_OR_OFF)) *why_out = why_sweep;
     if (ss > 0) {
       std::lock_guard<std::mutex> lk(h->marks_mu);
@@ -222,6 +223,7 @@
     h->evals_binned.fetch_add(1);
   }
   mark_stream(h, static_cast<hipStream_t>(stream));
+  if (swept && published_slot >= 0) note_published(h, published_slot, static_cast<hipStream_t>(stream));
   return INTERPN_HIP_OK;
 }
 
diff --git a/interpn_amd/csrc/abi_create.hip b/interpn_amd/csrc/abi_create.hip
--- a/interpn_amd/csrc/abi_create.hip
+++ b/interpn_amd/csrc/abi_create.hip
@@ -550,6 +550,7 @@
   });
   pool_free(h->device, h->first_bad);
   pool_return_pinned_word(h->device, h->finish_word);
+  for (auto& p : h->published) pool_return_pinned_word(h->device, p.word);
   pool_return_pinned_word(h->device, h->sampling.host);
   pool_free(h->device, h->grids_owned);
   pool_free(h->device, h->bricks_owned);
diff --git a/interpn_amd/csrc/abi_fields.hip b/interpn_amd/csrc/abi_fields.hip
--- a/interpn_amd/csrc/abi_fields.hip
+++ b/interpn_amd/csrc/abi_fields.hip
@@ -375,6 +375,7 @@
   size_t chunk = opt_chunk >= 1 ? (size_t)opt_chunk : ((size_t)2 << 20);
   if (chunk > nout) chunk = nout;
   std::lock_guard<std::mutex> host_lock(s->host_mu);
+  for (interpn_hip_interp* sh : s->sub) unpublish_all(sh);
   if (!s->stream) HIP_TRY(pool_take_kit(s->device, &s->stream, &s->kit_word));
   if (s->host_points < chunk) {
     HIP_TRY(hipStreamSynchronize(s->stream));
@@ -455,6 +456,7 @@
   const size_t cap = ((size_t)256 << 20) / (widest * elem);
   if (chunk > cap) chunk = cap ? cap : 1;
   std::lock_guard<std::mutex> host_lock(s->host_mu);
+  for (interpn_hip_interp* sh : s->sub) unpublish_all(sh);
   if (!s->stream) HIP_TRY(pool_take_kit(s->device, &s->stream, &s->kit_word));
   const size_t rows_bytes = align_up(chunk * point_stride * elem, 256);
   void* block = nullptr;
diff --git a/interpn_amd/csrc/abi_fields_grad.hip b/interpn_amd/csrc/abi_fields_grad.hip
--- a/interpn_amd/csrc/abi_fields_grad.hip
+++ b/interpn_amd/csrc/abi_fields_grad.hip
@@ -88,6 +88,7 @@
   size_t chunk = opt_chunk >= 1 ? (size_t)opt_chunk : ((size_t)2 << 20);
   if (chunk > nout) chunk = nout;
   std::lock_guard<std::mutex> host_lock(s->host_mu);
+  for (interpn_hip_interp* sh : s->sub) unpublish_all(sh);
   if (!s->stream) HIP_TRY(pool_take_kit(s->device, &s->stream, &s->kit_word));
   if (s->host_points < chunk) {
     HIP_TRY(hipStreamSynchronize(s->stream));
diff --git a/interpn_amd/csrc/abi_fields_lattice.hip b/interpn_amd/csrc/abi_fields_lattice.hip
--- a/interpn_amd/csrc/abi_fields_lattice.hip
+++ b/interpn_amd/csrc/abi_fields_lattice.hip
@@ -202,6 +202,7 @@
   DeviceGuard guard(s->device);
   if (!guard.ok()) return INTERPN_HIP_ERR_NO_DEVICE;
   std::lock_guard<std::mutex> host_lock(s->host_mu);
+  for (interpn_hip_interp* sh : s->sub) unpublish_all(sh);
   if (!s->stream) HIP_TRY(pool_take_kit(s->device, &s->stream, &s->kit_word));
   const size_t elem = s->dtype == kF64 ? 8 : 4;
   const size_t k = s->nfields;
diff --git a/interpn_amd/csrc/abi_grad.hip b/interpn_amd/csrc/abi_grad.hip
--- a/interpn_amd/csrc/abi_grad.hip
+++ b/interpn_amd/csrc/abi_grad.hip
@@ -62,6 +62,7 @@
   const int st0 = grad_checks(h, method, obs, obs_lens, true, nobs, out, grad, nout, &nothing);
   if (st0 || nothing) return st0;
   std::lock_guard<std::mutex> host_lock(h->host_mu);
+  unpublish_all(h);
   DeviceGuard guard(h->device);
   if (!guard.ok()) return INTERPN_HIP_ERR_NO_DEVICE;
   const size_t elem = h->desc.dtype == kF64 ? 8 : 4;
diff --git a/interpn_amd/csrc/abi_host.hip b/interpn_amd/csrc/abi_host.hip
--- a/interpn_amd/csrc/abi_host.hip
+++ b/interpn_amd/csrc/abi_host.hip
@@ -156,6 +156,7 @@
                           size_t* bad_index) {
   (void)nobs;
   std::lock_guard<std::mutex> host_lock(h->host_mu);
+  unpublish_all(h);
   DeviceGuard guard(h->device);
   if (!guard.ok()) return INTERPN_HIP_ERR_NO_DEVICE;
   if (nout <= kSmallPoints && h->desc.cfg.host_chunk < 1) {
@@ -226,7 +227,9 @@
   const bool by_kernel = h->finish_word_dev && h->desc.cfg.finish_kernel != 0 && count <= kMaxStatusWords && asked == hipSuccess &&
                          cs == hipStreamCaptureStatusNone;
   if (!by_kernel && count > 1) return -1;
-  if (by_kernel) {
+  const unsigned long long* const landed = by_kernel && count == 1 && words[0] == h->first_bad ? published_on(h, s) : nullptr;
+  if (landed) {
+  } else if (by_kernel) {
     StatusWords w;
     for (int k = 0; k < kMaxStatusWords; ++k) w.word[k] = words[k < count ? k : 0];
     w.count = count;
@@ -236,8 +239,10 @@
     HIP_TRY(hipMemcpyAsync(h->finish_word, words[0], sizeof(unsigned long long), hipMemcpyDeviceToHost, s));
   }
   HIP_TRY(hipStreamSynchronize(s));
-  const unsigned long long word = *(volatile unsigned long long*)h->finish_word;
+  const unsigned long long word = *(volatile const unsigned long long*)(landed ? landed : h->finish_word);
   if (word == kNoBadIndexHost) return INTERPN_HIP_OK;
+  for (int k = 0; k < count; ++k)
+    if (words[k] == h->first_bad) unpublish_all(h);
   for (int k = 0; k < count; ++k) HIP_TRY(hipMemsetAsync(words[k], 0xFF, sizeof(word), s));
   HIP_TRY(hipStreamSynchronize(s));
   if (first_bad_index) *first_bad_index = (uint64_t)word;
diff --git a/interpn_amd/csrc/abi_internal.h b/interpn_amd/csrc/abi_internal.h
--- a/interpn_amd/csrc/abi_internal.h
+++ b/interpn_amd/csrc/abi_internal.h
@@ -147,6 +147,13 @@
     word_in_block = &sampling.last_word;
   }
   std::atomic<long long> evals_binned{0}, evals_in_place{0}, evals_sweep{0};
+  struct Published {
+    unsigned long long* word = nullptr;
+    unsigned long long* word_dev = nullptr;
+    hipStream_t stream = nullptr;
+    bool valid = false;
+  } published[kMaxBinSlots];
+  std::mutex publish_mu;
   struct SweepSampling {
     unsigned long long* host = nullptr;
     unsigned* host_dev = nullptr;
@@ -335,8 +342,12 @@
 hipError_t launch_grad(const GridDesc& g, const void* const* obs, void* out, void* const* grad, size_t npts,
                        unsigned long long* first_bad, hipStream_t stream);
 
+void note_published(interpn_hip_interp* h, int slot_index, hipStream_t stream);
+void unpublish(interpn_hip_interp* h, hipStream_t stream);
+void unpublish_all(interpn_hip_interp* h);
+const unsigned long long* published_on(interpn_hip_interp* h, hipStream_t stream);
 int eval_device_sweep(interpn_hip_interp* h, const void* const* obs, void* out, size_t npoints, hipStream_t stream,
-                      unsigned flags, int* why);
+                      unsigned flags, int* why, int* published_slot);
 
 int ensure_lane(interpn_hip_interp* h, int which, size_t points);
 int eval_host_impl(interpn_hip_interp* h, const void* const* obs, size_t nobs, void* out, size_t nout, size_t* bad_index);
diff --git a/interpn_amd/csrc/abi_lattice.hip b/interpn_amd/csrc/abi_lattice.hip
--- a/interpn_amd/csrc/abi_lattice.hip
+++ b/interpn_amd/csrc/abi_lattice.hip
@@ -235,6 +235,7 @@
   int st = validate_lattice(h, axes, axis_lens, naxes, out, &s, &empty);
   if (st || empty) return st;
   std::lock_guard<std::mutex> host_lock(h->host_mu);
+  unpublish_all(h);
   DeviceGuard guard(h->device);
   if (!guard.ok()) return INTERPN_HIP_ERR_NO_DEVICE;
   interpn_hip_interp::HostLane& l = h->lane[0];
diff --git a/interpn_amd/csrc/abi_lattice_grad.hip b/interpn_amd/csrc/abi_lattice_grad.hip
--- a/interpn_amd/csrc/abi_lattice_grad.hip
+++ b/interpn_amd/csrc/abi_lattice_grad.hip
@@ -124,6 +124,7 @@
   int st = checks(h, axes, axis_lens, naxes, out, grad, &s, &empty);
   if (st || empty) return st;
   std::lock_guard<std::mutex> host_lock(h->host_mu);
+  unpublish_all(h);
   DeviceGuard guard(h->device);
   if (!guard.ok()) return INTERPN_HIP_ERR_NO_DEVICE;
   interpn_hip_interp::HostLane& l = h->lane[0];
diff --git a/interpn_amd/csrc/abi_launch.hip b/interpn_amd/csrc/abi_launch.hip
--- a/interpn_amd/csrc/abi_launch.hip
+++ b/interpn_amd/csrc/abi_launch.hip
@@ -52,6 +52,9 @@
   return launch<float>(g, reinterpret_cast<const float* const*>(obs), static_cast<float*>(out), npts, first_bad, stream);
 }
 
-void mark_stream(interpn_hip_interp* h, hipStream_t stream) { scratch_slots::mark_stream(*h, stream); }
+void mark_stream(interpn_hip_interp* h, hipStream_t stream) {
+  unpublish(h, stream);
+  scratch_slots::mark_stream(*h, stream);
+}
 
 }
diff --git a/interpn_amd/csrc/abi_options.hip b/interpn_amd/csrc/abi_options.hip
--- a/interpn_amd/csrc/abi_options.hip
+++ b/interpn_amd/csrc/abi_options.hip
@@ -187,6 +187,26 @@
     }
     return INTERPN_HIP_OK;
   }
+  if (!strcmp(name, "sweep_period_measured")) {
+    interpn_hip_interp* hm = const_cast<interpn_hip_interp*>(h);
+    std::lock_guard<std::mutex> lk(hm->bin_mu);
+    const interpn_hip_interp::BinSlot* best = nullptr;
+    for (const auto& sl : hm->bin_slots)
+      if (!sl.busy && sl.sweep_clean && sl.scratch && sl.bytes >= sweep_work_bytes() && (!best || sl.stamp > best->stamp)) best = &sl;
+    *value = 0;
+    if (best) {
+      DeviceGuard guard(h->device);
+      if (!guard.ok()) return INTERPN_HIP_ERR_NO_DEVICE;
+      unsigned w[2] = {0, 0};
+      if (hipDeviceSynchronize() != hipSuccess ||
+          hipMemcpy(w, static_cast<const unsigned char*>(best->scratch) + sweep_period_words_offset(), sizeof(w), hipMemcpyDeviceToHost) != hipSuccess) {
+        (void)hipGetLastError();
+        return INTERPN_HIP_ERR_INVALID_ARGUMENT;
+      }
+      *value = w[0] > w[1] ? w[0] : w[1];
+    }
+    return INTERPN_HIP_OK;
+  }
   if (!strcmp(name, "sweep_probe_streak")) {
     interpn_hip_interp* hm = const_cast<interpn_hip_interp*>(h);
     std::lock_guard<std::mutex> lk(hm->bin_mu);
diff --git a/interpn_amd/csrc/abi_points.hip b/interpn_amd/csrc/abi_points.hip
--- a/interpn_amd/csrc/abi_points.hip
+++ b/interpn_amd/csrc/abi_points.hip
@@ -186,6 +186,7 @@
 int host_chunks(interpn_hip_interp* h, const void* pts, size_t point_stride, size_t npoints, Bytes result_bytes, Eval eval,
                 Download download) {
   std::lock_guard<std::mutex> host_lock(h->host_mu);
+  unpublish_all(h);
   DeviceGuard guard(h->device);
   if (!guard.ok()) return INTERPN_HIP_ERR_NO_DEVICE;
   interpn_hip_interp::HostLane& l = h->lane[0];
diff --git a/interpn_amd/csrc/abi_sweep.hip b/interpn_amd/csrc/abi_sweep.hip
--- a/interpn_amd/csrc/abi_sweep.hip
+++ b/interpn_amd/csrc/abi_sweep.hip
@@ -77,10 +77,51 @@
 
 }
 
+static unsigned long long* landing_word(interpn_hip_interp* h, int slot_index) {
+  std::lock_guard<std::mutex> lk(h->publish_mu);
+  interpn_hip_interp::Published& p = h->published[slot_index];
+  p.valid = false;
+  if (!p.word) {
+    if (pool_take_pinned_word(h->device, &p.word) != hipSuccess || !p.word) { (void)hipGetLastError(); p.word = nullptr; return nullptr; }
+    *(volatile unsigned long long*)p.word = kNoBadIndexHost;
+    void* dp = nullptr;
+    if (hipHostGetDevicePointer(&dp, p.word, 0) == hipSuccess) p.word_dev = static_cast<unsigned long long*>(dp);
+    else (void)hipGetLastError();
+  }
+  return p.word_dev;
+}
+
+void note_published(interpn_hip_interp* h, int slot_index, hipStream_t stream) {
+  std::lock_guard<std::mutex> lk(h->publish_mu);
+  for (auto& p : h->published)
+    if (p.stream == stream) p.valid = false;
+  h->published[slot_index].stream = stream;
+  h->published[slot_index].valid = true;
+}
+
+void unpublish(interpn_hip_interp* h, hipStream_t stream) {
+  std::lock_guard<std::mutex> lk(h->publish_mu);
+  for (auto& p : h->published)
+    if (p.stream == stream) p.valid = false;
+}
+
+void unpublish_all(interpn_hip_interp* h) {
+  std::lock_guard<std::mutex> lk(h->publish_mu);
+  for (auto& p : h->published) p.valid = false;
+}
+
+const unsigned long long* published_on(interpn_hip_interp* h, hipStream_t stream) {
+  std::lock_guard<std::mutex> lk(h->publish_mu);
+  for (const auto& p : h->published)
+    if (p.valid && p.stream == stream) return p.word;
+  return nullptr;
+}
+
 int eval_device_sweep(interpn_hip_interp* h, const void* const* obs, void* out, size_t npoints, hipStream_t stream,
-                      unsigned flags, int* why) {
+                      unsigned flags, int* why, int* published_slot) {
   const GridDesc& g = h->desc;
   *why = INTERPN_HIP_WHY_NONE;
+  *published_slot = -1;
   const int applies = sweep_applies(g, npoints);
   if (applies < 2) { *why = applies ? INTERPN_HIP_WHY_SMALL_OR_OFF : INTERPN_HIP_WHY_NONE; return -1; }
   if (reinterpret_cast<uintptr_t>(out) % 16) { *why = INTERPN_HIP_WHY_MISALIGNED; return -1; }
@@ -108,16 +149,23 @@
     h->sampling.last_word = static_cast<const unsigned char*>(slot->scratch) + sweep_probe_word_offset();
   }
   hipError_t err = hipSuccess;
-  if (!slot->sweep_clean) err = hipMemsetAsync(slot->scratch, 0, sweep_work_bytes(), stream);
+  if (!slot->sweep_clean) {
+    err = hipMemsetAsync(slot->scratch, 0, sweep_work_bytes(), stream);
+    slot->sweep_set = 0;
+  }
   if (c.sample && err == hipSuccess) err = launch_sweep_probe(g, obs, npoints, slot->scratch, stream, c.host_word, c.seq);
+  const int slot_index = (int)(slot - h->bin_slots.data());
+  unsigned long long* const landing = !c.sample && g.cfg.finish_kernel != 0 ? landing_word(h, slot_index) : nullptr;
   if (err == hipSuccess) {
-    if (c.sample) {
-      GridDesc gs = g;
-      gs.sweep_gated = true;
-      err = launch_sweep(gs, obs, out, npoints, h->first_bad, slot->scratch, stream);
-      g.tag = gs.tag;
-    } else {
-      err = launch_sweep(g, obs, out, npoints, h->first_bad, slot->scratch, stream);
+    GridDesc gs = g;
+    gs.sweep_gated = c.sample;
+    gs.sweep_set = slot->sweep_set;
+    gs.sweep_publish = landing;
+    err = launch_sweep(gs, obs, out, npoints, h->first_bad, slot->scratch, stream);
+    g.tag = gs.tag;
+    if (err == hipSuccess) {
+      slot->sweep_set ^= 1u;
+      if (landing) *published_slot = slot_index;
     }
   }
   if (c.sample && err == hipSuccess) {
diff --git a/interpn_amd/csrc/interpn_host.h b/interpn_amd/csrc/interpn_host.h
--- a/interpn_amd/csrc/interpn_host.h
+++ b/interpn_amd/csrc/interpn_host.h
@@ -78,6 +78,8 @@
   const unsigned* launch_gate = nullptr;
   bool sweep_gated = false;
   bool launch_fat = false;
+  unsigned sweep_set = 0;
+  unsigned long long* sweep_publish = nullptr;
   int method = kLinear;
   int kind = kRegular;
   int dtype = kF64;
@@ -196,6 +198,7 @@
 hipError_t launch_sweep_probe(const GridDesc& g, const void* const* obs, size_t npts, void* work, hipStream_t stream,
                               unsigned* host_word = nullptr, unsigned seq = 0);
 size_t sweep_probe_word_offset();
+size_t sweep_period_words_offset();
 
 hipError_t allow_dynamic_lds(const void* kernel, size_t bytes);
 
diff --git a/interpn_amd/csrc/k_cubic_sweep.hip b/interpn_amd/csrc/k_cubic_sweep.hip
--- a/interpn_amd/csrc/k_cubic_sweep.hip
+++ b/interpn_amd/csrc/k_cubic_sweep.hip
@@ -52,7 +52,7 @@
 
 template <typename T, int N, bool RECT, bool FMA, int K = cubic_sweep_rows<T, RECT, N>(), int KL = cubic_sweep_parked<T, RECT, N>(), int TH = cubic_sweep_threads<T, RECT, N>()>
 static hipError_t go(const GridDesc& g, CubicSweepArgs<T, N> s, void* work, hipStream_t stream) {
-  if (!sweep_schedule(s.r, g, s.r.npts, (size_t)64 * (K + KL), 4000, work)) return hipErrorInvalidValue;
+  if (!sweep_schedule(s.r, g, s.r.npts, (size_t)64 * (K + KL), 4000, work, s.c.first_bad)) return hipErrorInvalidValue;
   const unsigned blocks = sweep_blocks(g, s.r.rounds, TH);
   auto kern = k_cubic_sweep<T, RECT, FMA, K, KL, TH, N>;
   const size_t lds = (size_t)CubicSweepLds<T, K, KL, N>::kWave * (TH / 64) + CubicSweepLds<T, K, KL, N>::kWorkgroup + ((RECT && s.c.ax.use_lds) ? (size_t)s.c.ax.image_bytes : 0);
diff --git a/interpn_amd/csrc/k_linear2_brick.hip b/interpn_amd/csrc/k_linear2_brick.hip
--- a/interpn_amd/csrc/k_linear2_brick.hip
+++ b/interpn_amd/csrc/k_linear2_brick.hip
@@ -323,7 +323,7 @@
   sweep_key(g, 0, &r.key_start, &r.key_scale);
   r.key_cells = g.n[0] - 2;
   r.key_shift = sweep_key_shift(r.key_cells);
-  if (!sweep_schedule(r, g, npts, (size_t)64 * (K + KL), 2500, work)) return hipErrorInvalidValue;
+  if (!sweep_schedule(r, g, npts, (size_t)64 * (K + KL), 2500, work, first_bad)) return hipErrorInvalidValue;
   const unsigned blocks = sweep_blocks(g, r.rounds, TH);
   const size_t lds = (size_t)SweepRoundsLds<T, 2, K, KL>::kWave * (TH / 64) + SweepRoundsLds<T, 2, K, KL>::kWorkgroup;
   auto launch = [&](auto kern, bool fma) -> hipError_t {
diff --git a/interpn_amd/csrc/k_linear_sweep.hip b/interpn_amd/csrc/k_linear_sweep.hip
--- a/interpn_amd/csrc/k_linear_sweep.hip
+++ b/interpn_amd/csrc/k_linear_sweep.hip
@@ -191,6 +191,7 @@
 }
 
 size_t sweep_probe_word_offset() { return offsetof(SweepWork, take_brick); }
+size_t sweep_period_words_offset() { return offsetof(SweepWork, period); }
 
 template <typename T>
 static hipError_t launch_t(const GridDesc& g, const void* const* obs, void* out, size_t npts, unsigned long long* first_bad,
@@ -226,7 +227,7 @@
   s.key_shift = sweep_key_shift(g.n[0] - 2);
   step_reciprocals(g, s.rstep, &s.fastdiv);
   const size_t chunk = (size_t)64 * (g.kind == kRectilinear ? sweep_rows<T, true>() + sweep_parked<T, true>() : sweep_rows<T, false>() + sweep_parked<T, false>());
-  if (!sweep_schedule(s, g, npts, chunk, 2600, work)) return hipErrorInvalidValue;
+  if (!sweep_schedule(s, g, npts, chunk, 2600, work, first_bad)) return hipErrorInvalidValue;
   const unsigned blocks = sweep_blocks(g, s.rounds, kSweepThreads);
 #define SWEEP_KIND(RECT_, AXR_) (g.fma ? go_layout<T, RECT_, true, AXR_>(g, s, blocks, stream) : go_layout<T, RECT_, false, AXR_>(g, s, blocks, stream))
   switch (axr) {
diff --git a/interpn_amd/csrc/k_nearest.hip b/interpn_amd/csrc/k_nearest.hip
--- a/interpn_amd/csrc/k_nearest.hip
+++ b/interpn_amd/csrc/k_nearest.hip
@@ -268,7 +268,7 @@
   sweep_key(g, 0, &r.key_start, &r.key_scale);
   r.key_cells = g.n[0] - 2;
   r.key_shift = sweep_key_shift(r.key_cells);
-  if (!sweep_schedule(r, g, npts, (size_t)64 * (K + KL), 2000, work)) return hipErrorInvalidValue;
+  if (!sweep_schedule(r, g, npts, (size_t)64 * (K + KL), 2000, work, first_bad)) return hipErrorInvalidValue;
   const unsigned blocks = sweep_blocks(g, r.rounds, TH);
   const size_t lds = (size_t)SweepRoundsLds<T, N, K, KL>::kWave * (TH / 64) + SweepRoundsLds<T, N, K, KL>::kWorkgroup;
   auto launch = [&](auto kern, bool fma) -> hipError_t {
diff --git a/interpn_amd/csrc/linear_sweep.h b/interpn_amd/csrc/linear_sweep.h
--- a/interpn_amd/csrc/linear_sweep.h
+++ b/interpn_amd/csrc/linear_sweep.h
@@ -18,7 +18,10 @@
   unsigned period;
   unsigned period_default;
   unsigned gated;
+  unsigned set;
   SweepWork* work;
+  const unsigned long long* status;
+  unsigned long long* publish;
   unsigned long long* stamps;
 };
 
@@ -49,7 +52,11 @@
   constexpr int SK = Geom::SK;
   typedef SweepLds<T, K, KL> L;
   const BrickArgs<T, 3>& a = s.b;
-  if (s.gated && __hip_atomic_load(&s.work->take_brick, __ATOMIC_RELAXED, __HIP_MEMORY_SCOPE_AGENT) != 0u) return;
+  constexpr unsigned kMaxPeriod = 20000;
+  if (s.gated && __hip_atomic_load(&s.work->take_brick, __ATOMIC_RELAXED, __HIP_MEMORY_SCOPE_AGENT) != 0u) {
+    if (blockIdx.x == 0 && threadIdx.x == 0) sweep_turn_sets(s.work, s.set, false, 0u, 0u, kMaxPeriod);
+    return;
+  }
   extern __shared__ __attribute__((aligned(16))) unsigned char smem_raw[];
   const unsigned lane = threadIdx.x & 63u;
   const unsigned wave = threadIdx.x >> 6;
@@ -85,18 +92,14 @@
     }
   }
   SweepWork* const work = s.work;
-  unsigned period = s.period;
-  if (period == 0) {
-    period = __hip_atomic_load(&work->period, __ATOMIC_RELAXED, __HIP_MEMORY_SCOPE_AGENT);
-    if (period == 0) period = s.period_default;
-  }
-  period = __builtin_amdgcn_readfirstlane(period);
+  SweepSet& mine_set = work->set[s.set & 1u];
+  const unsigned period = sweep_period_in(work, s.set, s.period, s.period_default);
   unsigned xcc;
   asm volatile("s_getreg_b32 %0, hwreg(HW_REG_XCC_ID)" : "=s"(xcc));
   unsigned shard = xcc & 7u;
   auto take = [&](unsigned sh) -> unsigned {
     unsigned v = 0;
-    if (lane == 0) v = atomicAdd(&work->head[sh][0], 1u);
+    if (lane == 0) v = atomicAdd(&mine_set.head[sh][0], 1u);
     return v;
   };
   const unsigned long long t_begin = __builtin_amdgcn_s_memrealtime();
@@ -105,20 +108,21 @@
   unsigned my_rounds = 0;
   __builtin_amdgcn_s_setprio(2);
   unsigned ticket = take(shard);
+  if (blockIdx.x == 0 && threadIdx.x == 0) sweep_turn_sets(work, s.set, true, s.rounds, nwaves, kMaxPeriod);
   while (true) {
-    unsigned rr = __builtin_amdgcn_readfirstlane(ticket);
-    if (rr >= s.per_shard || shard * s.per_shard + rr >= s.rounds) {
+    const unsigned tk = __builtin_amdgcn_readfirstlane(ticket);
+    const unsigned r = sweep_round_of(shard, tk, s.per_shard, s.rounds);
+    if (r == kSweepNoRound) {
       bool found = false;
       for (unsigned c = 1; c < 8 && !found; ++c) {
         const unsigned sh = (shard + c) & 7u;
-        const unsigned seen = __hip_atomic_load(&work->head[sh][0], __ATOMIC_RELAXED, __HIP_MEMORY_SCOPE_AGENT);
-        if (seen < s.per_shard && sh * s.per_shard + seen < s.rounds) { found = true; shard = sh; }
+        const unsigned seen = __hip_atomic_load(&mine_set.head[sh][0], __ATOMIC_RELAXED, __HIP_MEMORY_SCOPE_AGENT);
+        if (sweep_round_of(sh, seen, s.per_shard, s.rounds) != kSweepNoRound) { found = true; shard = sh; }
       }
       if (!found) break;
       ticket = take(shard);
       continue;
     }
-    const unsigned r = shard * s.per_shard + rr;
     ticket = take(shard);
     ++my_rounds;
     const size_t base = (size_t)r * kChunk;
@@ -382,6 +386,8 @@
     wave_sync();
   }
   const unsigned long long t_end = __builtin_amdgcn_s_memrealtime();
+  unsigned long long* const publish = sweep_late_argument<unsigned long long*>(offsetof(SweepArgs<T>, publish));
+  sweep_wave_settle(publish);
   if (lane == 0) {
     const unsigned my_ticks = (unsigned)(t_end - t_begin);
     atomicAdd(&wg_words[0], my_ticks);
@@ -389,26 +395,7 @@
     __builtin_amdgcn_fence(__ATOMIC_RELEASE, "workgroup");
     if (atomicAdd(&wg_words[2], 1u) == THREADS / 64 - 1) {
       __builtin_amdgcn_fence(__ATOMIC_ACQUIRE, "workgroup");
-      const unsigned wg_ticks = wg_words[0], wg_rounds = wg_words[1];
-      if (wg_rounds) {
-        const unsigned long long r1 = atomicAdd(&work->ticks, (unsigned long long)wg_ticks);
-        const unsigned r2 = atomicAdd(&work->rounds, wg_rounds);
-        asm volatile("" ::"v"(r1), "v"(r2));
-      }
-      const unsigned d = atomicAdd(&work->done[0], 1u);
-      if (d == gridDim.x - 1) {
-        const unsigned long long ticks = atomicAdd(&work->ticks, 0ull);
-        const unsigned rounds = atomicAdd(&work->rounds, 0u);
-        if (rounds >= 4 * nwaves) {
-          unsigned long long p = ticks * 9 / ((unsigned long long)rounds * 10);
-          p = p < 200 ? 200 : (p > 20000 ? 20000 : p);
-          atomicExch(&work->period, (unsigned)p);
-        }
-        for (int x = 0; x < 8; ++x) atomicExch(&work->head[x][0], 0u);
-        atomicExch(&work->ticks, 0ull);
-        atomicExch(&work->rounds, 0u);
-        atomicExch(&work->done[0], 0u);
-      }
+      sweep_workgroup_done(mine_set, wg_words[1] ? wg_words[0] : 0u, a.first_bad, publish);
     }
     if constexpr (STAMPS) {
       if (s.stamps) {
diff --git a/interpn_amd/csrc/scratch_slots.h b/interpn_amd/csrc/scratch_slots.h
--- a/interpn_amd/csrc/scratch_slots.h
+++ b/interpn_amd/csrc/scratch_slots.h
@@ -20,6 +20,7 @@
   unsigned long long stamp = 0;
   bool totals_clean = false;
   bool sweep_clean = false;
+  unsigned sweep_set = 0;
   typename RT::Event stage[5] = {};
   bool staged = false;
 };
diff --git a/interpn_amd/csrc/sweep_deal.h b/interpn_amd/csrc/sweep_deal.h
--- /dev/null
+++ b/interpn_amd/csrc/sweep_deal.h
@@ -0,0 +1,26 @@
+#pragma once
+
+#if defined(__HIPCC__) || defined(__CUDACC__)
+#define SWEEP_DEAL_FN __host__ __device__ inline
+#else
+#define SWEEP_DEAL_FN inline
+#endif
+
+namespace interpn {
+
+constexpr unsigned kSweepNoRound = ~0u;
+
+SWEEP_DEAL_FN unsigned sweep_round_of(unsigned shard, unsigned index, unsigned per_shard, unsigned rounds) {
+  if (index >= per_shard) return kSweepNoRound;
+  const unsigned r = shard * per_shard + index;
+  return r < rounds ? r : kSweepNoRound;
+}
+
+SWEEP_DEAL_FN unsigned sweep_next_period(unsigned long long ticks, unsigned rounds, unsigned kept, unsigned max_ticks) {
+  if (rounds == 0) return kept;
+  unsigned long long p = ticks * 9ull / ((unsigned long long)rounds * 10ull);
+  p = p < 200ull ? 200ull : (p > (unsigned long long)max_ticks ? (unsigned long long)max_ticks : p);
+  return (unsigned)p;
+}
+
+}
diff --git a/interpn_amd/csrc/sweep_rounds.h b/interpn_amd/csrc/sweep_rounds.h
--- a/interpn_amd/csrc/sweep_rounds.h
+++ b/interpn_amd/csrc/sweep_rounds.h
@@ -4,19 +4,67 @@
 
 #include "interpn_device.h"
 #include "interpn_host.h"
+#include "sweep_deal.h"
 
 namespace interpn {
 
-struct SweepWork {
+struct SweepSet {
   unsigned head[8][32];
   unsigned done[32];
   unsigned long long ticks;
   unsigned rounds;
-  unsigned period;
+  unsigned pad[29];
+};
+struct SweepWork {
+  SweepSet set[2];
+  unsigned period[2];
   unsigned probe_changes, probe_done, take_brick;
-  unsigned pad[25];
+  unsigned pad[27];
 };
-static_assert(sizeof(SweepWork) == 10 * 128, "one line per counter");
+static_assert(sizeof(SweepSet) == 10 * 128 && sizeof(SweepWork) == 21 * 128, "one line per counter");
+
+#if defined(__HIPCC__)
+__device__ __forceinline__ unsigned sweep_period_in(const SweepWork* work, unsigned set, unsigned forced, unsigned dflt) {
+  if (forced != 0) return forced;
+  const unsigned p = work->period[set & 1u];
+  return p != 0 ? p : dflt;
+}
+
+__device__ __forceinline__ void sweep_turn_sets(SweepWork* work, unsigned set, bool counting, unsigned rounds, unsigned nwaves, unsigned max_ticks) {
+  SweepSet& other = work->set[(set & 1u) ^ 1u];
+  const unsigned long long ticks = __hip_atomic_load(&other.ticks, __ATOMIC_RELAXED, __HIP_MEMORY_SCOPE_AGENT);
+  const unsigned orounds = __hip_atomic_load(&other.rounds, __ATOMIC_RELAXED, __HIP_MEMORY_SCOPE_AGENT);
+  const unsigned kept = __hip_atomic_load(&work->period[set & 1u], __ATOMIC_RELAXED, __HIP_MEMORY_SCOPE_AGENT);
+  __hip_atomic_store(&work->period[(set & 1u) ^ 1u], sweep_next_period(ticks, orounds, kept, max_ticks), __ATOMIC_RELAXED, __HIP_MEMORY_SCOPE_AGENT);
+  for (int x = 0; x < 8; ++x) __hip_atomic_store(&other.head[x][0], 0u, __ATOMIC_RELAXED, __HIP_MEMORY_SCOPE_AGENT);
+  __hip_atomic_store(&other.done[0], 0u, __ATOMIC_RELAXED, __HIP_MEMORY_SCOPE_AGENT);
+  __hip_atomic_store(&other.ticks, 0ull, __ATOMIC_RELAXED, __HIP_MEMORY_SCOPE_AGENT);
+  __hip_atomic_store(&other.rounds, 0u, __ATOMIC_RELAXED, __HIP_MEMORY_SCOPE_AGENT);
+  if (counting) __hip_atomic_store(&work->set[set & 1u].rounds, rounds >= 4u * nwaves ? rounds : 0u, __ATOMIC_RELAXED, __HIP_MEMORY_SCOPE_AGENT);
+}
+
+__device__ __forceinline__ void sweep_workgroup_done(SweepSet& mine, unsigned wg_ticks, const unsigned long long* status, unsigned long long* publish) {
+  if (wg_ticks) (void)atomicAdd(&mine.ticks, (unsigned long long)wg_ticks);
+  if (publish) {
+    const unsigned d = atomicAdd(&mine.done[0], 1u);
+    if (d == gridDim.x - 1) {
+      const unsigned long long v = __hip_atomic_load(status, __ATOMIC_RELAXED, __HIP_MEMORY_SCOPE_AGENT);
+      __hip_atomic_store(publish, v, __ATOMIC_RELAXED, __HIP_MEMORY_SCOPE_SYSTEM);
+    }
+  }
+}
+
+template <typename P>
+__device__ __forceinline__ P sweep_late_argument(size_t offset) {
+  typedef const unsigned char __attribute__((address_space(4))) kernarg_byte;
+  kernarg_byte* base = (kernarg_byte*)__builtin_amdgcn_kernarg_segment_ptr();
+  return *(const P __attribute__((address_space(4)))*)(base + offset);
+}
+
+__device__ __forceinline__ void sweep_wave_settle(const void* publish) {
+  if (publish) asm volatile("s_waitcnt vmcnt(0)" ::: "memory");
+}
+#endif
 
 
 template <int FROM, int TO, typename F>
@@ -41,7 +89,10 @@
   unsigned period;
   unsigned period_default;
   unsigned gated;
+  unsigned set;
   SweepWork* work;
+  const unsigned long long* status;
+  unsigned long long* publish;
   T fake_start[N], fake_step[N];
   int fake_n[N];
   unsigned long long* stamps;
@@ -62,7 +113,11 @@
 
 template <typename T, int N, int K, int KL, int THREADS, int KEYDIM, typename L, int ABL = 0, bool STAMPS = false, int OPAQUE_LANE = 0, typename RowFn>
 __device__ __forceinline__ void sweep_rounds(const SweepRounds<T, N>& sr, unsigned char* smem_raw, RowFn&& row_fn) {
-  if (sr.gated && __hip_atomic_load(&sr.work->take_brick, __ATOMIC_RELAXED, __HIP_MEMORY_SCOPE_AGENT) != 0u) return;
+  constexpr unsigned kMaxPeriod = 40000;
+  if (sr.gated && __hip_atomic_load(&sr.work->take_brick, __ATOMIC_RELAXED, __HIP_MEMORY_SCOPE_AGENT) != 0u) {
+    if (blockIdx.x == 0 && threadIdx.x == 0) sweep_turn_sets(sr.work, sr.set, false, 0u, 0u, kMaxPeriod);
+    return;
+  }
   constexpr int PPV = 16 / (int)sizeof(T);
   constexpr int KT = K + KL;
   static_assert(KT % PPV == 0 && KT % 2 == 0 && K >= PPV && KT <= 32, "rows per wave and round");
@@ -81,18 +136,14 @@
   constexpr size_t kChunk = (size_t)64 * KT;
   const unsigned nwaves = gridDim.x * (THREADS / 64);
   SweepWork* const work = sr.work;
-  unsigned period = sr.period;
-  if (period == 0) {
-    period = __hip_atomic_load(&work->period, __ATOMIC_RELAXED, __HIP_MEMORY_SCOPE_AGENT);
-    if (period == 0) period = sr.period_default;
-  }
-  period = __builtin_amdgcn_readfirstlane(period);
+  SweepSet& mine_set = work->set[sr.set & 1u];
+  const unsigned period = sweep_period_in(work, sr.set, sr.period, sr.period_default);
   unsigned xcc;
   asm volatile("s_getreg_b32 %0, hwreg(HW_REG_XCC_ID)" : "=s"(xcc));
   unsigned shard = xcc & 7u;
   auto take = [&](unsigned sh) -> unsigned {
     unsigned v = 0;
-    if (lane == 0) v = atomicAdd(&work->head[sh][0], 1u);
+    if (lane == 0) v = atomicAdd(&mine_set.head[sh][0], 1u);
     return v;
   };
   const unsigned long long t_begin = __builtin_amdgcn_s_memrealtime();
@@ -101,20 +152,21 @@
   unsigned my_rounds = 0;
   __builtin_amdgcn_s_setprio(2);
   unsigned ticket = take(shard);
+  if (blockIdx.x == 0 && threadIdx.x == 0) sweep_turn_sets(work, sr.set, true, sr.rounds, nwaves, kMaxPeriod);
   while (true) {
-    unsigned rr = __builtin_amdgcn_readfirstlane(ticket);
-    if (rr >= sr.per_shard || shard * sr.per_shard + rr >= sr.rounds) {
+    const unsigned tk = __builtin_amdgcn_readfirstlane(ticket);
+    const unsigned r = sweep_round_of(shard, tk, sr.per_shard, sr.rounds);
+    if (r == kSweepNoRound) {
       bool found = false;
       for (unsigned c = 1; c < 8 && !found; ++c) {
         const unsigned sh = (shard + c) & 7u;
-        const unsigned seen = __hip_atomic_load(&work->head[sh][0], __ATOMIC_RELAXED, __HIP_MEMORY_SCOPE_AGENT);
-        if (seen < sr.per_shard && sh * sr.per_shard + seen < sr.rounds) { found = true; shard = sh; }
+        const unsigned seen = __hip_atomic_load(&mine_set.head[sh][0], __ATOMIC_RELAXED, __HIP_MEMORY_SCOPE_AGENT);
+        if (sweep_round_of(sh, seen, sr.per_shard, sr.rounds) != kSweepNoRound) { found = true; shard = sh; }
       }
       if (!found) break;
       ticket = take(shard);
       continue;
     }
-    const unsigned r = shard * sr.per_shard + rr;
     ticket = take(shard);
     ++my_rounds;
     unsigned ln = lane;
@@ -249,6 +301,7 @@
     wave_sync();
   }
   const unsigned long long t_end = __builtin_amdgcn_s_memrealtime();
+  sweep_wave_settle(sr.publish);
   if (lane == 0) {
     const unsigned my_ticks = (unsigned)(t_end - t_begin);
     atomicAdd(&wg_words[0], my_ticks);
@@ -256,26 +309,7 @@
     __builtin_amdgcn_fence(__ATOMIC_RELEASE, "workgroup");
     if (atomicAdd(&wg_words[2], 1u) == THREADS / 64 - 1) {
       __builtin_amdgcn_fence(__ATOMIC_ACQUIRE, "workgroup");
-      const unsigned wg_ticks = wg_words[0], wg_rounds = wg_words[1];
-      if (wg_rounds) {
-        const unsigned long long r1 = atomicAdd(&work->ticks, (unsigned long long)wg_ticks);
-        const unsigned r2 = atomicAdd(&work->rounds, wg_rounds);
-        asm volatile("" ::"v"(r1), "v"(r2));
-      }
-      const unsigned d = atomicAdd(&work->done[0], 1u);
-      if (d == gridDim.x - 1) {
-        const unsigned long long ticks = atomicAdd(&work->ticks, 0ull);
-        const unsigned rounds = atomicAdd(&work->rounds, 0u);
-        if (rounds >= 4 * nwaves) {
-          unsigned long long p = ticks * 9 / ((unsigned long long)rounds * 10);
-          p = p < 200 ? 200 : (p > 40000 ? 40000 : p);
-          atomicExch(&work->period, (unsigned)p);
-        }
-        for (int xx = 0; xx < 8; ++xx) atomicExch(&work->head[xx][0], 0u);
-        atomicExch(&work->ticks, 0ull);
-        atomicExch(&work->rounds, 0u);
-        atomicExch(&work->done[0], 0u);
-      }
+      sweep_workgroup_done(mine_set, wg_words[1] ? wg_words[0] : 0u, sr.status, sr.publish);
     }
     if constexpr (STAMPS) {
       if (sr.stamps) {
@@ -320,7 +354,7 @@
 }
 
 template <typename A>
-inline bool sweep_schedule(A& s, const GridDesc& g, size_t npts, size_t round_points, unsigned period_default, void* work) {
+inline bool sweep_schedule(A& s, const GridDesc& g, size_t npts, size_t round_points, unsigned period_default, void* work, const unsigned long long* status) {
   const size_t rounds = (npts + round_points - 1) / round_points;
   if (rounds > 0xFFFFFFF0ull) return false;
   s.rounds = (unsigned)rounds;
@@ -328,7 +362,10 @@
   s.period = g.cfg.sweep_period > 0 ? (unsigned)g.cfg.sweep_period : 0u;
   s.period_default = period_default;
   s.gated = g.sweep_gated ? 1u : 0u;
+  s.set = g.sweep_set & 1u;
   s.work = static_cast<SweepWork*>(work);
+  s.status = status;
+  s.publish = status ? g.sweep_publish : nullptr;
   s.stamps = nullptr;
   return true;
 }
```

Measured after the change: 109,800 (median of 6 runs). About the same (+0.5%).
